# LeonhardFeiner/sparse_rcnn

Measured on AMD Instinct MI355X. Metric: active-voxels/sec fwd+bwd, ScanNet U-Net backbone, higher is better.
Workload: dtype f32

## Files before the change

### include/scn_mi355x.h

```cpp
#ifndef SCN_MI355X_H
#define SCN_MI355X_H

#include <stdint.h>

#ifdef __cplusplus
extern "C" {
#endif

#define SCN_OK 0
#define SCN_EINVAL 1
#define SCN_ESIZE 2
#define SCN_EHASH 3
#define SCN_EHIP 4

#define SCN_ABI_VERSION 5

#define SCN_F_RELU_IN 1
#define SCN_F_W_TRANSPOSED 2
#define SCN_F_OFF_REVERSE 4
#define SCN_F_RESIDUAL_LAST 8
#define SCN_F_SPLIT_SUM 16
#define SCN_F_TILE_ORDER_X 64
#define SCN_F_GEMM_V1 32

// ... 68 lines not shown
int scn_gemm_table(const float* X, int64_t n_in, int cin, const int32_t* table, int n_off, int64_t n_out,
                   const float* W, const float* bias, const float* residual, const float* relu_mask, float* Y,
                   int cout, int flags, scn_stream_t stream);

int64_t scn_tiles_scratch_bytes(int n_off, int64_t n);
int scn_tiles_build(const int32_t* table, int n_off, int64_t n, int32_t* perm, int32_t* tstab, uint32_t* tile_mask,
                    int32_t* tile_order, void* scratch, scn_stream_t stream);
int64_t scn_tiles_order_ints(int64_t n, int with_x);
int scn_tiles_build_x(const int32_t* table, int n_off, int64_t n, int32_t* perm, int32_t* tstab, uint32_t* tile_mask,
                      int32_t* tile_order, int with_x, void* scratch, scn_stream_t stream);

int64_t scn_sort_pairs_scratch_bytes(int64_t n);
int scn_sort_pairs(const uint32_t* keys, const int32_t* vals, int64_t n, int bits, uint32_t* keys_out,
                   int32_t* vals_out, void* scratch, scn_stream_t stream);

int64_t scn_conv_tiles_scratch_bytes(int cin, int64_t n_out, int cout);
int64_t scn_conv_tiles_arrival_counters(int cin, int64_t n_out, int cout);
int scn_conv_tiles(const float* X, int64_t n_in, int cin, const int32_t* tstab, const uint32_t* tile_mask, const int32_t* perm,
                   const int32_t* tile_order, int n_off, int64_t n_out, const float* W, const float* bias, const float* residual,
                   const float* relu_mask, float* Y, int cout, int flags, void* scratch, int32_t* arrival,
                   scn_stream_t stream);
typedef struct scn_conv_role {
    const void* X; const void* W; const void* bias; const void* residual; const void* relu_mask; void* Y;
    int32_t flags; int32_t reserved;
} scn_conv_role;
int scn_conv_tiles_chain(int n_roles, const scn_conv_role* roles, int64_t n_in, int cin, const int32_t* tstab,
                         const uint32_t* tile_mask, const int32_t* perm, const int32_t* tile_order, int n_off, int64_t n_out,
                         int cout, void* scratch, int32_t* arrival, scn_stream_t stream);
void scn_conv_tiles_chain_counts(int64_t out[2], int reset);
void scn_conv_tiles_path_counts(int64_t out[4], int reset);
int64_t scn_conv_tiles_split_count(int reset);
int scn_conv_tiles_finish(int cin, int64_t n_out, const float* bias, const float* residual, const float* relu_mask,
                          float* Y, int cout, int flags, void* scratch, scn_stream_t stream);

int64_t scn_conv_tiles_bf16_image_bytes(int cin, int cout, int n_off);
int scn_conv_tiles_bf16_pack(const float* W, int cin, int cout, int n_off, int flags, uint16_t* image, scn_stream_t stream);
int scn_conv_tiles_bf16_pack_many(int n, const float* const* W_host, const int32_t* cin_host, const int32_t* cout_host,
                                  const int32_t* n_off_host, const int32_t* flags_host, uint16_t* const* image_host,
                                  scn_stream_t stream);
int64_t scn_conv_tiles_bf16_scratch_bytes(int cin, int64_t n_out, int cout);
int64_t scn_conv_tiles_bf16_arrival_counters(int cin, int64_t n_out, int cout);
int scn_conv_tiles_bf16(const uint16_t* X, int64_t n_in, int cin, const int32_t* tstab, const uint32_t* tile_mask,
                        const int32_t* perm, const int32_t* tile_order, int n_off, int64_t n_out, const uint16_t* image,
                        const float* bias, const uint16_t* residual, const uint16_t* relu_mask, uint16_t* Y, int cout,
                        int flags, void* scratch, int32_t* arrival, scn_stream_t stream);

int scn_gemm_rules(const float* X, int cin, const int32_t* in_rows, const int32_t* out_rows,
                   const int64_t* prefix_host, int n_off, const float* W, const float* bias, const float* relu_mask,
                   float* Y, int cout, int flags, scn_stream_t stream);

int64_t scn_wgrad_scratch_bytes(int cin, int cout, const int64_t* prefix_host, int n_off);
int scn_wgrad_rules(const float* X, int cin, const float* dY, int cout, const int32_t* in_rows,
                    const int32_t* out_rows, const int64_t* prefix_host, int n_off, float* dW, void* scratch,
                    int flags, scn_stream_t stream);

int scn_gemm_rows2(const void* X0, int cx0, const void* X1, int cx1, int64_t n, const float* W, const float* bias,
                   const void* residual, const void* relu_mask, void* Y0, int cy0, void* Y1, int cy1, int flags,
                   int bf16_storage, scn_stream_t stream);

int scn_gemm_table_bf16(const uint16_t* X, int64_t n_in, int cin, const int32_t* table, int n_off, int64_t n_out,
                        const float* W, const float* bias, const uint16_t* residual, const uint16_t* relu_mask,
                        uint16_t* Y, int cout, int flags, scn_stream_t stream);
int scn_gemm_rules_bf16(const uint16_t* X, int cin, const int32_t* in_rows, const int32_t* out_rows,
                        const int64_t* prefix_host, int n_off, const float* W, const float* bias,
                        const uint16_t* relu_mask, uint16_t* Y, int cout, int flags, scn_stream_t stream);

int scn_wgrad_rules_bf16(const uint16_t* X, int cin, const uint16_t* dY, int cout, const int32_t* in_rows,
                         const int32_t* out_rows, const int64_t* prefix_host, int n_off, float* dW, void* scratch,
                         int flags, scn_stream_t stream);
int scn_wgrad_bias_rules_bf16(const uint16_t* X, int cin, const uint16_t* dY, int cout, const int32_t* in_rows,
                              const int32_t* out_rows, const int64_t* prefix_host, int n_off, float* dW, float* db,
                              uint32_t db_offsets, void* scratch, int flags, scn_stream_t stream);
int scn_wgrad_bias_rules(const float* X, int cin, const float* dY, int cout, const int32_t* in_rows,
                         const int32_t* out_rows, const int64_t* prefix_host, int n_off, float* dW, float* db,
                         uint32_t db_offsets, void* scratch, int flags, scn_stream_t stream);

int scn_wgrad_defer_begin(void);
int scn_wgrad_defer_flush(scn_stream_t stream);
int scn_wgrad_step_begin(void);
int scn_wgrad_step_hold(int on);
int scn_wgrad_step_flush(scn_stream_t stream);
int scn_wgrad_step_discard(void);
void scn_wgrad_group_counts(int64_t out[4], int reset);
int64_t scn_wgrad_scratch_bytes2(int cin, int cout, const int64_t* prefix_host, int n_off);
int scn_wgrad_bias_rules2(const float* X0, const float* dY0, const float* X1, const float* dY1, int cin, int cout,
                          const int32_t* in_rows, const int32_t* out_rows, const int64_t* prefix_host, int n_off,
                          float* dW, float* db, uint32_t db_offsets, void* scratch, int flags, scn_stream_t stream);

int64_t scn_wgrad_scratch_bytes_n(int cin, int cout, const int64_t* prefix_host, int n_off, int n_prob);
int scn_wgrad_bias_rules_n(const float* const* Xs, const float* const* dYs, int n_prob, int cin, int cout,
                          const int32_t* in_rows, const int32_t* out_rows, const int64_t* prefix_host, int n_off,
                          float* dW, float* db, uint32_t db_offsets, void* scratch, int flags, scn_stream_t stream);
int scn_wgrad_bias_rules_n_bf16(const uint16_t* const* Xs, const uint16_t* const* dYs, int n_prob, int cin, int cout,
                               const int32_t* in_rows, const int32_t* out_rows, const int64_t* prefix_host, int n_off,
                               float* dW, float* db, uint32_t db_offsets, void* scratch, int flags, scn_stream_t stream);
int scn_wgrad_bias_rules2_bf16(const uint16_t* X0, const uint16_t* dY0, const uint16_t* X1, const uint16_t* dY1, int cin,
                               int cout, const int32_t* in_rows, const int32_t* out_rows, const int64_t* prefix_host,
                               int n_off, float* dW, float* db, uint32_t db_offsets, void* scratch, int flags,
                               scn_stream_t stream);

#define SCN_COLSUM_BLOCKS 512
int scn_colsum(const float* dY, int64_t n, int c, float* db, void* scratch, scn_stream_t stream);
int scn_colsum_bf16(const uint16_t* dY, int64_t n, int c, float* db, void* scratch, scn_stream_t stream);


int scn_relu_fwd(const float* X, int64_t count, float* Y, scn_stream_t stream);
int scn_relu_bwd(const float* X, const float* dY, int64_t count, float* dX, scn_stream_t stream);
int scn_add(const float* A, const float* B, int64_t count, float* Y, scn_stream_t stream);

int64_t scn_bn_scratch_bytes(int c);
int scn_bn_stats(const float* X, int64_t n, int c, float* mean, float* var_biased,
                 void* scratch , scn_stream_t stream);
int scn_bn_fwd(const float* X, int64_t n, int c, const float* mean, const float* var, float eps, const float* gamma,
               const float* beta, float leak, float* Y, scn_stream_t stream);
int scn_bn_bwd(const float* X, const float* dY, int64_t n, int c, const float* mean, const float* var, float eps,
               const float* gamma, const float* beta, float leak, int training, float* dX, float* dgamma, float* dbeta,
               void* scratch , scn_stream_t stream);

int scn_bn_sums(const float* X, int64_t n, int c, double* sums, void* scratch, scn_stream_t stream);
int scn_bn_bwd_reduce(const float* X, const float* dY, int64_t n, int c, const float* mean, const float* var, float eps,
                      const float* gamma, const float* beta, float leak, float* dgamma, float* dbeta, double* sums,
                      void* scratch, scn_stream_t stream);
int scn_bn_bwd_apply(const float* X, const float* dY, int64_t n, int c, const float* mean, const float* var, float eps,
                     const float* gamma, const float* beta, float leak, const double* sums, int64_t n_stat, float* dX,
                     scn_stream_t stream);

int scn_input_fwd(const float* feats, const int32_t* item_row, const int32_t* row_count, const int32_t* row_first,
                  int64_t n_items, int64_t n_rows, int c, int mode, float* Y, double* acc64, int32_t* row_last,
                  scn_stream_t stream);
int scn_input_bwd(const float* dY, const int32_t* item_row, const int32_t* row_count, const int32_t* row_first,
                  const int32_t* row_last, int64_t n_items, int c, int mode, float* dfeats, scn_stream_t stream);
int scn_gather_rows(const float* X, const int32_t* rows, int64_t m, int c, float* Y, scn_stream_t stream);
int scn_segment_sum(const float* dY, const int32_t* item_row, int64_t n_items, int64_t n_rows, int c, float* dX,
                    double* acc64, scn_stream_t stream);

int64_t scn_segment_pool_scratch_bytes(int n_samples, int c);
int scn_sample_counts(const int32_t* coords, int64_t n, int n_samples, int32_t* cnt, int32_t* unsorted, scn_stream_t stream);
int scn_segment_pool_fwd(const float* X, const int32_t* coords, int64_t n, int c, int n_samples, int op, float* Y,
                         int32_t* cnt, int32_t* unsorted, void* scratch, scn_stream_t stream);
int scn_segment_pool_bwd(const float* X, const float* Y, const float* dY, const int32_t* coords, int64_t n, int c,
                         int n_samples, int op, const int32_t* cnt, float* dX, void* scratch, scn_stream_t stream);

int scn_sparse_to_dense_fwd(const float* X, const int32_t* coords, int64_t n, int c, const int64_t* size3_host,
                            float* out, scn_stream_t stream);
int scn_sparse_to_dense_bwd(const float* dOut, const int32_t* coords, int64_t n, int c, const int64_t* size3_host,
                            float* dX, scn_stream_t stream);

int scn_pool_fwd(const float* X, const int32_t* child, int64_t n_coarse, int c, int average, float* Y,
                 scn_stream_t stream);
int scn_pool_bwd(const float* X, const float* Y, const float* dY, const int32_t* parent, int64_t n_fine, int c,
                 int average, float* dX, scn_stream_t stream);


int scn_mask_scatter(const float* scores, int64_t m, int k, const int32_t* src_point, const int32_t* box_of,
                     const int64_t* class_of_box, int num_valid, const int64_t* row_base, float* out,
                     scn_stream_t stream);

int scn_mask_gather(const float* scores, int64_t m, int k, const int32_t* src_point, const int32_t* box_of,
                    const int64_t* label_of_box, const int64_t* gt_base, const float* gt_flat, float* pred, float* gt,
                    uint8_t* keep_row, scn_stream_t stream);
int scn_mask_gather_bwd(const float* dpred, int64_t m, int k, const int32_t* box_of, const int64_t* label_of_box,
                        const int64_t* gt_base, float* dscores, scn_stream_t stream);

int scn_nms(const float* boxes, int batch, int n, float overlap_threshold, uint8_t* keep, scn_stream_t stream);
int64_t scn_nms_scratch_bytes(int batch, int n);
int scn_nms_bits(const float* boxes, int batch, int n, float overlap_threshold, uint8_t* keep, void* scratch,
                 scn_stream_t stream);

int64_t scn_topk_scratch_bytes(int batch);
int scn_topk_boxes(const float* scores, const float* boxes, int batch, int64_t n, int k, float* out_scores,
                   int64_t* out_index, float* out_boxes, void* scratch, scn_stream_t stream);


int64_t scn_vox_scratch_bytes(int64_t n);
int scn_vox_project(const float* points, int64_t n, const float* rot_and_scale_host, const float* offset_host,
                    float* aug, float* shift_max, void* scratch, scn_stream_t stream);

int scn_vox_discretize(const float* aug, int64_t n, const float* shift, const int32_t* test_start_host,
                       const int32_t* size_host, int32_t* discrete, int32_t* table, scn_stream_t stream);

int scn_vox_gather(const int32_t* discrete, const int32_t* rows, int64_t m, const int32_t* start_host,
                   int64_t batch_index, int64_t* out, scn_stream_t stream);


int scn_pad_params_many(int n, const float* const* in_host, float* const* out_host, const int32_t* desc_host, int backward,
                        scn_stream_t stream);
// ... 188 lines not shown
```

### sparse_rcnn_amd/_lib.py

```python
from __future__ import annotations

import ctypes as C
import os

import torch

_HERE = os.path.dirname(os.path.abspath(__file__))
LIB_PATH = os.environ.get("SCN_MI355X_LIB") or os.path.join(_HERE, "libscn_mi355x.so")

_lib = None

p = C.c_void_p
i32, i64, f32 = C.c_int, C.c_int64, C.c_float

_SIGS = {
    "scn_abi_version": (C.c_int, []),
    "scn_last_error_string": (C.c_char_p, []),
    "scn_debug_set": (C.c_int, [C.c_char_p, C.c_char_p]),
    "scn_debug_get": (C.c_int, [C.c_char_p, C.POINTER(C.c_int), C.POINTER(i64)]),
    "scn_hash_capacity": (i64, [i64]),
    "scn_coords_to_i32": (C.c_int, [p, i64, p, p, C.POINTER(i64), p]),
    "scn_dedup_scratch_bytes": (i64, [i64]),
    "scn_dedup_build": (C.c_int, [p, i64, i32, p, p, i64, p, p, p, p, p, C.POINTER(i64), p]),
    "scn_dedup_launch": (C.c_int, [p, i64, i32, p, p, i64, p, p, p, p, p, p, p]),
    "scn_dedup_launch_div": (C.c_int, [p, i64, i32, i32, i32, p, p, i64, p, p, p, p, p, p, p]),
    "scn_child_table_div": (C.c_int, [p, p, i64, i64, i32, i32, i32, p, p, p]),
    "scn_parent_lookup_div": (C.c_int, [p, i64, i32, i32, i32, p, p, i64, p, p, p]),
    "scn_subm_table": (C.c_int, [p, i64, p, p, i64, i32, p, p]),
    "scn_child_table": (C.c_int, [p, p, i64, i64, p, p, p]),
    "scn_rules_blocks": (i64, [i32, i64]),
    "scn_rules_scan": (C.c_int, [p, i32, i64, p, p, C.POINTER(i64), p]),
    "scn_rules_fill": (C.c_int, [p, i32, i64, p, p, p, p, p]),
    "scn_pyramid_workspace_bytes": (i64, [i64, i32, i32]),
    "scn_pyramid_build": (C.c_int, [p, i64, i32, i32, p, i64, C.POINTER(i64), p]),
    "scn_pyramid_build_ex": (C.c_int, [p, i64, i32, i32, p, i64, C.POINTER(i64), i32, p]),
    "scn_roi_units": (i64, [i64]),
    "scn_roi_count": (C.c_int, [p, i64, p, i32, p, p, p, p]),
    "scn_roi_fill": (C.c_int, [p, i64, p, i32, p, p, p, p, p, p]),
    "scn_roi_inside": (C.c_int, [p, p, i64, i64, i32, p, p]),
    "scn_roi_coords": (C.c_int, [p, p, p, i64, p, p]),
    "scn_roi_boxes": (C.c_int, [p, p, i32, p, p, p, p]),
    "scn_gemm_table": (C.c_int, [p, i64, i32, p, i32, i64, p, p, p, p, p, i32, i32, p]),
    "scn_tiles_scratch_bytes": (i64, [i32, i64]),
    "scn_tiles_build": (C.c_int, [p, i32, i64, p, p, p, p, p, p]),
    "scn_tiles_build_x": (C.c_int, [p, i32, i64, p, p, p, p, i32, p, p]),
    "scn_tiles_order_ints": (i64, [i64, i32]),
    "scn_sort_pairs_scratch_bytes": (i64, [i64]),
    "scn_sort_pairs": (C.c_int, [p, p, i64, i32, p, p, p, p]),
    "scn_conv_tiles_scratch_bytes": (i64, [i32, i64, i32]),
    "scn_conv_tiles_arrival_counters": (i64, [i32, i64, i32]),
    "scn_conv_tiles": (C.c_int, [p, i64, i32, p, p, p, p, i32, i64, p, p, p, p, p, i32, i32, p, p, p]),
    "scn_conv_tiles_chain": (C.c_int, [i32, p, i64, i32, p, p, p, p, i32, i64, i32, p, p, p]),
    "scn_conv_tiles_chain_counts": (None, [C.POINTER(i64), i32]),
    "scn_wgrad_tiles32_scratch_bytes": (i64, []),
    "scn_wgrad_tiles32": (C.c_int, [p, i64, p, i64, p, p, p, p, p, p, i32, p]),
    "scn_conv_tiles_path_counts": (None, [C.POINTER(i64), i32]),
    "scn_conv_tiles_split_count": (i64, [i32]),
    "scn_conv_tiles_finish": (C.c_int, [i32, i64, p, p, p, p, i32, i32, p, p]),
    "scn_conv_tiles_bf16_image_bytes": (i64, [i32, i32, i32]),
    "scn_conv_tiles_bf16_pack": (C.c_int, [p, i32, i32, i32, i32, p, p]),
    "scn_conv_tiles_bf16_pack_many": (C.c_int, [i32, p, p, p, p, p, p, p]),
    "scn_conv_tiles_bf16_scratch_bytes": (i64, [i32, i64, i32]),
    "scn_conv_tiles_bf16_arrival_counters": (i64, [i32, i64, i32]),
    "scn_conv_tiles_bf16": (C.c_int, [p, i64, i32, p, p, p, p, i32, i64, p, p, p, p, p, i32, i32, p, p, p]),
    "scn_gemm_rules": (C.c_int, [p, i32, p, p, C.POINTER(i64), i32, p, p, p, p, i32, i32, p]),
    "scn_wgrad_scratch_bytes": (i64, [i32, i32, C.POINTER(i64), i32]),
    "scn_wgrad_rules": (C.c_int, [p, i32, p, i32, p, p, C.POINTER(i64), i32, p, p, i32, p]),
    "scn_gemm_table_bf16": (C.c_int, [p, i64, i32, p, i32, i64, p, p, p, p, p, i32, i32, p]),
    "scn_gemm_rules_bf16": (C.c_int, [p, i32, p, p, C.POINTER(i64), i32, p, p, p, p, i32, i32, p]),
    "scn_gemm_rows2": (C.c_int, [p, i32, p, i32, i64, p, p, p, p, p, i32, p, i32, i32, i32, p]),
    "scn_wgrad_rules_bf16": (C.c_int, [p, i32, p, i32, p, p, C.POINTER(i64), i32, p, p, i32, p]),
    "scn_wgrad_bias_rules": (C.c_int, [p, i32, p, i32, p, p, C.POINTER(i64), i32, p, p, C.c_uint32, p, i32, p]),
    "scn_wgrad_bias_rules_bf16": (C.c_int, [p, i32, p, i32, p, p, C.POINTER(i64), i32, p, p, C.c_uint32, p, i32, p]),
    "scn_wgrad_scratch_bytes2": (i64, [i32, i32, C.POINTER(i64), i32]),
    "scn_wgrad_defer_begin": (C.c_int, []),
    "scn_wgrad_defer_flush": (C.c_int, [p]),
    "scn_wgrad_step_begin": (C.c_int, []),
    "scn_wgrad_step_hold": (C.c_int, [i32]),
    "scn_wgrad_step_flush": (C.c_int, [p]),
    "scn_wgrad_step_discard": (C.c_int, []),
    "scn_wgrad_group_counts": (None, [C.POINTER(i64), i32]),
    "scn_wgrad_bias_rules2": (C.c_int, [p, p, p, p, i32, i32, p, p, C.POINTER(i64), i32, p, p, C.c_uint32, p, i32, p]),
    "scn_wgrad_bias_rules2_bf16": (C.c_int, [p, p, p, p, i32, i32, p, p, C.POINTER(i64), i32, p, p, C.c_uint32, p, i32, p]),
    "scn_wgrad_scratch_bytes_n": (i64, [i32, i32, C.POINTER(i64), i32, i32]),
    "scn_wgrad_bias_rules_n": (C.c_int, [C.POINTER(p), C.POINTER(p), i32, i32, i32, p, p, C.POINTER(i64), i32, p, p, C.c_uint32, p, i32, p]),
    "scn_wgrad_bias_rules_n_bf16": (C.c_int, [C.POINTER(p), C.POINTER(p), i32, i32, i32, p, p, C.POINTER(i64), i32, p, p, C.c_uint32, p, i32, p]),
    "scn_colsum": (C.c_int, [p, i64, i32, p, p, p]),
    "scn_colsum_bf16": (C.c_int, [p, i64, i32, p, p, p]),
    "scn_relu_fwd": (C.c_int, [p, i64, p, p]),
    "scn_relu_bwd": (C.c_int, [p, p, i64, p, p]),
    "scn_add": (C.c_int, [p, p, i64, p, p]),
    "scn_bn_scratch_bytes": (i64, [i32]),
    "scn_bn_stats": (C.c_int, [p, i64, i32, p, p, p, p]),
    "scn_bn_sums": (C.c_int, [p, i64, i32, p, p, p]),
    "scn_bn_bwd_reduce": (C.c_int, [p, p, i64, i32, p, p, f32, p, p, f32, p, p, p, p, p]),
    "scn_bn_bwd_apply": (C.c_int, [p, p, i64, i32, p, p, f32, p, p, f32, p, i64, p, p]),
    "scn_bn_fwd": (C.c_int, [p, i64, i32, p, p, f32, p, p, f32, p, p]),
    "scn_bn_bwd": (C.c_int, [p, p, i64, i32, p, p, f32, p, p, f32, i32, p, p, p, p, p]),
    "scn_input_fwd": (C.c_int, [p, p, p, p, i64, i64, i32, i32, p, p, p, p]),
    "scn_input_bwd": (C.c_int, [p, p, p, p, p, i64, i32, i32, p, p]),
    "scn_gather_rows": (C.c_int, [p, p, i64, i32, p, p]),
    "scn_segment_sum": (C.c_int, [p, p, i64, i64, i32, p, p, p]),
    "scn_mask_scatter": (C.c_int, [p, i64, i32, p, p, p, i32, p, p, p]),
    "scn_mask_gather": (C.c_int, [p, i64, i32, p, p, p, p, p, p, p, p, p]),
    "scn_mask_gather_bwd": (C.c_int, [p, i64, i32, p, p, p, p, p]),
    "scn_vox_scratch_bytes": (i64, [i64]),
    "scn_vox_project": (C.c_int, [p, i64, p, p, p, p, p, p]),
    "scn_vox_discretize": (C.c_int, [p, i64, p, p, p, p, p, p]),
    "scn_vox_gather": (C.c_int, [p, p, i64, p, i64, p, p]),
    "scn_nms": (C.c_int, [p, i32, i32, f32, p, p]),
    "scn_dilate_gather_fwd": (C.c_int, [p, p, i32, C.POINTER(i64), i32, i32, p, p, p]),
    "scn_dilate_gather_bwd": (C.c_int, [p, p, i64, C.POINTER(i64), i32, i32, p, p]),
    "scn_cell_map": (C.c_int, [p, i64, i32, C.POINTER(i64), p, p, p, p]),
    "scn_nms_scratch_bytes": (i64, [i32, i32]),
    "scn_nms_bits": (C.c_int, [p, i32, i32, f32, p, p, p]),
    "scn_topk_scratch_bytes": (C.c_int64, [i32]),
    "scn_topk_boxes": (C.c_int, [p, p, i32, i64, i32, p, p, p, p, p]),
    "scn_pool_fwd": (C.c_int, [p, p, i64, i32, i32, p, p]),
    "scn_pool_bwd": (C.c_int, [p, p, p, p, i64, i32, i32, p, p]),
    "scn_segment_pool_scratch_bytes": (i64, [i32, i32]),
    "scn_sample_counts": (C.c_int, [p, i64, i32, p, p, p]),
    "scn_segment_pool_fwd": (C.c_int, [p, p, i64, i32, i32, i32, p, p, p, p, p]),
    "scn_segment_pool_bwd": (C.c_int, [p, p, p, p, i64, i32, i32, i32, p, p, p, p]),
    "scn_pad_params_many": (C.c_int, [i32, p, p, p, i32, p]),
    "scn_cast_f32_to_bf16": (C.c_int, [p, i64, p, p]),
    "scn_cast_bf16_to_f32": (C.c_int, [p, i64, p, p]),
    "scn_add_bf16": (C.c_int, [p, p, i64, p, p]),
    "scn_gather_rows_bf16": (C.c_int, [p, p, i64, i32, p, p]),
    "scn_segment_sum_bf16": (C.c_int, [p, p, i64, i64, i32, p, p, p]),
    "scn_pool_fwd_bf16": (C.c_int, [p, p, i64, i32, i32, p, p]),
    "scn_pool_bwd_bf16": (C.c_int, [p, p, p, p, i64, i32, i32, p, p]),
    "scn_sparse_to_dense_fwd_bf16": (C.c_int, [p, p, i64, i32, C.POINTER(i64), p, p]),
    "scn_sparse_to_dense_bwd_bf16": (C.c_int, [p, p, i64, i32, C.POINTER(i64), p, p]),
    "scn_exec_struct_bytes": (i64, [i32]),
    "scn_exec_requirements": (C.c_int, [p, i32, p, i32, C.POINTER(i64), C.POINTER(i64)]),
    "scn_exec_run": (C.c_int, [p, i32, p, i32, p, p, p, p, i64, p, p]),
    "scn_exec_run_streams": (C.c_int, [p, i32, p, i32, p, p, p, p, i64, p, p, p, p, i64]),
    "scn_exec_timing_enable": (C.c_int, [i32]),
    "scn_exec_timing_collect": (i64, [p, p, i64]),
    "scn_sparse_to_dense_fwd": (C.c_int, [p, p, i64, i32, C.POINTER(i64), p, p]),
    "scn_sparse_to_dense_bwd": (C.c_int, [p, p, i64, i32, C.POINTER(i64), p, p]),
    "scn_adam_segment_bytes": (i64, []),
    "scn_adam_launches": (C.c_int, [p, i32, C.POINTER(i32)]),
    "scn_adam_many": (C.c_int, [p, i32, C.c_double, C.c_double, C.c_double, C.c_double, p]),
    "scn_rpn_targets": (C.c_int, [p, i64, p, C.POINTER(i64), i32, p, p, p, p]),
    "scn_rpn_sample_workspace_bytes": (i64, []),
    "scn_rpn_sample_batchwise": (C.c_int, [p, i64, f32, f32, f32, C.c_uint64, C.c_uint64, p, p, p, p, p, p]),
    "scn_rpn_loss_scratch_bytes": (i64, [i64]),
    "scn_rpn_loss": (C.c_int, [p, p, p, p, p, p, i64, f32, p, p, p, p, p, p]),
    "scn_rpn_loss_scale": (C.c_int, [p, p, i64, p, p, p, p, p]),
    "scn_mask_overlap_draw": (C.c_int, [p, C.POINTER(i64), p, C.POINTER(i64), i32, p, p, i32, f32, i32, C.c_uint64,
                                        C.c_uint64, C.POINTER(i64), p, p, p, p, p]),
    "scn_mask_loss_scratch_bytes": (i64, [i64, i64]),
    "scn_mask_loss": (C.c_int, [p, i64, i32, p, p, p, C.POINTER(i64), p, C.POINTER(i64), p, C.POINTER(i64), C.POINTER(i64), i32,
                                p, p, p, p]),
    "scn_mask_loss_bwd": (C.c_int, [p, p, i64, i64, i32, p, p, p]),
    "scn_mask_pack": (C.c_int, [C.POINTER(p), C.POINTER(i64), C.POINTER(i64), i32, p, p]),
    "scn_xent_scratch_bytes": (i64, [i64, i32]),
    "scn_xent_fwd": (C.c_int, [p, i64, i32, p, p, i64, p, p, p, p]),
    "scn_xent_bwd": (C.c_int, [p, p, i64, i32, p, p, i64, p, p, p]),
    "scn_softmax_argmax": (C.c_int, [p, i64, i32, p, p, p]),
    "scn_eval_mask_bits": (C.c_int, [p, i64, i32, p, p, p, i32, f32, p, i64, i64, p, p]),
    "scn_eval_pack_threshold": (C.c_int, [p, i64, i64, f32, p, p]),
    "scn_eval_mask_iou": (C.c_int, [p, C.POINTER(i64), p, C.POINTER(i64), C.POINTER(i64), C.POINTER(i64), C.POINTER(i64),
                                    C.POINTER(i64), i32, p, p, p, p, p, p]),
    "scn_eval_bbox_iou": (C.c_int, [p, C.POINTER(i64), p, C.POINTER(i64), C.POINTER(i64), i32, p, p]),
    "scn_eval_match": (C.c_int, [p, p, p, p, i32, i64, p, p, p, p, p, p, p, i32, i32, p, p, p]),
    "scn_eval_confusion": (C.c_int, [p, p, i64, i32, p, p, p]),
    "scn_sample_stats": (C.c_int, [p, p, p, i64, i32, p, p, p, p]),
    "scn_sample_pack": (C.c_int, [p, i64, p, p, p, i32, p, p, i32, p, i32, i32, i32, i32, p, p, p, p, i64, p, p]),
    "scn_roialign_fwd": (C.c_int, [p, i32, C.POINTER(i64), i32, p, p, i64, C.POINTER(i64), p, p, p]),
# ... 124 lines not shown
```

### sparse_rcnn_amd/csrc/scn_common.h

```cpp
#pragma once
#include <hip/hip_runtime.h>
#include <atomic>
#include <stdint.h>
#include <stdio.h>
#include <string.h>

#include "../../include/scn_mi355x.h"

namespace scn {

extern thread_local char g_err[512];

inline int fail(int code, const char* fmt, const char* a = "", long long b = 0, long long c = 0) {
    snprintf(g_err, sizeof(g_err), fmt, a, b, c);
    return code;
}

#define SCN_HIP(expr)                                                                               \
    do {                                                                                            \
        hipError_t e_ = (expr);                                                                     \
        if (e_ != hipSuccess) {                                                                     \
            snprintf(scn::g_err, sizeof(scn::g_err), "%s failed: %s (%s:%d)", #expr,                \
                     hipGetErrorString(e_), __FILE__, __LINE__);                                    \
            return SCN_EHIP;                                                                        \
        }                                                                                           \
    } while (0)

#define SCN_LAUNCH_CHECK()                                                                          \
    do {                                                                                            \
        hipError_t e_ = hipGetLastError();                                                          \
        if (e_ != hipSuccess) {                                                                     \
            snprintf(scn::g_err, sizeof(scn::g_err), "kernel launch failed: %s (%s:%d)",            \
                     hipGetErrorString(e_), __FILE__, __LINE__);                                    \
            return SCN_EHIP;                                                                        \
        }                                                                                           \
    } while (0)

#define SCN_REQUIRE(cond)                                                                           \
    do {                                                                                            \
        if (!(cond)) {                                                                              \
            snprintf(scn::g_err, sizeof(scn::g_err), "%s: requirement failed: %s", __func__, #cond); \
            return SCN_EINVAL;                                                                      \
        }                                                                                           \
    } while (0)

enum Switch {
    SW_TS_SPLIT, SW_TS_SPLIT_MAX, SW_TS_NO_TAIL, SW_TS_W_HALF, SW_TS_W_BOTH, SW_TB_NB, SW_TB_KH, SW_TB_STREAM,
    SW_TB_NO_XORDER, SW_TS_STREAM, SW_TSS_NW, SW_EXEC_DEFER_SUMS, SW_PYRAMID_V1, SW_PYRAMID_ONE_STREAM, SW_WD_NO_T3,
    SW_WGRAD_BF16_MFMA, SW_WGRAD_SPLITS, SW_WD_NO_EVEC, SW_PYRAMID_NO_BRICKS, SW_CU_BUDGET, SW_EXP_A, SW_EXP_B, SW_TS_NO_CHAIN, SW_TS_PROG, SW_TB_NO_BINS,
    SW_EXEC_GROUP_WGRAD, SW_EXEC_GROUP_STEP, SW_COUNT
};
struct SwitchVal { bool set = false; long long i = 0; double f = 0.0; };
SwitchVal sw(Switch s);
inline int cu_budget() { const SwitchVal v = sw(SW_CU_BUDGET); return (v.set && v.i >= 32 && v.i <= 256) ? (int)v.i : 256; }

struct DeviceOnce {
    std::atomic<uint64_t> mask{0};
    static int cur() { int d = 0; return (hipGetDevice(&d) == hipSuccess && d >= 0 && d < 64) ? d : -1; }
    bool needed() const { const int d = cur(); return d < 0 || !(mask.load(std::memory_order_acquire) & (1ull << d)); }
    void done() { const int d = cur(); if (d >= 0) mask.fetch_or(1ull << d, std::memory_order_release); }
};

int wgrad_defer_group(bool on);

inline hipStream_t S(scn_stream_t s) { return reinterpret_cast<hipStream_t>(s); }

inline int64_t cdiv(int64_t a, int64_t b) { return (a + b - 1) / b; }

inline int ew_grid(int64_t work_items, int block) {
    int64_t g = cdiv(work_items, block);
    if (g > 256 * 8) g = 256 * 8;
    if (g < 1) g = 1;
    return (int)g;
}

}

#define SCN_EMPTY_KEY 0xFFFFFFFFFFFFFFFFull

__device__ __forceinline__ unsigned long long scn_pack_key(int x, int y, int z, int b) {
    return ((unsigned long long)(unsigned)b << 48) | ((unsigned long long)(unsigned)x << 32) |
           ((unsigned long long)(unsigned)y << 16) | (unsigned long long)(unsigned)z;
}

__device__ __forceinline__ unsigned long long scn_hash_slot(unsigned long long key, unsigned long long mask) {
    unsigned long long h = key;
    h ^= h >> 33;
    h *= 0xff51afd7ed558ccdull;
    h ^= h >> 33;
    h *= 0xc4ceb9fe1a85ec53ull;
    h ^= h >> 33;
    return h & mask;
}

__device__ __forceinline__ float scn_mask_sigmoid(float x) { return 1.f / (1.f + __expf(-x)); }

__device__ __forceinline__ float scn_box_iou(const float* as, const float* ae, float area_a, const float* bx) {
#pragma clang fp contract(off)
    float inter = 1.f;
#pragma unroll
    for (int d = 0; d < 3; ++d) {
        const float lo = fmaxf(as[d], bx[d]), hi = fminf(ae[d], bx[3 + d]);
        const float e = fmaxf((hi - lo), 0.f);
        inter = d == 0 ? e : (inter * e);
    }
    const float uni = (area_a + bx[6]) - inter;
    return (inter / uni);
}
```

### sparse_rcnn_amd/csrc/scn_conv.hip

```cpp
#include "scn_common.h"

using scn::S;
using scn::cdiv;

namespace scn {
bool gemm_lt_usable(const void* X0, const void* X1, int cx0, int cx1, const void* W);
int gemm_lt_rows(const void* X0, int cx0, const void* X1, int cx1, int64_t n, const float* W, const float* bias,
                 const void* residual, const void* relu_mask, void* Y0, int cy0, void* Y1, int cy1, int flags, bool hb,
                 scn_stream_t stream);
int gemm_lt_rules(const void* X, int cin, const int32_t* in_rows, const int32_t* out_rows, const int64_t* prefix_host,
                  int n_off, const float* W, const float* bias, const void* relu_mask, void* Y, int cout, int flags,
                  bool hb, scn_stream_t stream);
}

typedef float f32x16 __attribute__((ext_vector_type(16)));

#define MFMA(a, b, c) __builtin_amdgcn_mfma_f32_32x32x2f32((a), (b), (c), 0, 0, 0)

__device__ __forceinline__ int acc_row(int v, int h) { return (v & 3) + 8 * (v >> 2) + 4 * h; }

__device__ __forceinline__ float bf16_bits_to_f32(unsigned short h) { return __uint_as_float((unsigned)h << 16); }
__device__ __forceinline__ unsigned short f32_to_bf16_bits(float f) { return __builtin_bit_cast(unsigned short, (__bf16)f); }

template <bool FAST, bool WT, bool HB = false>
// ... 178 lines not shown
                           : X + (long long)(idx >= 0 ? idx : 0) * cin;
    tile_mac<FAST, WT, HB>(acc, xrow, idx >= 0, cin, Wo, cout, n, n_ok, h, flags & SCN_F_RELU_IN);

    const float bv = (bias && n_ok) ? bias[n] : 0.f;
#pragma unroll
    for (int v = 0; v < 16; ++v) {
        const int r = __shfl(orow, acc_row(v, h));
        if (r >= 0 && n_ok) {
            const long long off = (long long)r * cout + n;
            float y = acc[v] + bv;
            if (HB) {
                if (relu_mask && !(bf16_bits_to_f32(((const unsigned short*)relu_mask)[off]) > 0.f)) y = 0.f;
                ((unsigned short*)Y)[off] = f32_to_bf16_bits(y);
            } else {
                if (relu_mask && !(relu_mask[off] > 0.f)) y = 0.f;
                Y[off] = y;
            }
        }
    }
}

static int make_seg_tiles(const int64_t* prefix_host, int n_off, int tile, SegTiles& seg) {
    seg.n_off = n_off;
    seg.rule_start[0] = prefix_host[0];
    seg.tile_start[0] = 0;
    for (int o = 0; o < n_off; ++o) {
        int64_t cnt = prefix_host[o + 1] - prefix_host[o];
        if (cnt < 0) return SCN_EINVAL;
        seg.rule_start[o + 1] = prefix_host[o + 1];
        seg.tile_start[o + 1] = seg.tile_start[o] + cdiv(cnt, tile);
    }
    return SCN_OK;
}

static int gemm_rules_impl(const float* X, int cin, const int32_t* in_rows, const int32_t* out_rows,
                           const int64_t* prefix_host, int n_off, const float* W, const float* bias,
                           const float* relu_mask, float* Y, int cout, int flags, scn_stream_t stream, bool hb) {
    SCN_REQUIRE(prefix_host && n_off >= 1 && n_off <= 32 && cin >= 1 && cout >= 1);
    SegTiles seg;
    SCN_REQUIRE(make_seg_tiles(prefix_host, n_off, 32, seg) == SCN_OK);
    const long long tiles = seg.tile_start[n_off];
    if (tiles == 0) return SCN_OK;
    SCN_REQUIRE(X && in_rows && out_rows && W && Y);
    const bool fast = (cin % 8 == 0) && (((uintptr_t)X & 15) == 0) && (((uintptr_t)W & 15) == 0);
    const bool wt = flags & SCN_F_W_TRANSPOSED;
    if (fast && cout > 32 && !(flags & SCN_F_GEMM_V1))
        return scn::gemm_lt_rules(X, cin, in_rows, out_rows, prefix_host, n_off, W, bias, relu_mask, Y, cout, flags, hb,
                                  stream);
    dim3 grid((unsigned)cdiv(tiles, 4), (unsigned)cdiv(cout, 32));
#define LAUNCH_R(F, T, H)                                                                                     \
    hipLaunchKernelGGL((k_gemm_rules<F, T, H>), grid, dim3(256), 0, S(stream), X, cin, in_rows, out_rows, seg, \
                       W, bias, relu_mask, Y, cout, flags)
#define PICK_R(H)                                                                                             \
    do {                                                                                                      \
        if (fast && wt) LAUNCH_R(true, true, H);                                                              \
        else if (fast) LAUNCH_R(true, false, H);                                                              \
        else if (wt) LAUNCH_R(false, true, H);                                                                \
        else LAUNCH_R(false, false, H);                                                                       \
    } while (0)
    if (hb) PICK_R(true); else PICK_R(false);
#undef PICK_R
#undef LAUNCH_R
    SCN_LAUNCH_CHECK();
    return SCN_OK;
}

extern "C" int scn_gemm_rules(const float* X, int cin, const int32_t* in_rows, const int32_t* out_rows,
                              const int64_t* prefix_host, int n_off, const float* W, const float* bias,
                              const float* relu_mask, float* Y, int cout, int flags, scn_stream_t stream) {
    return gemm_rules_impl(X, cin, in_rows, out_rows, prefix_host, n_off, W, bias, relu_mask, Y, cout, flags, stream,
                           false);
}

extern "C" int scn_gemm_rules_bf16(const uint16_t* X, int cin, const int32_t* in_rows, const int32_t* out_rows,
                                   const int64_t* prefix_host, int n_off, const float* W, const float* bias,
                                   const uint16_t* relu_mask, uint16_t* Y, int cout, int flags, scn_stream_t stream) {
    return gemm_rules_impl((const float*)X, cin, in_rows, out_rows, prefix_host, n_off, W, bias,
                           (const float*)relu_mask, (float*)Y, cout, flags, stream, true);
}

template <bool HB>
__global__ __launch_bounds__(256) void k_colsum_partial(const float* __restrict__ dY, long long n, int c,
                                                        float* __restrict__ partial) {
    const unsigned short* dYh = (const unsigned short*)dY;
    const long long rows_per_block = (n + gridDim.x - 1) / gridDim.x;
    const long long r_lo = blockIdx.x * rows_per_block;
    long long r_hi = r_lo + rows_per_block;
    if (r_hi > n) r_hi = n;
    __shared__ float red[256];
    for (int c0 = 0; c0 < c; c0 += 256) {
        const int width = min(256, c - c0);
        const int lanes_per_row = width;
        const int rows_par = 256 / lanes_per_row > 0 ? 256 / lanes_per_row : 1;
        const int col = threadIdx.x % lanes_per_row;
        const int rsub = threadIdx.x / lanes_per_row;
        float s = 0.f;
        if (rsub < rows_par)
            for (long long r = r_lo + rsub; r < r_hi; r += rows_par)
                s += HB ? bf16_bits_to_f32(dYh[r * c + c0 + col]) : dY[r * c + c0 + col];
        red[threadIdx.x] = (rsub < rows_par) ? s : 0.f;
        __syncthreads();
        if (threadIdx.x < width) {
            float t = 0.f;
            for (int k = 0; k < rows_par; ++k) t += red[k * lanes_per_row + threadIdx.x];
            partial[(long long)blockIdx.x * c + c0 + threadIdx.x] = t;
        }
        __syncthreads();
    }
}

__global__ __launch_bounds__(256) void k_colsum_final(const float* __restrict__ partial, int nblk, int c,
                                                      float* __restrict__ db) {
    const int col = blockIdx.x;
    float s = 0.f;
    for (int b = threadIdx.x; b < nblk; b += 256) s += partial[(long long)b * c + col];
#pragma unroll
    for (int d = 32; d >= 1; d >>= 1) s += __shfl_down(s, d);
    __shared__ float w[4];
    if ((threadIdx.x & 63) == 0) w[threadIdx.x >> 6] = s;
    __syncthreads();
    if (threadIdx.x == 0) db[col] = (w[0] + w[1]) + (w[2] + w[3]);
}

static int colsum_impl(const float* dY, int64_t n, int c, float* db, void* scratch, scn_stream_t stream, bool hb) {
    SCN_REQUIRE(n >= 0 && c >= 1 && db && scratch);
    int nblk = (int)(n < SCN_COLSUM_BLOCKS * 8 ? cdiv(n, 8) : SCN_COLSUM_BLOCKS);
    if (nblk < 1) nblk = 1;
    if (n > 0) SCN_REQUIRE(dY);
    if (hb)
        hipLaunchKernelGGL(k_colsum_partial<true>, dim3(nblk), dim3(256), 0, S(stream), dY, (long long)n, c, (float*)scratch);
    else
        hipLaunchKernelGGL(k_colsum_partial<false>, dim3(nblk), dim3(256), 0, S(stream), dY, (long long)n, c, (float*)scratch);
    SCN_LAUNCH_CHECK();
    hipLaunchKernelGGL(k_colsum_final, dim3(c), dim3(256), 0, S(stream), (const float*)scratch, nblk, c, db);
    SCN_LAUNCH_CHECK();
    return SCN_OK;
}

extern "C" int scn_colsum(const float* dY, int64_t n, int c, float* db, void* scratch, scn_stream_t stream) {
    return colsum_impl(dY, n, c, db, scratch, stream, false);
}

extern "C" int scn_colsum_bf16(const uint16_t* dY, int64_t n, int c, float* db, void* scratch, scn_stream_t stream) {
    return colsum_impl((const float*)dY, n, c, db, scratch, stream, true);
}
```

### sparse_rcnn_amd/csrc/scn_debug.hip

```cpp
#include <stdlib.h>

#include <mutex>

#include "scn_common.h"

namespace scn {
namespace {
struct Entry { const char* name; SwitchVal v; };
Entry g_sw[SW_COUNT] = {
    {"SCN_TS_SPLIT", {}},        {"SCN_TS_SPLIT_MAX", {}},  {"SCN_TS_NO_TAIL", {}},       {"SCN_TS_W_HALF", {}},
    {"SCN_TS_W_BOTH", {}},       {"SCN_TB_NB", {}},         {"SCN_TB_KH", {}},            {"SCN_TB_STREAM", {}},
    {"SCN_TB_NO_XORDER", {}},    {"SCN_TS_STREAM", {}},     {"SCN_TSS_NW", {}},           {"SCN_EXEC_DEFER_SUMS", {}},
    {"SCN_PYRAMID_V1", {}},      {"SCN_PYRAMID_ONE_STREAM", {}}, {"SCN_WD_NO_T3", {}},    {"SCN_WGRAD_BF16_MFMA", {}},
    {"SCN_WGRAD_SPLITS", {}},    {"SCN_WD_NO_EVEC", {}},    {"SCN_PYRAMID_NO_BRICKS", {}},            {"SCN_CU_BUDGET", {}},
    {"SCN_EXP_A", {}},           {"SCN_EXP_B", {}},         {"SCN_TS_NO_CHAIN", {}},
    {"SCN_TS_PROG", {}},         {"SCN_TB_NO_BINS", {}},    {"SCN_EXEC_GROUP_WGRAD", {}},
    {"SCN_EXEC_GROUP_STEP", {}},
};
std::once_flag g_once;
std::mutex g_mu;

void assign(SwitchVal& v, const char* s) {
    v.set = s != nullptr;
    v.i = s ? atoll(s) : 0;
    v.f = s ? atof(s) : 0.0;
}
void load_env() {
    for (int k = 0; k < SW_COUNT; ++k) assign(g_sw[k].v, getenv(g_sw[k].name));
}
}

SwitchVal sw(Switch s) {
    std::call_once(g_once, load_env);
    std::lock_guard<std::mutex> lock(g_mu);
    return g_sw[s].v;
}
}

extern "C" int scn_debug_set(const char* name, const char* value) {
    SCN_REQUIRE(name != nullptr);
    std::call_once(scn::g_once, scn::load_env);
    std::lock_guard<std::mutex> lock(scn::g_mu);
    for (int k = 0; k < scn::SW_COUNT; ++k)
        if (strcmp(scn::g_sw[k].name, name) == 0) {
            scn::assign(scn::g_sw[k].v, value);
            return SCN_OK;
        }
    return scn::fail(SCN_EINVAL, "scn_debug_set: no switch named %s", name);
}

extern "C" int scn_debug_get(const char* name, int* is_set, int64_t* value) {
    SCN_REQUIRE(name != nullptr);
    for (int k = 0; k < scn::SW_COUNT; ++k)
        if (strcmp(scn::g_sw[k].name, name) == 0) {
            const scn::SwitchVal v = scn::sw((scn::Switch)k);
            if (is_set) *is_set = v.set ? 1 : 0;
            if (value) *value = v.i;
            return SCN_OK;
        }
    return scn::fail(SCN_EINVAL, "scn_debug_get: no switch named %s", name);
}
```

### sparse_rcnn_amd/csrc/scn_exec.hip

```cpp
#include <stdlib.h>
#include <vector>

#include <atomic>
#include <mutex>
#include <vector>

#include "scn_common.h"

using scn::cdiv;

namespace {

struct Ctx {
    const scn_exec_level* levels;
    int n_levels;
    void* const* bufs;
    const void* const* params;
    void* const* grads;
    void* scratch;
    int32_t* arrival;
    scn_stream_t stream;
};

inline int64_t align256(int64_t b) { return (b + 255) & ~(int64_t)255; }

int64_t wgrad_scratch_of(const scn_exec_op& o, const scn_exec_level& L) {
    switch (o.op) {
    case SCN_OP_WGRAD_SUBM: return scn_wgrad_scratch_bytes(o.cin, o.cout, L.prefix_host, 27);
    case SCN_OP_WGRAD2_SUBM: return scn_wgrad_scratch_bytes2(o.cin, o.cout, L.prefix_host, 27);
    case SCN_OP_WGRAD_DOWN:
    case SCN_OP_WGRAD_UP: return scn_wgrad_scratch_bytes(o.cin, o.cout, L.c_prefix_host, 8);
    case SCN_OP_WGRAD_IDENT: {
        const int64_t ident[2] = {0, (o.flags & SCN_XF_COARSE_ROWS) ? L.n_coarse : L.n};
        return scn_wgrad_scratch_bytes(o.cin, o.cout, ident, 1);
    }
    default: return 0;
    }
}

inline bool bf(const scn_exec_op& o) { return (o.flags & SCN_XF_BF16) != 0; }
inline int call_flags(const scn_exec_op& o) { return o.flags & 0xffff; }
inline int64_t rows_of(const scn_exec_op& o, const scn_exec_level& L) {
    return (o.flags & SCN_XF_COARSE_ROWS) ? L.n_coarse : L.n;
}

template <typename T>
inline T* B(const Ctx& c, int id) { return id < 0 ? nullptr : (T*)c.bufs[id]; }
template <typename T>
inline const T* P(const Ctx& c, int id) { return id < 0 ? nullptr : (const T*)c.params[id]; }
template <typename T>
inline T* G(const Ctx& c, int id) { return id < 0 ? nullptr : (T*)c.grads[id]; }

int run_op(const Ctx& c0, const scn_exec_op& o, void* own_scratch = nullptr) {
    SCN_REQUIRE(o.level >= 0 && o.level < c0.n_levels);
    const scn_exec_level& L = c0.levels[o.level];
    Ctx c = c0;
    if (own_scratch) c.scratch = own_scratch;
    const int fl = call_flags(o);
    const bool h = bf(o);
    scn_stream_t st = c.stream;
    typedef uint16_t u16;
    switch (o.op) {
    case SCN_OP_GEMM_IDENT: {
        const int64_t n = rows_of(o, L);
        if (h) return scn_gemm_table_bf16(B<u16>(c, o.x), n, o.cin, nullptr, 1, n, P<float>(c, o.w), P<float>(c, o.b),
                                          B<u16>(c, o.r), B<u16>(c, o.m), B<u16>(c, o.y), o.cout, fl, st);
        return scn_gemm_table(B<float>(c, o.x), n, o.cin, nullptr, 1, n, P<float>(c, o.w), P<float>(c, o.b), B<float>(c, o.r),
                              B<float>(c, o.m), B<float>(c, o.y), o.cout, fl, st);
    }
    case SCN_OP_CONV_SUBM:
    case SCN_OP_CONV_CHILD: {
        const bool child = o.op == SCN_OP_CONV_CHILD;
        const int64_t n_in = L.n, n_out = child ? L.n_coarse : L.n;
        const int n_off = child ? 8 : 27;
        const int32_t* tstab = child ? L.c_tstab : L.tstab;
        const uint32_t* tmask = child ? L.c_tile_mask : L.tile_mask;
        const int32_t* perm = child ? L.c_perm : L.perm;
        const int32_t* order = child ? L.c_tile_order : L.tile_order;
        if (h) {
            int32_t* arr = scn_conv_tiles_bf16_arrival_counters(o.cin, n_out, o.cout) ? c.arrival : nullptr;
            const int flx = fl | ((!child && (L.flags & SCN_XL_TILE_ORDER_X)) ? SCN_F_TILE_ORDER_X : 0);
            return scn_conv_tiles_bf16(B<u16>(c, o.x), n_in, o.cin, tstab, tmask, perm, order, n_off, n_out, P<u16>(c, o.w),
                                       P<float>(c, o.b), B<u16>(c, o.r), B<u16>(c, o.m), B<u16>(c, o.y), o.cout, flx, c.scratch,
                                       arr, st);
        }
        int32_t* arr = o.cin > 32 ? c.arrival : nullptr;
        return scn_conv_tiles(B<float>(c, o.x), n_in, o.cin, tstab, tmask, perm, order, n_off, n_out, P<float>(c, o.w),
                              P<float>(c, o.b), B<float>(c, o.r), B<float>(c, o.m), B<float>(c, o.y), o.cout, fl, c.scratch, arr,
                              st);
    }
    case SCN_OP_RULES_CHILD: {
        if (h) return scn_gemm_rules_bf16(B<u16>(c, o.x), o.cin, L.c_out_rows, L.c_in_rows, L.c_prefix_host, 8, P<float>(c, o.w),
                                          P<float>(c, o.b), B<u16>(c, o.m), B<u16>(c, o.y), o.cout, fl, st);
        return scn_gemm_rules(B<float>(c, o.x), o.cin, L.c_out_rows, L.c_in_rows, L.c_prefix_host, 8, P<float>(c, o.w),
                              P<float>(c, o.b), B<float>(c, o.m), B<float>(c, o.y), o.cout, fl, st);
    }
    case SCN_OP_ROWS2: {
        const int64_t n = rows_of(o, L);
        if (o.y1 >= 0)
            return scn_gemm_rows2(B<void>(c, o.x), o.cin, nullptr, 0, n, P<float>(c, o.w), nullptr, nullptr, nullptr,
                                  B<void>(c, o.y), o.cout, B<void>(c, o.y1), o.c1, fl, h ? 1 : 0, st);
        return scn_gemm_rows2(B<void>(c, o.x), o.cin, B<void>(c, o.x1), o.c1, n, P<float>(c, o.w), P<float>(c, o.b), nullptr,
                              nullptr, B<void>(c, o.y), o.cout, nullptr, 0, fl, h ? 1 : 0, st);
    }
    case SCN_OP_WGRAD_SUBM: {
        const uint32_t dbm = o.b >= 0 ? (1u << 13) : 0u;
        if (h) return scn_wgrad_bias_rules_bf16(B<u16>(c, o.x), o.cin, B<u16>(c, o.y), o.cout, L.in_rows, L.out_rows, L.prefix_host,
                                                27, G<float>(c, o.w), G<float>(c, o.b), dbm, c.scratch, fl, st);
        return scn_wgrad_bias_rules(B<float>(c, o.x), o.cin, B<float>(c, o.y), o.cout, L.in_rows, L.out_rows, L.prefix_host, 27,
                                    G<float>(c, o.w), G<float>(c, o.b), dbm, c.scratch, fl, st);
    }
    case SCN_OP_WGRAD2_SUBM: {
        const uint32_t dbm = o.b >= 0 ? (1u << 13) : 0u;
        if (h) return scn_wgrad_bias_rules2_bf16(B<u16>(c, o.x), B<u16>(c, o.y), B<u16>(c, o.x1), B<u16>(c, o.y1), o.cin, o.cout,
                                                 L.in_rows, L.out_rows, L.prefix_host, 27, G<float>(c, o.w), G<float>(c, o.b), dbm,
                                                 c.scratch, fl, st);
        return scn_wgrad_bias_rules2(B<float>(c, o.x), B<float>(c, o.y), B<float>(c, o.x1), B<float>(c, o.y1), o.cin, o.cout,
                                     L.in_rows, L.out_rows, L.prefix_host, 27, G<float>(c, o.w), G<float>(c, o.b), dbm, c.scratch,
                                     fl, st);
    }
    case SCN_OP_WGRAD_DOWN: {
        if (h) return scn_wgrad_rules_bf16(B<u16>(c, o.x), o.cin, B<u16>(c, o.y), o.cout, L.c_in_rows, L.c_out_rows,
                                           L.c_prefix_host, 8, G<float>(c, o.w), c.scratch, fl, st);
        return scn_wgrad_rules(B<float>(c, o.x), o.cin, B<float>(c, o.y), o.cout, L.c_in_rows, L.c_out_rows, L.c_prefix_host, 8,
                               G<float>(c, o.w), c.scratch, fl, st);
    }
    case SCN_OP_WGRAD_UP: {
        if (o.b < 0) {
            if (h) return scn_wgrad_rules_bf16(B<u16>(c, o.x), o.cin, B<u16>(c, o.y), o.cout, L.c_out_rows, L.c_in_rows,
                                               L.c_prefix_host, 8, G<float>(c, o.w), c.scratch, fl, st);
            return scn_wgrad_rules(B<float>(c, o.x), o.cin, B<float>(c, o.y), o.cout, L.c_out_rows, L.c_in_rows, L.c_prefix_host,
                                   8, G<float>(c, o.w), c.scratch, fl, st);
        }
        if (h) return scn_wgrad_bias_rules_bf16(B<u16>(c, o.x), o.cin, B<u16>(c, o.y), o.cout, L.c_out_rows, L.c_in_rows,
                                                L.c_prefix_host, 8, G<float>(c, o.w), G<float>(c, o.b), 0xFFu, c.scratch, fl, st);
        return scn_wgrad_bias_rules(B<float>(c, o.x), o.cin, B<float>(c, o.y), o.cout, L.c_out_rows, L.c_in_rows, L.c_prefix_host,
                                    8, G<float>(c, o.w), G<float>(c, o.b), 0xFFu, c.scratch, fl, st);
    }
    case SCN_OP_WGRAD_IDENT: {
        const int64_t ident[2] = {0, rows_of(o, L)};
        float* dW = G<float>(c, o.w);
        SCN_REQUIRE(dW != nullptr);
        dW += o.aux;
        if (o.b < 0) {
            if (h) return scn_wgrad_rules_bf16(B<u16>(c, o.x), o.cin, B<u16>(c, o.y), o.cout, nullptr, nullptr, ident, 1, dW,
                                               c.scratch, fl, st);
            return scn_wgrad_rules(B<float>(c, o.x), o.cin, B<float>(c, o.y), o.cout, nullptr, nullptr, ident, 1, dW, c.scratch, fl,
                                   st);
        }
        if (h) return scn_wgrad_bias_rules_bf16(B<u16>(c, o.x), o.cin, B<u16>(c, o.y), o.cout, nullptr, nullptr, ident, 1, dW,
                                                G<float>(c, o.b), 1u, c.scratch, fl, st);
        return scn_wgrad_bias_rules(B<float>(c, o.x), o.cin, B<float>(c, o.y), o.cout, nullptr, nullptr, ident, 1, dW,
                                    G<float>(c, o.b), 1u, c.scratch, fl, st);
    }
    case SCN_OP_COLSUM: {
        const int64_t n = rows_of(o, L);
        if (h) return scn_colsum_bf16(B<u16>(c, o.x), n, o.cin, G<float>(c, o.b), c.scratch, st);
        return scn_colsum(B<float>(c, o.x), n, o.cin, G<float>(c, o.b), c.scratch, st);
    }
    case SCN_OP_ADD: {
        const int64_t count = rows_of(o, L) * o.cin;
        if (h) return scn_add_bf16(B<u16>(c, o.x), B<u16>(c, o.x1), count, B<u16>(c, o.y), st);
        return scn_add(B<float>(c, o.x), B<float>(c, o.x1), count, B<float>(c, o.y), st);
    }
    case SCN_OP_CAST: {
        const int64_t count = rows_of(o, L) * o.cin;
        if (h) return scn_cast_f32_to_bf16(B<float>(c, o.x), count, B<u16>(c, o.y), st);
        return scn_cast_bf16_to_f32(B<u16>(c, o.x), count, B<float>(c, o.y), st);
    }
    default:
        return scn::fail(SCN_EINVAL, "scn_exec_run: unknown op %s%lld", "", o.op);
    }
}

}

extern "C" int64_t scn_exec_struct_bytes(int which) {
    return which == 0 ? (int64_t)sizeof(scn_exec_op) : (which == 1 ? (int64_t)sizeof(scn_exec_level) : -1);
}

namespace {
int pass_needs(const scn_exec_op* ops, int n_ops, const scn_exec_level* levels, int n_levels, int64_t* shared, int64_t* wg_sum,
               int64_t* wg_max, int* n_wg, int64_t* arrival) {
    int64_t sb = 256, ac = 0, ws = 0, wm = 0;
    int nw = 0;
    for (int i = 0; i < n_ops; ++i) {
        const scn_exec_op& o = ops[i];
        SCN_REQUIRE(o.level >= 0 && o.level < n_levels);
        const scn_exec_level& L = levels[o.level];
        int64_t s = 0, a = 0;
        switch (o.op) {
        case SCN_OP_CONV_SUBM:
        case SCN_OP_CONV_CHILD: {
            const int64_t n_out = o.op == SCN_OP_CONV_CHILD ? L.n_coarse : L.n;
            if (bf(o)) {
                s = scn_conv_tiles_bf16_scratch_bytes(o.cin, n_out, o.cout);
                a = scn_conv_tiles_bf16_arrival_counters(o.cin, n_out, o.cout);
            } else {
                s = scn_conv_tiles_scratch_bytes(o.cin, n_out, o.cout);
                a = scn_conv_tiles_arrival_counters(o.cin, n_out, o.cout);
            }
            break;
        }
        case SCN_OP_COLSUM: s = (int64_t)SCN_COLSUM_BLOCKS * o.cin * (int64_t)sizeof(float); break;
        default: {
            const int64_t w = wgrad_scratch_of(o, L);
            if (w < 0) return scn::fail(SCN_EINVAL, "scn_exec: op %s%lld has bad arguments", "", i);
            if (w > 0) { ws += align256(w); ++nw; if (w > wm) wm = w; }
            break;
        }
        }
        if (s < 0) return scn::fail(SCN_EINVAL, "scn_exec: op %s%lld has bad arguments", "", i);
        if (s > sb) sb = s;
        if (a > ac) ac = a;
    }
    *shared = sb; *wg_sum = ws; *wg_max = wm; *n_wg = nw; *arrival = ac;
    return SCN_OK;
}
}

extern "C" int scn_exec_requirements(const scn_exec_op* ops, int n_ops, const scn_exec_level* levels, int n_levels,
                                     int64_t* scratch_bytes, int64_t* arrival_counters) {
    SCN_REQUIRE(n_ops >= 0 && (n_ops == 0 || ops) && levels && n_levels >= 1 && scratch_bytes && arrival_counters);
    int64_t shared, wg_sum, wg_max, ac;
    int n_wg;
    const int rc = pass_needs(ops, n_ops, levels, n_levels, &shared, &wg_sum, &wg_max, &n_wg, &ac);
    if (rc != SCN_OK) return rc;
    int64_t sb = align256(shared) + wg_sum;
    if (wg_max > sb) sb = wg_max;
    *scratch_bytes = sb;
    *arrival_counters = ac;
    return SCN_OK;
}

namespace {
struct EventPool {
    static constexpr int N = 32;
    hipEvent_t ev[N] = {};
    int next = 0;
    bool ok = false;
    bool init() {
        if (ok) return true;
        for (auto& e : ev)
            if (hipEventCreateWithFlags(&e, hipEventDisableTiming) != hipSuccess) return false;
        return ok = true;
    }
    hipEvent_t take() { hipEvent_t e = ev[next]; next = (next + 1) % N; return e; }
};
thread_local EventPool g_events;

struct TimingRec { hipEvent_t a, b; int64_t info[7]; };
struct Timing {
    std::mutex mu;
    std::atomic<bool> on{false}, all{false};
    std::vector<hipEvent_t> pool;
    size_t used = 0;
    std::vector<TimingRec> recs;
    hipEvent_t take() {
        if (used == pool.size()) {
            hipEvent_t e = nullptr;
            if (hipEventCreate(&e) != hipSuccess) return nullptr;
            pool.push_back(e);
        }
        return pool[used++];
    }
};
Timing g_timing;

inline bool is_wgrad(int op) {
    return op == SCN_OP_WGRAD_SUBM || op == SCN_OP_WGRAD2_SUBM || op == SCN_OP_WGRAD_DOWN || op == SCN_OP_WGRAD_UP ||
           op == SCN_OP_WGRAD_IDENT;
}
inline bool is_leaf(int op) {
    return op == SCN_OP_WGRAD_SUBM || op == SCN_OP_WGRAD2_SUBM || op == SCN_OP_WGRAD_DOWN || op == SCN_OP_WGRAD_UP ||
           op == SCN_OP_WGRAD_IDENT || op == SCN_OP_COLSUM;
}

bool overwritten_later(const scn_exec_op* ops, int n_ops, int i, void* const* bufs) {
    const scn_exec_op& o = ops[i];
    const int reads[4] = {o.x, o.y, o.x1, o.y1};
    for (int j = i + 1; j < n_ops; ++j) {
        if (is_leaf(ops[j].op)) continue;
        const int writes[2] = {ops[j].y, ops[j].y1};
        for (int w : writes) {
            if (w < 0) continue;
            for (int r : reads)
                if (r >= 0 && (r == w || (bufs[r] != nullptr && bufs[r] == bufs[w]))) return true;
        }
    }
    return false;
}
}

extern "C" int scn_exec_run_streams(const scn_exec_op* ops, int n_ops, const scn_exec_level* levels, int n_levels,
                                    void* const* bufs, const void* const* params, void* const* grads, void* scratch,
                                    int64_t scratch_bytes, int32_t* arrival, scn_stream_t stream, scn_stream_t side_stream,
                                    void* side_scratch, int64_t side_scratch_bytes) {
    SCN_REQUIRE(n_ops >= 0 && (n_ops == 0 || ops) && levels && n_levels >= 1 && bufs && scratch && scratch_bytes >= 256);
    const bool fork = side_stream != nullptr && side_stream != stream && side_scratch != nullptr && side_scratch_bytes >= scratch_bytes;
    if (fork && !g_events.init()) return scn::fail(SCN_EHIP, "%sevents for the side stream could not be created", "");
    const bool defer_env = !(scn::sw(scn::SW_EXEC_DEFER_SUMS).set && scn::sw(scn::SW_EXEC_DEFER_SUMS).i == 0);
    int n_wg = 0;
    for (int i = 0; i < n_ops; ++i) n_wg += is_wgrad(ops[i].op) ? 1 : 0;
    std::vector<int64_t> own(defer_env && !fork && n_wg >= 2 ? n_ops : 0, 0);
    bool defer = false;
    if (!own.empty()) {
        int64_t shared, wg_sum, wg_max, ac;
        int nw;
        const int rc_needs = pass_needs(ops, n_ops, levels, n_levels, &shared, &wg_sum, &wg_max, &nw, &ac);
        if (rc_needs != SCN_OK) return rc_needs;
        if (align256(shared) + wg_sum <= scratch_bytes) {
            int64_t cursor = align256(shared);
            for (int i = 0; i < n_ops; ++i) {
                const int64_t w = is_wgrad(ops[i].op) ? wgrad_scratch_of(ops[i], levels[ops[i].level]) : 0;
                if (w > 0) { own[i] = cursor; cursor += align256(w); }
            }
            defer = true;
        }
    }
    const scn::SwitchVal group_sw = scn::sw(scn::SW_EXEC_GROUP_WGRAD);
    const bool group = defer && !(group_sw.set && group_sw.i == 0) && !g_timing.on;
    Ctx c{levels, n_levels, bufs, params, grads, scratch, arrival, stream};
    Ctx cs{levels, n_levels, bufs, params, grads, side_scratch, arrival, side_stream};
    if (defer) SCN_REQUIRE(scn_wgrad_defer_begin() == SCN_OK);
    if (group) SCN_REQUIRE(scn::wgrad_defer_group(true) == SCN_OK);
    bool side_used = false;
    for (int i = 0; i < n_ops; ++i) {
        int rc;
        if (fork && is_leaf(ops[i].op)) {
            hipEvent_t e = g_events.take();
            SCN_HIP(hipEventRecord(e, scn::S(stream)));
            SCN_HIP(hipStreamWaitEvent(scn::S(side_stream), e, 0));
            rc = run_op(cs, ops[i]);
            side_used = true;
        } else if (g_timing.on && (g_timing.all || ops[i].op == SCN_OP_CONV_SUBM || ops[i].op == SCN_OP_CONV_CHILD)) {
            std::lock_guard<std::mutex> lock(g_timing.mu);
            const scn_exec_op& o = ops[i];
            const scn_exec_level& L = levels[o.level];
            const bool child = o.op == SCN_OP_CONV_CHILD;
            TimingRec r{};
            r.a = g_timing.take();
            r.b = g_timing.take();
            if (r.a && r.b) SCN_HIP(hipEventRecord(r.a, scn::S(stream)));
            rc = run_op(c, ops[i], defer && own[i] ? (char*)scratch + own[i] : nullptr);
            if (r.a && r.b) {
                SCN_HIP(hipEventRecord(r.b, scn::S(stream)));
                r.info[0] = o.op; r.info[1] = bf(o) ? 1 : 0; r.info[2] = o.cin; r.info[3] = o.cout;
                r.info[4] = L.n; r.info[5] = child ? L.n_coarse : L.n;
                r.info[6] = child ? L.n : (L.prefix_host ? L.prefix_host[27] - L.prefix_host[0] : 0);
                g_timing.recs.push_back(r);
            }
        } else if (group && is_wgrad(ops[i].op) && overwritten_later(ops, n_ops, i, bufs)) {
            (void)scn::wgrad_defer_group(false);
            rc = run_op(c, ops[i], own[i] ? (char*)scratch + own[i] : nullptr);
            (void)scn::wgrad_defer_group(true);
        } else {
            rc = run_op(c, ops[i], defer && own[i] ? (char*)scratch + own[i] : nullptr);
        }
        if (rc != SCN_OK) {
            char inner[400];
            snprintf(inner, sizeof(inner), "%s", scn::g_err);
            snprintf(scn::g_err, sizeof(scn::g_err), "scn_exec_run: op %d (kind %d, level %d): %s", i, ops[i].op, ops[i].level,
                     inner);
            if (defer) (void)scn_wgrad_defer_flush(stream);
            return rc;
        }
    }
    if (defer) {
        const int rc = scn_wgrad_defer_flush(stream);
        if (rc != SCN_OK) return rc;
    }
    if (side_used) {
        hipEvent_t e = g_events.take();
        SCN_HIP(hipEventRecord(e, scn::S(side_stream)));
        SCN_HIP(hipStreamWaitEvent(scn::S(stream), e, 0));
    }
    return SCN_OK;
}

extern "C" int scn_exec_timing_enable(int on) {
    std::lock_guard<std::mutex> lock(g_timing.mu);
    g_timing.on = on != 0;
    g_timing.all = on == 2;
    return SCN_OK;
}

extern "C" int64_t scn_exec_timing_collect(float* ms, int64_t* info, int64_t cap) {
    std::lock_guard<std::mutex> lock(g_timing.mu);
    int64_t n = 0;
    size_t taken = 0;
    for (; taken < g_timing.recs.size() && n < cap; ++taken) {
        const TimingRec& r = g_timing.recs[taken];
        float t = 0.f;
        if (hipEventSynchronize(r.b) != hipSuccess || hipEventElapsedTime(&t, r.a, r.b) != hipSuccess) continue;
        ms[n] = t;
        for (int j = 0; j < 7; ++j) info[7 * n + j] = r.info[j];
        ++n;
    }
    g_timing.recs.erase(g_timing.recs.begin(), g_timing.recs.begin() + (ptrdiff_t)taken);
    if (g_timing.recs.empty()) g_timing.used = 0;
    return n;
}

extern "C" int scn_exec_run(const scn_exec_op* ops, int n_ops, const scn_exec_level* levels, int n_levels, void* const* bufs,
                            const void* const* params, void* const* grads, void* scratch, int64_t scratch_bytes,
                            int32_t* arrival, scn_stream_t stream) {
    return scn_exec_run_streams(ops, n_ops, levels, n_levels, bufs, params, grads, scratch, scratch_bytes, arrival, stream,
                                nullptr, nullptr, 0);
}
```

### sparse_rcnn_amd/csrc/scn_wgrad.hip

```cpp
#include <stdlib.h>

#include <string.h>
#include <mutex>
#include <vector>

#include "scn_common.h"

#ifndef WD_DEEP_ALL
#define WD_DEEP_ALL 1
#endif

using scn::S;
using scn::cdiv;

typedef float f32x4 __attribute__((ext_vector_type(4)));
#define MFMA16(a, b, c) __builtin_amdgcn_mfma_f32_16x16x4f32((a), (b), (c), 0, 0, 0)

#ifndef WD_EXP
#define WD_EXP 0
#endif
#ifndef WD_TIMELINE
#define WD_TIMELINE 0
#endif
#if WD_TIMELINE
// ... 299 lines not shown
        for (int b = 0; b < TB; ++b) acc[a][b] = (f32x4){0.f, 0.f, 0.f, 0.f};
    f32x4 dbacc[TB];
#pragma unroll
    for (int b = 0; b < TB; ++b) dbacc[b] = (f32x4){0.f, 0.f, 0.f, 0.f};
    s16x8 ones;
#pragma unroll
    for (int e = 0; e < 8; ++e) ones[e] = (lane & 15) == 0 ? (short)0x3F80 : (short)0;

    const int g = lane >> 4, q = (lane & 15) >> 2, pp = lane & 3;
    int tr_a[2][TA], tr_b[2][TB];
#pragma unroll
    for (int t = 0; t < 2; ++t) {
        const int row = 8 * g + 4 * t + q;
#pragma unroll
        for (int a = 0; a < TA; ++a) tr_a[t][a] = wtb_off(row, 2 * (wi * TA + a) + (pp >> 1)) + 8 * (pp & 1);
#pragma unroll
        for (int b = 0; b < TB; ++b) tr_b[t][b] = IMG + wtb_off(row, 2 * (wj * TB + b) + (pp >> 1)) + 8 * (pp & 1);
    }

    int idx0[NLD], idx1[NLD];
    uint4 st[NLD];
    if (nsteps > 0) {
        load_idx(0, idx0);
        load_idx(1, idx1);
        load_rows(idx0, st);
    }
    for (int s = 0; s < nsteps; ++s) {
        const int buf = s & 1;
        store_rows(buf, st);
        if (s + 1 < nsteps) {
            if (s & 1) { load_rows(idx0, st); load_idx(s + 2, idx1); }
            else { load_rows(idx1, st); load_idx(s + 2, idx0); }
        }
        __syncthreads();
        const char* base = wlds + buf * 2 * IMG;
        bf16x8 fa[TA], fb[TB];
#pragma unroll
        for (int a = 0; a < TA; ++a) {
            const s16x4 lo = __builtin_amdgcn_ds_read_tr16_b64_v4i16((__attribute__((address_space(3))) s16x4*)(base + tr_a[0][a]));
            const s16x4 hi = __builtin_amdgcn_ds_read_tr16_b64_v4i16((__attribute__((address_space(3))) s16x4*)(base + tr_a[1][a]));
            fa[a] = __builtin_bit_cast(bf16x8, __builtin_shufflevector(lo, hi, 0, 1, 2, 3, 4, 5, 6, 7));
        }
#pragma unroll
        for (int b = 0; b < TB; ++b) {
            const s16x4 lo = __builtin_amdgcn_ds_read_tr16_b64_v4i16((__attribute__((address_space(3))) s16x4*)(base + tr_b[0][b]));
            const s16x4 hi = __builtin_amdgcn_ds_read_tr16_b64_v4i16((__attribute__((address_space(3))) s16x4*)(base + tr_b[1][b]));
            fb[b] = __builtin_bit_cast(bf16x8, __builtin_shufflevector(lo, hi, 0, 1, 2, 3, 4, 5, 6, 7));
        }
#pragma unroll
        for (int a = 0; a < TA; ++a)
#pragma unroll
            for (int b = 0; b < TB; ++b) acc[a][b] = MFMAB32(fa[a], fb[b], acc[a][b]);
        if (do_db) {
#pragma unroll
            for (int b = 0; b < TB; ++b) dbacc[b] = MFMAB32(__builtin_bit_cast(bf16x8, ones), fb[b], dbacc[b]);
        }
    }

    float* slab = slabs + ((long long)unit * (plan.nbi * plan.nbj) + blockIdx.z) * (CBI * CBJ);
    const int i = lane & 15, kq = lane >> 4;
#pragma unroll
    for (int a = 0; a < TA; ++a)
#pragma unroll
        for (int b = 0; b < TB; ++b)
#pragma unroll
            for (int j = 0; j < 4; ++j)
                slab[(16 * (wi * TA + a) + 4 * kq + j) * CBJ + 16 * (wj * TB + b) + i] = acc[a][b][j];
    if (do_db && kq == 0) {
#pragma unroll
        for (int b = 0; b < TB; ++b) {
            const int c = co0 + 16 * (wj * TB + b) + i;
            if (c < cout_pad) db_slabs[(long long)unit * cout_pad + c] = dbacc[b][0];
        }
    }
}

struct SumArgs {
    const float* slabs; float* dW; const float* db_slabs; float* db;
    int unit_start[129];
    int n_off, n_real, cbi, cbj, nbi, nbj, cin, cout, cout_pad, main_blocks, G;
    unsigned db_mask;
};

template <int V, typename A>
__device__ __forceinline__ void wgradd_sum_body(const A& a, int block) {
    typedef typename Frag<V>::type vec_t;
    const float* __restrict__ slabs = a.slabs;
    const int cin = a.cin, cout = a.cout, G = a.G;
    if (block >= a.main_blocks) {
        const int cidx = block - a.main_blocks;
        const int prob = cidx / cout, co = cidx - prob * cout;
        float s = 0.f;
        for (int o = 0; o < a.n_real; ++o) {
            if (!((a.db_mask >> o) & 1u)) continue;
            const int ov = prob * a.n_real + o;
            for (int u = a.unit_start[ov] + threadIdx.x; u < a.unit_start[ov + 1]; u += 256)
                s += a.db_slabs[(long long)u * a.cout_pad + co];
        }
#pragma unroll
        for (int d = 32; d >= 1; d >>= 1) s += __shfl_down(s, d);
        __shared__ float w[4];
        if ((threadIdx.x & 63) == 0) w[threadIdx.x >> 6] = s;
        __syncthreads();
        if (threadIdx.x == 0) a.db[cidx] = (w[0] + w[1]) + (w[2] + w[3]);
        return;
    }
    __shared__ __attribute__((aligned(16))) float part[256 * V];
    const int per_block = 256 / G;
    const int el = threadIdx.x % per_block, g = threadIdx.x / per_block;
    const long long total = (long long)a.n_off * cin * (cout / V);
    const int cbi = a.cbi, cbj = a.cbj, nblk = a.nbi * a.nbj;
    const long long eg = (long long)block * per_block + el;
    vec_t sum;
#pragma unroll
    for (int v = 0; v < V; ++v) sum[v] = 0.f;
    long long e = 0;
    if (eg < total) {
        e = eg * V;
        const int co = (int)(e % cout);
        const int ci = (int)((e / cout) % cin);
        const int o = (int)(e / ((long long)cin * cout));
        const int blk = (ci / cbi) * a.nbj + co / cbj;
        const int u0 = a.unit_start[o], nu = a.unit_start[o + 1] - u0;
        const long long stride = (long long)nblk * cbi * cbj;
        const float* p = slabs + ((long long)u0 * nblk + blk) * (cbi * cbj) + (ci % cbi) * cbj + co % cbj;
        for (int s = g; s < nu; s += G) {
            const vec_t x = *(const vec_t*)(p + s * stride);
#pragma unroll
            for (int v = 0; v < V; ++v) sum[v] += x[v];
        }
    }
    if (G > 1) {
        *(vec_t*)(part + (g * per_block + el) * V) = sum;
        __syncthreads();
        if (g == 0) {
            for (int k = 1; k < G; ++k) {
                const vec_t x = *(const vec_t*)(part + (k * per_block + el) * V);
#pragma unroll
                for (int v = 0; v < V; ++v) sum[v] += x[v];
            }
        }
    }
    if (g == 0 && eg < total) *(vec_t*)(a.dW + e) = sum;
}

template <int V>
__global__ __launch_bounds__(256) void k_wgradd_sum(SumArgs a) { wgradd_sum_body<V>(a, (int)blockIdx.x); }

#define WD_SUM_MANY 6
struct SumJobs { int n; int block_start[WD_SUM_MANY + 1]; SumArgs job[WD_SUM_MANY]; };

__global__ __launch_bounds__(256) void k_wgradd_sum_many(SumJobs jobs) {
    int j = 0;
    while (j + 1 < jobs.n && (int)blockIdx.x >= jobs.block_start[j + 1]) ++j;
    wgradd_sum_body<4>(jobs.job[j], (int)blockIdx.x - jobs.block_start[j]);
}

__global__ __launch_bounds__(256) void k_wgradd_sum_many_tab(const SumArgs* __restrict__ job,
                                                             const int* __restrict__ block_start, int n) {
    int lo = 0, hi = n;
    while (hi - lo > 1) {
        const int mid = (lo + hi) >> 1;
        if ((int)blockIdx.x >= block_start[mid]) lo = mid; else hi = mid;
    }
    wgradd_sum_body<4>(job[lo], (int)blockIdx.x - block_start[lo]);
}

namespace {
struct Shape { int ta, tb; bool quad; };

Shape pick_shape(int cin, int cout, bool hb = false) {
    Shape s;
    s.ta = cin > 32 ? 4 : 2;
    s.tb = cout > 32 ? 4 : 2;
    s.quad = cin > 64 && cout > 64;
    const bool no_t3 = scn::sw(scn::SW_WD_NO_T3).set;
    if (!hb && !no_t3 && cin % 48 == 0 && cout % 48 == 0 && cin <= 96 && cout <= 96) { s.ta = s.tb = 3; s.quad = false; }
    return s;
}

int tb_tiles(int c) { return c <= 32 ? 1 : (c <= 64 ? 2 : 4); }
bool tb_usable(int cin, int cout) {
    const bool off = scn::sw(scn::SW_WGRAD_BF16_MFMA).set && scn::sw(scn::SW_WGRAD_BF16_MFMA).i == 0;
    return !off && cin % 8 == 0 && cout % 8 == 0;
}

int make_dplan(int cin, int cout, const int64_t* prefix_host, int n_off, DPlan& pl, bool hb_mfma = false, bool hb = false) {
    const Shape sh = pick_shape(cin, cout, hb || hb_mfma);
    pl.n_off = n_off;
    pl.n_real = n_off;
    pl.p_rules = 0;
    pl.cbi = 16 * sh.ta * (sh.quad ? 2 : 1);
    pl.cbj = 16 * sh.tb * (sh.quad ? 2 : 1);
    if (hb_mfma) { pl.cbi = 32 * tb_tiles(cin); pl.cbj = 32 * tb_tiles(cout); }
    pl.nbi = (int)cdiv(cin, pl.cbi);
    pl.nbj = (int)cdiv(cout, pl.cbj);
    pl.rule_start[0] = prefix_host[0];
    for (int o = 0; o < n_off; ++o) {
        if (prefix_host[o + 1] < prefix_host[o]) return SCN_EINVAL;
        pl.rule_start[o + 1] = prefix_host[o + 1];
    }
    const int64_t total = prefix_host[n_off] - prefix_host[0];
    const int64_t nblk = (int64_t)pl.nbi * pl.nbj;
    int occ = sh.quad ? 2 : (sh.ta == 4 && sh.tb == 4 ? 2 : (sh.ta == 2 && sh.tb == 2 ? 4 : 3));
    int rounds = (sh.quad ? nblk > 1 : (sh.ta == 4 && sh.tb == 4) || (sh.ta == 3 && nblk > 1)) ? 2 : 1;
    const bool tb_big = hb_mfma && tb_tiles(cin) == 4 && tb_tiles(cout) == 4;
    if (hb_mfma) { occ = 4; rounds = 1; }
    int64_t target = ((int64_t)scn::cu_budget() * occ * rounds) / nblk - n_off;
    if (scn::sw(scn::SW_WGRAD_SPLITS).set) target = (int)scn::sw(scn::SW_WGRAD_SPLITS).i;
    if (target < 1) target = 1;
    const int64_t gran = hb_mfma ? 32 : (sh.quad ? 16 : 64);
    int64_t per = cdiv(cdiv(total, target), gran) * gran;
    if (tb_big && !scn::sw(scn::SW_WGRAD_SPLITS).set && n_off > 0 && total > 0 && per < 1024) {
        const int64_t avg = cdiv(total, n_off), slots = ((int64_t)scn::cu_budget() * 2) / nblk;
        int64_t k = (slots + n_off / 2) / n_off;
        if (k < 1) k = 1;
        for (;; --k) {
            per = cdiv(cdiv(avg, k), gran) * gran;
            int64_t units = 0;
            for (int o = 0; o < n_off; ++o) units += cdiv(prefix_host[o + 1] - prefix_host[o], per);
            if (units <= slots || k == 1) break;
        }
    }
    const int64_t min_per = hb_mfma ? 256 : (sh.quad ? 128 : 512);
    if (per < min_per) per = min_per;
    pl.per = per;
    pl.unit_start[0] = 0;
    for (int o = 0; o < n_off; ++o)
        pl.unit_start[o + 1] = pl.unit_start[o] + (int)cdiv(prefix_host[o + 1] - prefix_host[o], per);
    return SCN_OK;
}
}

extern "C" int64_t scn_wgrad_scratch_bytes(int cin, int cout, const int64_t* prefix_host, int n_off) {
    if (!prefix_host || n_off < 1 || n_off > 32 || cin < 1 || cout < 1) return -1;
    int64_t best = -1;
    for (int v = 0; v < 3; ++v) {
        if (v == 2 && !tb_usable(cin, cout)) continue;
        DPlan pl;
        if (make_dplan(cin, cout, prefix_host, n_off, pl, v == 2, v == 1) != SCN_OK) return -1;
        const int64_t b = (int64_t)pl.unit_start[n_off] *
                              ((int64_t)pl.nbi * pl.nbj * pl.cbi * pl.cbj + (int64_t)pl.nbj * pl.cbj) * (int64_t)sizeof(float) + 512;
        if (b > best) best = b;
    }
    return best;
}

static int multi_problem_plan(int cin, int cout, const int64_t* prefix_host, int n_off, int n_prob, DPlan& pl,
                              bool hb_mfma = false, bool hb = false) {
    if (n_off > 32 || n_prob < 2 || n_prob > WD_MAX_PROB || prefix_host[0] != 0) return SCN_EINVAL;
    int64_t vprefix[129];
    const int64_t P = prefix_host[n_off];
    for (int v = 0; v <= n_prob * n_off; ++v) vprefix[v] = (v / n_off) * P + prefix_host[v % n_off];
    vprefix[n_prob * n_off] = n_prob * P;
    const int rc = make_dplan(cin, cout, vprefix, n_prob * n_off, pl, hb_mfma, hb);
    pl.n_real = n_off;
    pl.p_rules = P;
    return rc;
}

namespace {
struct WdLaunch {
    DPlan pl;
    int ta, tb;
    bool quad, edge, ident, hb;
    const float* X; const float* dY;
    int cin, cout, relu_in, cout_pad, n_prob;
    const int32_t* in_rows; const int32_t* out_rows;
    float* slabs; float* db_slabs;
    unsigned db_mask;
    WdOps more;
    int kind() const { return WD_KIND(ta, tb, quad, edge, ident, hb); }
    int units() const { return pl.unit_start[pl.n_off]; }
    int64_t workgroups() const { return (int64_t)units() * pl.nbi * pl.nbj; }
    double wg_work() const { return (double)pl.per * pl.cbi * pl.cbj; }
    size_t lds() const { return (quad ? 4 * 64 : 4 * ta * tb * 4 * 64 + 4 * 64) * sizeof(float); }
};

std::atomic<int64_t> g_counts[4];

int launch_direct(const WdLaunch& r, scn_stream_t stream) {
    g_counts[2].fetch_add(1, std::memory_order_relaxed);
    const dim3 grid((unsigned)r.units(), 1, (unsigned)(r.pl.nbi * r.pl.nbj));
    const bool ident = r.ident, edge = r.edge, hb = r.hb;
#define LAUNCH_WD(TA_, TB_, Q_, E_, I_, H_)                                                                      \
    do {                                                                                                         \
        const size_t lds_ = ((Q_) ? 4 * 64 : 4 * (TA_) * (TB_) * 4 * 64 + 4 * 64) * sizeof(float);               \
        static scn::DeviceOnce attr_set;                                                                            \
        if (attr_set.needed()) {                                                                                         \
            SCN_HIP(hipFuncSetAttribute((const void*)k_wgrad_direct<TA_, TB_, Q_, E_, I_, H_>,                   \
                                        hipFuncAttributeMaxDynamicSharedMemorySize, 160 * 1024));                \
            attr_set.done();                                                                                     \
        }                                                                                                        \
        hipLaunchKernelGGL((k_wgrad_direct<TA_, TB_, Q_, E_, I_, H_>), grid, dim3(256), lds_, S(stream), r.X, r.cin, \
                           r.dY, r.cout, r.in_rows, r.out_rows, r.pl, r.slabs, r.relu_in, r.db_slabs, r.db_mask,  \
                           r.cout_pad, r.more);                                                                  \
    } while (0)
#define PICK_I(TA_, TB_, Q_, E_, H_)                                                                             \
    do { if (ident) LAUNCH_WD(TA_, TB_, Q_, E_, true, H_); else LAUNCH_WD(TA_, TB_, Q_, E_, false, H_); } while (0)
#define PICK_EI(TA_, TB_, Q_)                                                                                    \
    do {                                                                                                         \
        if (hb) { if (edge) PICK_I(TA_, TB_, Q_, true, true); else PICK_I(TA_, TB_, Q_, false, true); }          \
        else { if (edge) PICK_I(TA_, TB_, Q_, true, false); else PICK_I(TA_, TB_, Q_, false, false); }           \
    } while (0)
    if (r.quad) PICK_EI(4, 4, true);
    else if (r.ta == 3) { if (ident) LAUNCH_WD(3, 3, false, false, true, false); else LAUNCH_WD(3, 3, false, false, false, false); }
    else if (r.ta == 4 && r.tb == 4) PICK_EI(4, 4, false);
    else if (r.ta == 4) PICK_EI(4, 2, false);
    else if (r.tb == 4) PICK_EI(2, 4, false);
    else PICK_EI(2, 2, false);
#undef PICK_EI
#undef PICK_I
#undef LAUNCH_WD
    SCN_LAUNCH_CHECK();
    return SCN_OK;
}

int group_variant(const WdLaunch& r) {
    if (r.hb || r.edge || r.n_prob > 2 || r.pl.n_off > WG_MAXV || r.pl.n_real > WG_MAXR) return 0;
    return (r.ta == 2 && r.tb == 2 && !r.quad) ? 4 : 2;
}

struct DeferState {
    bool on = false, group = false;
    std::vector<SumArgs> jobs; std::vector<int> blocks;
    std::vector<WdLaunch> units;
};
thread_local DeferState g_defer;

struct StepState {
    bool open = false, hold = false;
    std::vector<SumArgs> jobs; std::vector<int> blocks;
    std::vector<WdLaunch> units;
    void clear() { jobs.clear(); blocks.clear(); units.clear(); }
};
thread_local StepState g_step;

struct TableRing {
    static constexpr int N = 4;
    struct Slot { char* host = nullptr; char* dev = nullptr; size_t cap = 0; hipEvent_t ev = nullptr; bool busy = false; };
    std::mutex mu;
    Slot slot[N];
    int next = 0;
    int release(Slot& s) {
        if (s.busy) SCN_HIP(hipEventSynchronize(s.ev));
        s.busy = false;
        if (s.host) SCN_HIP(hipHostFree(s.host));
        s.host = nullptr;
        if (s.dev) SCN_HIP(hipFree(s.dev));
        s.dev = nullptr;
        s.cap = 0;
        return SCN_OK;
    }
    int take(size_t bytes, Slot** out) {
        Slot& s = slot[next];
        next = (next + 1) % N;
        if (!s.ev) SCN_HIP(hipEventCreateWithFlags(&s.ev, hipEventDisableTiming));
        if (s.busy) SCN_HIP(hipEventSynchronize(s.ev));
        s.busy = false;
        if (s.cap < bytes) {
            const int rc = release(s);
            if (rc != SCN_OK) return rc;
            const size_t cap = (bytes + 65535) & ~(size_t)65535;
            SCN_HIP(hipHostMalloc((void**)&s.host, cap, hipHostMallocDefault));
            SCN_HIP(hipMalloc((void**)&s.dev, cap));
            s.cap = cap;
        }
        *out = &s;
        return SCN_OK;
    }
};
constexpr int RING_DEVICES = 64;
TableRing g_rings[RING_DEVICES];

void fill_gjob(const WdLaunch& r, GJob& J) {
    for (int p = 0; p < 2; ++p) {
        J.X[p] = p == 0 ? (const void*)r.X : (r.n_prob > 1 ? r.more.X[p] : nullptr);
        J.dY[p] = p == 0 ? (const void*)r.dY : (r.n_prob > 1 ? r.more.dY[p] : nullptr);
    }
    J.in_rows = r.in_rows; J.out_rows = r.out_rows; J.slabs = r.slabs; J.db_slabs = r.db_slabs;
    J.per = r.pl.per;
    J.cin = r.cin; J.cout = r.cout; J.relu_in = r.relu_in; J.cout_pad = r.cout_pad;
    J.n_off = r.pl.n_off; J.n_real = r.pl.n_real; J.nbi = r.pl.nbi; J.nbj = r.pl.nbj;
    J.units = r.units(); J.kind = r.kind(); J.db_mask = r.db_mask;
    for (int v = 0; v <= r.pl.n_off; ++v) J.unit_start[v] = r.pl.unit_start[v];
    for (int o = 0; o <= r.pl.n_real; ++o) J.prefix[o] = r.pl.rule_start[o];
}

void sort_members(const std::vector<WdLaunch>& R, std::vector<int>& members) {
    std::stable_sort(members.begin(), members.end(), [&](int a, int b) {
        if (R[a].wg_work() != R[b].wg_work()) return R[a].wg_work() > R[b].wg_work();
        return R[a].workgroups() > R[b].workgroups();
    });
}

template <typename SRC>
int launch_group(int var, const SRC& g, unsigned blocks, size_t lds, scn_stream_t stream) {
    if (var == 4) {
        g_counts[0].fetch_add(1, std::memory_order_relaxed);
        hipLaunchKernelGGL((k_wgrad_group<4, SRC>), dim3(blocks), dim3(256), lds, S(stream), g);
    } else {
        static scn::DeviceOnce attr_set;
        if (attr_set.needed()) {
            SCN_HIP(hipFuncSetAttribute((const void*)k_wgrad_group<2, SRC>, hipFuncAttributeMaxDynamicSharedMemorySize,
                                        160 * 1024));
            attr_set.done();
        }
        g_counts[1].fetch_add(1, std::memory_order_relaxed);
        hipLaunchKernelGGL((k_wgrad_group<2, SRC>), dim3(blocks), dim3(256), lds, S(stream), g);
    }
    SCN_LAUNCH_CHECK();
    return SCN_OK;
}

int flush_units(scn_stream_t stream) {
    std::vector<WdLaunch>& R = g_defer.units;
    if (R.empty()) return SCN_OK;
    size_t dom = 0;
    for (size_t k = 1; k < R.size(); ++k)
        if ((double)R[k].workgroups() * R[k].wg_work() > (double)R[dom].workgroups() * R[dom].wg_work()) dom = k;
    const int var = group_variant(R[dom]);
    std::vector<int> members;
    for (size_t k = 0; k < R.size(); ++k) {
        const int v = group_variant(R[k]);
        if (var != 0 && v != 0 && v >= var) members.push_back((int)k);
    }
    if (members.size() < 2) members.clear();
    std::vector<char> grouped(R.size(), 0);
    for (int k : members) grouped[k] = 1;
    for (size_t k = 0; k < R.size(); ++k)
        if (!grouped[k]) {
            const int rc = launch_direct(R[k], stream);
            if (rc != SCN_OK) return rc;
        }
    sort_members(R, members);
    for (size_t base = 0; base < members.size(); base += WG_MAX_JOBS) {
        GroupJobs g;
        memset(&g, 0, sizeof(g));
        g.n = (int)(members.size() - base < WG_MAX_JOBS ? members.size() - base : WG_MAX_JOBS);
        size_t lds = 0;
        for (int q = 0; q < g.n; ++q) {
            const WdLaunch& r = R[members[base + q]];
            fill_gjob(r, g.job[q]);
            g.block_start[q + 1] = g.block_start[q] + (int)r.workgroups();
            if (r.lds() > lds) lds = r.lds();
        }
        const int rc = launch_group(var, g, (unsigned)g.block_start[g.n], lds, stream);
        if (rc != SCN_OK) return rc;
    }
    return SCN_OK;
}

int flush_step(scn_stream_t stream) {
    const std::vector<WdLaunch>& R = g_step.units;
    std::vector<int> m2, m4;
    for (size_t k = 0; k < R.size(); ++k) {
        const int v = group_variant(R[k]);
        if (v == 4) m4.push_back((int)k);
        else if (v == 2) m2.push_back((int)k);
    }
    if (m2.size() < 2) m2.clear();
    if (m4.size() < 2) m4.clear();
    std::vector<char> grouped(R.size(), 0);
    for (int k : m2) grouped[k] = 1;
    for (int k : m4) grouped[k] = 1;
    for (size_t k = 0; k < R.size(); ++k)
        if (!grouped[k]) {
            const int rc = launch_direct(R[k], stream);
            if (rc != SCN_OK) return rc;
        }
    sort_members(R, m2);
    sort_members(R, m4);
    const size_t n2 = m2.size(), n4 = m4.size(), ns = g_step.jobs.size();
    if (n2 + n4 + ns == 0) return SCN_OK;
    auto up = [](size_t b) { return (b + 63) & ~(size_t)63; };
    const size_t o2 = 0, o4 = up(o2 + n2 * sizeof(GJob)), os = up(o4 + n4 * sizeof(GJob));
    const size_t b2 = up(os + ns * sizeof(SumArgs)), b4 = up(b2 + (n2 + 1) * sizeof(int));
    const size_t bs = up(b4 + (n4 + 1) * sizeof(int)), bytes = up(bs + (ns + 1) * sizeof(int));
    int dev_id = 0;
    SCN_HIP(hipGetDevice(&dev_id));
    SCN_REQUIRE(dev_id >= 0 && dev_id < RING_DEVICES);
    TableRing& ring = g_rings[dev_id];
    std::lock_guard<std::mutex> ring_lock(ring.mu);
    TableRing::Slot* slot = nullptr;
    int rc = ring.take(bytes, &slot);
    if (rc != SCN_OK) return rc;
    char* h = slot->host;
    memset(h, 0, bytes);
    size_t lds2 = 0, lds4 = 0;
    int* s2 = (int*)(h + b2);
    for (size_t q = 0; q < n2; ++q) {
        const WdLaunch& r = R[m2[q]];
        fill_gjob(r, ((GJob*)(h + o2))[q]);
        s2[q + 1] = s2[q] + (int)r.workgroups();
        if (r.lds() > lds2) lds2 = r.lds();
    }
    int* s4 = (int*)(h + b4);
    for (size_t q = 0; q < n4; ++q) {
        const WdLaunch& r = R[m4[q]];
        fill_gjob(r, ((GJob*)(h + o4))[q]);
        s4[q + 1] = s4[q] + (int)r.workgroups();
        if (r.lds() > lds4) lds4 = r.lds();
    }
    int* ss = (int*)(h + bs);
    for (size_t q = 0; q < ns; ++q) {
        memcpy(h + os + q * sizeof(SumArgs), &g_step.jobs[q], sizeof(SumArgs));
        ss[q + 1] = ss[q] + g_step.blocks[q];
    }
    SCN_HIP(hipMemcpyAsync(slot->dev, h, bytes, hipMemcpyHostToDevice, S(stream)));
    const char* d = slot->dev;
    if (n2) {
        GroupTable t{(const GJob*)(d + o2), (const int*)(d + b2), (int)n2};
        rc = launch_group(2, t, (unsigned)s2[n2], lds2, stream);
    }
    if (rc == SCN_OK && n4) {
        GroupTable t{(const GJob*)(d + o4), (const int*)(d + b4), (int)n4};
        rc = launch_group(4, t, (unsigned)s4[n4], lds4, stream);
    }
    if (rc == SCN_OK && ns) {
        g_counts[3].fetch_add(1, std::memory_order_relaxed);
        hipLaunchKernelGGL(k_wgradd_sum_many_tab, dim3((unsigned)ss[ns]), dim3(256), 0, S(stream),
                           (const SumArgs*)(d + os), (const int*)(d + bs), (int)ns);
        const hipError_t e = hipGetLastError();
        if (e != hipSuccess) rc = scn::fail(SCN_EHIP, "kernel launch failed: %s", hipGetErrorString(e));
    }
    if (hipEventRecord(slot->ev, S(stream)) == hipSuccess) slot->busy = true;
    else if (rc == SCN_OK) rc = scn::fail(SCN_EHIP, "%shipEventRecord failed for a job-table slot", "");
    return rc;
}
}

namespace scn {
int wgrad_defer_group(bool on) {
    if (on && !g_defer.on) return SCN_EINVAL;
    g_defer.group = on;
    return SCN_OK;
}
}

static int wgrad_impl(const float* X, int cin, const float* dY, int cout, const int32_t* in_rows,
                      const int32_t* out_rows, const int64_t* prefix_host, int n_off_real, float* dW, float* db,
                      unsigned db_mask, void* scratch, int flags, scn_stream_t stream, bool hb = false,
                      int n_prob = 1, const void* const* Xs = nullptr, const void* const* dYs = nullptr) {
    SCN_REQUIRE(prefix_host && n_off_real >= 1 && n_off_real <= 32 && cin >= 1 && cout >= 1 && dW && scratch);
    SCN_REQUIRE((in_rows == nullptr) == (out_rows == nullptr));
    SCN_REQUIRE(in_rows || n_off_real == 1);
    const bool multi = n_prob > 1;
    SCN_REQUIRE(n_prob >= 1 && n_prob <= WD_MAX_PROB && (!multi || (Xs && dYs && in_rows)));
    WdOps more{};
    uintptr_t all_ptrs = (uintptr_t)X | (uintptr_t)dY;
    for (int q = 0; multi && q < n_prob; ++q) {
        SCN_REQUIRE(Xs[q] && dYs[q]);
        more.X[q] = Xs[q];
        more.dY[q] = dYs[q];
        all_ptrs |= (uintptr_t)Xs[q] | (uintptr_t)dYs[q];
    }
    SCN_REQUIRE(!multi || (Xs[0] == (const void*)X && dYs[0] == (const void*)dY));
    const int n_off = n_prob * n_off_real;
    const bool mfma16 = hb && tb_usable(cin, cout) && ((all_ptrs & 15) == 0);
    DPlan pl;
    if (multi) SCN_REQUIRE(multi_problem_plan(cin, cout, prefix_host, n_off_real, n_prob, pl, mfma16, hb) == SCN_OK);
    else SCN_REQUIRE(make_dplan(cin, cout, prefix_host, n_off, pl, mfma16, hb) == SCN_OK);
    SCN_REQUIRE(prefix_host[n_off_real] == prefix_host[0] || (X && dY));
    SCN_REQUIRE((all_ptrs & (hb ? 1 : 3)) == 0);
    if (pl.unit_start[n_off] == 0) {
        SCN_HIP(hipMemsetAsync(dW, 0, sizeof(float) * (size_t)n_off * cin * cout, S(stream)));
        if (db) SCN_HIP(hipMemsetAsync(db, 0, sizeof(float) * (size_t)n_prob * cout, S(stream)));
        return SCN_OK;
    }
    const Shape sh = pick_shape(cin, cout, hb);
    const bool edge = (cin % (16 * sh.ta) != 0) || (cout % (16 * sh.tb) != 0) ||
                      ((all_ptrs & (sh.ta == 3 ? 3 : 15)) != 0);
    const bool ident = in_rows == nullptr;
    const int cout_pad = pl.nbj * pl.cbj;
    float* db_slabs = db ? (float*)scratch + (int64_t)pl.unit_start[n_off] * pl.nbi * pl.nbj * pl.cbi * pl.cbj : nullptr;
    dim3 grid((unsigned)pl.unit_start[n_off], 1, (unsigned)(pl.nbi * pl.nbj));
    const bool evec = edge && !hb && cin % sh.ta == 0 && cout % sh.tb == 0 && (all_ptrs & 15) == 0 &&
                      (cin * 4) % 16 == 0 && (cout * 4) % 16 == 0 && !scn::sw(scn::SW_WD_NO_EVEC).set;
    const int relu_in = ((flags & SCN_F_RELU_IN) ? 1 : 0) | (evec ? 2 : 0);
    const int V = (cout % 4 == 0 && (((uintptr_t)dW | (uintptr_t)scratch) & 15) == 0) ? 4 : 1;
    const bool deferred = g_defer.on && V == 4;
    if (mfma16) {
        const int ta = tb_tiles(cin), tb = tb_tiles(cout);
#define LAUNCH_WT(TA_, TB_, I_)                                                                                  \
    hipLaunchKernelGGL((k_wgrad_tb<TA_, TB_, I_>), grid, dim3(256), 4 * 32 * 256, S(stream), (const unsigned short*)X, cin, \
                       (const unsigned short*)dY, cout, in_rows, out_rows, pl, (float*)scratch, relu_in, db_slabs, db_mask, \
                       cout_pad, more)
#define PICK_WT(TA_, TB_) do { if (ident) LAUNCH_WT(TA_, TB_, true); else LAUNCH_WT(TA_, TB_, false); } while (0)
        if (ta == 1 && tb == 1) PICK_WT(1, 1);
        else if (ta == 1 && tb == 2) PICK_WT(1, 2);
        else if (ta == 1 && tb == 4) PICK_WT(1, 4);
        else if (ta == 2 && tb == 1) PICK_WT(2, 1);
        else if (ta == 2 && tb == 2) PICK_WT(2, 2);
        else if (ta == 2 && tb == 4) PICK_WT(2, 4);
        else if (ta == 4 && tb == 1) PICK_WT(4, 1);
        else if (ta == 4 && tb == 2) PICK_WT(4, 2);
        else PICK_WT(4, 4);
#undef PICK_WT
#undef LAUNCH_WT
        SCN_LAUNCH_CHECK();
        g_counts[2].fetch_add(1, std::memory_order_relaxed);
    } else {
        WdLaunch r;
        r.pl = pl;
        r.ta = sh.ta; r.tb = sh.tb; r.quad = sh.quad; r.edge = edge; r.ident = ident; r.hb = hb;
        if (sh.ta == 3) r.edge = false;
        r.X = X; r.dY = dY; r.cin = cin; r.cout = cout; r.relu_in = relu_in; r.cout_pad = cout_pad; r.n_prob = n_prob;
        r.in_rows = in_rows; r.out_rows = out_rows; r.slabs = (float*)scratch; r.db_slabs = db_slabs; r.db_mask = db_mask;
        r.more = more;
        if (deferred && g_defer.group) g_defer.units.push_back(r);
        else {
            const int rc = launch_direct(r, stream);
            if (rc != SCN_OK) return rc;
        }
    }
    const int64_t groups = (int64_t)n_off * cin * (cout / V);
    int G = 1;
    while (G < 16 && groups * G < 128 * 1024) G *= 2;
    SumArgs sa;
    sa.slabs = (const float*)scratch; sa.dW = dW; sa.db_slabs = db_slabs; sa.db = db;
    memcpy(sa.unit_start, pl.unit_start, sizeof(sa.unit_start));
    sa.n_off = pl.n_off; sa.n_real = pl.n_real; sa.cbi = pl.cbi; sa.cbj = pl.cbj; sa.nbi = pl.nbi; sa.nbj = pl.nbj;
    sa.cin = cin; sa.cout = cout; sa.cout_pad = cout_pad; sa.main_blocks = (int)cdiv(groups, 256 / G); sa.G = G;
    sa.db_mask = db_mask;
    const int blocks = sa.main_blocks + (db ? n_prob * cout : 0);
    if (deferred) {
        g_defer.jobs.push_back(sa);
        g_defer.blocks.push_back(blocks);
        return SCN_OK;
    }
    if (V == 4) hipLaunchKernelGGL(k_wgradd_sum<4>, dim3(blocks), dim3(256), 0, S(stream), sa);
    else hipLaunchKernelGGL(k_wgradd_sum<1>, dim3(blocks), dim3(256), 0, S(stream), sa);
    SCN_LAUNCH_CHECK();
    g_counts[3].fetch_add(1, std::memory_order_relaxed);
    return SCN_OK;
}

extern "C" int scn_wgrad_defer_begin(void) {
    g_defer.on = true;
    g_defer.group = false;
    g_defer.jobs.clear();
    g_defer.blocks.clear();
    g_defer.units.clear();
    return SCN_OK;
}

extern "C" int scn_wgrad_defer_flush(scn_stream_t stream) {
    SCN_REQUIRE(g_defer.on);
    g_defer.on = false;
    g_defer.group = false;
    if (g_step.open && g_step.hold) {
        g_step.units.insert(g_step.units.end(), g_defer.units.begin(), g_defer.units.end());
        g_step.jobs.insert(g_step.jobs.end(), g_defer.jobs.begin(), g_defer.jobs.end());
        g_step.blocks.insert(g_step.blocks.end(), g_defer.blocks.begin(), g_defer.blocks.end());
        g_defer.units.clear();
        g_defer.jobs.clear();
        g_defer.blocks.clear();
        return SCN_OK;
    }
    int rc = flush_units(stream);
    g_defer.units.clear();
    const size_t n = g_defer.jobs.size();
    for (size_t base = 0; rc == SCN_OK && base < n; base += WD_SUM_MANY) {
        SumJobs jobs;
        jobs.n = (int)(n - base < WD_SUM_MANY ? n - base : WD_SUM_MANY);
        jobs.block_start[0] = 0;
        for (int j = 0; j < jobs.n; ++j) {
            jobs.job[j] = g_defer.jobs[base + j];
            jobs.block_start[j + 1] = jobs.block_start[j] + g_defer.blocks[base + j];
        }
        if (jobs.n == 1) hipLaunchKernelGGL(k_wgradd_sum<4>, dim3(jobs.block_start[1]), dim3(256), 0, S(stream), jobs.job[0]);
        else hipLaunchKernelGGL(k_wgradd_sum_many, dim3(jobs.block_start[jobs.n]), dim3(256), 0, S(stream), jobs);
        g_counts[3].fetch_add(1, std::memory_order_relaxed);
        const hipError_t e = hipGetLastError();
        if (e != hipSuccess) rc = scn::fail(SCN_EHIP, "kernel launch failed: %s", hipGetErrorString(e));
    }
    g_defer.jobs.clear();
    g_defer.blocks.clear();
    return rc;
}

extern "C" int scn_wgrad_step_begin(void) {
    g_step.open = true;
    g_step.hold = false;
    g_step.clear();
    return SCN_OK;
}

extern "C" int scn_wgrad_step_hold(int on) {
    const scn::SwitchVal v = scn::sw(scn::SW_EXEC_GROUP_STEP);
    g_step.hold = on != 0 && g_step.open && !(v.set && v.i == 0);
    return g_step.hold ? 1 : 0;
}

extern "C" int scn_wgrad_step_flush(scn_stream_t stream) {
    SCN_REQUIRE(g_step.open);
    g_step.open = g_step.hold = false;
    const int rc = flush_step(stream);
    g_step.clear();
    return rc;
}

extern "C" int scn_wgrad_step_discard(void) {
    g_step.open = g_step.hold = false;
    g_step.clear();
    return SCN_OK;
}

extern "C" void scn_wgrad_group_counts(int64_t out[4], int reset) {
    for (int k = 0; k < 4; ++k) {
        if (out) out[k] = g_counts[k].load(std::memory_order_relaxed);
        if (reset) g_counts[k].store(0, std::memory_order_relaxed);
    }
}

extern "C" int scn_wgrad_rules(const float* X, int cin, const float* dY, int cout, const int32_t* in_rows,
                               const int32_t* out_rows, const int64_t* prefix_host, int n_off, float* dW, void* scratch,
                               int flags, scn_stream_t stream) {
    return wgrad_impl(X, cin, dY, cout, in_rows, out_rows, prefix_host, n_off, dW, nullptr, 0u, scratch, flags, stream);
}

extern "C" int scn_wgrad_rules_bf16(const uint16_t* X, int cin, const uint16_t* dY, int cout, const int32_t* in_rows,
                                    const int32_t* out_rows, const int64_t* prefix_host, int n_off, float* dW,
                                    void* scratch, int flags, scn_stream_t stream) {
    return wgrad_impl((const float*)X, cin, (const float*)dY, cout, in_rows, out_rows, prefix_host, n_off, dW, nullptr,
                      0u, scratch, flags, stream, true);
}

extern "C" int scn_wgrad_bias_rules(const float* X, int cin, const float* dY, int cout, const int32_t* in_rows,
                                    const int32_t* out_rows, const int64_t* prefix_host, int n_off, float* dW, float* db,
                                    uint32_t db_offsets, void* scratch, int flags, scn_stream_t stream) {
    SCN_REQUIRE(db && db_offsets);
    return wgrad_impl(X, cin, dY, cout, in_rows, out_rows, prefix_host, n_off, dW, db, db_offsets, scratch, flags,
                      stream);
}

extern "C" int64_t scn_wgrad_scratch_bytes_n(int cin, int cout, const int64_t* prefix_host, int n_off, int n_prob) {
    if (!prefix_host || n_off < 1 || n_off > 32 || cin < 1 || cout < 1 || n_prob < 2 || n_prob > WD_MAX_PROB) return -1;
    int64_t best = -1;
    for (int v = 0; v < 3; ++v) {
        if (v == 2 && !tb_usable(cin, cout)) continue;
        DPlan pl;
        if (multi_problem_plan(cin, cout, prefix_host, n_off, n_prob, pl, v == 2, v == 1) != SCN_OK) return -1;
        const int64_t b = (int64_t)pl.unit_start[n_prob * n_off] *
                              ((int64_t)pl.nbi * pl.nbj * pl.cbi * pl.cbj + (int64_t)pl.nbj * pl.cbj) * (int64_t)sizeof(float) + 512;
        if (b > best) best = b;
    }
    return best;
}

extern "C" int64_t scn_wgrad_scratch_bytes2(int cin, int cout, const int64_t* prefix_host, int n_off) {
    return scn_wgrad_scratch_bytes_n(cin, cout, prefix_host, n_off, 2);
}

extern "C" int scn_wgrad_bias_rules_n(const float* const* Xs, const float* const* dYs, int n_prob, int cin, int cout,
                                     const int32_t* in_rows, const int32_t* out_rows, const int64_t* prefix_host, int n_off,
                                     float* dW, float* db, uint32_t db_offsets, void* scratch, int flags,
                                     scn_stream_t stream) {
    SCN_REQUIRE(Xs && dYs && n_prob >= 2 && n_prob <= WD_MAX_PROB && in_rows && out_rows);
    SCN_REQUIRE((db != nullptr) == (db_offsets != 0));
    return wgrad_impl(Xs[0], cin, dYs[0], cout, in_rows, out_rows, prefix_host, n_off, dW, db, db_offsets, scratch, flags,
                      stream, false, n_prob, (const void* const*)Xs, (const void* const*)dYs);
}

extern "C" int scn_wgrad_bias_rules_n_bf16(const uint16_t* const* Xs, const uint16_t* const* dYs, int n_prob, int cin,
                                          int cout, const int32_t* in_rows, const int32_t* out_rows,
                                          const int64_t* prefix_host, int n_off, float* dW, float* db, uint32_t db_offsets,
                                          void* scratch, int flags, scn_stream_t stream) {
    SCN_REQUIRE(Xs && dYs && n_prob >= 2 && n_prob <= WD_MAX_PROB && in_rows && out_rows);
    SCN_REQUIRE((db != nullptr) == (db_offsets != 0));
    return wgrad_impl((const float*)Xs[0], cin, (const float*)dYs[0], cout, in_rows, out_rows, prefix_host, n_off, dW, db,
                      db_offsets, scratch, flags, stream, true, n_prob, (const void* const*)Xs, (const void* const*)dYs);
}

extern "C" int scn_wgrad_bias_rules2(const float* X0, const float* dY0, const float* X1, const float* dY1, int cin, int cout,
                                     const int32_t* in_rows, const int32_t* out_rows, const int64_t* prefix_host, int n_off,
                                     float* dW, float* db, uint32_t db_offsets, void* scratch, int flags,
                                     scn_stream_t stream) {
    const float* Xs[2] = {X0, X1};
    const float* dYs[2] = {dY0, dY1};
    return scn_wgrad_bias_rules_n(Xs, dYs, 2, cin, cout, in_rows, out_rows, prefix_host, n_off, dW, db, db_offsets, scratch,
                                 flags, stream);
}
// ... 19 lines not shown
```

### sparse_rcnn_amd/dp.py

```python
from __future__ import annotations

import contextlib
import os

import torch
import torch.distributed as dist


def _dist_on(min_world=2):
    return dist.is_available() and dist.is_initialized() and dist.get_world_size() >= min_world


class FlatParams:

    TAIL_FRACTION = 0.05
    EVENT_RING = 32

    def __init__(self, module: torch.nn.Module, n_buckets: int = 0):
        self.params = [p for p in module.parameters() if p.requires_grad]
        total = sum(p.numel() for p in self.params)
        ref = self.params[0]
        self.flat = torch.empty(total, dtype=ref.dtype, device=ref.device)
        self.flat_grad = torch.zeros(total, dtype=ref.dtype, device=ref.device)
        self.grad_views = []
# ... 90 lines not shown
    def _launch_bucket(self, b):
        ids, flat_slice = self.buckets[b]
        have = [(self.grad_views[i], self.params[i].grad) for i in ids if self.params[i].grad is not None]
        if len(have) != len(ids):
            flat_slice.zero_()
        if have:
            torch._foreach_copy_([v for v, _ in have], [g for _, g in have])
        if self.rank_weight != 1.0:
            flat_slice.mul_(self.rank_weight)
        self._works.append(dist.all_reduce(flat_slice, op=dist.ReduceOp.SUM, async_op=True))

    def zero_grad(self):
        for p in self.params:
            p.grad = None
        if self.buckets:
            self._reset_buckets()

    def gather_grads(self):
        have = [(v, p.grad) for v, p in zip(self.grad_views, self.params) if p.grad is not None]
        if len(have) != len(self.params):
            self.flat_grad.zero_()
        if have:
            torch._foreach_copy_([v for v, _ in have], [g for _, g in have])
        self.flat_grad_valid = True

    def _event_pair(self):
        if not self.flat.is_cuda:
            return None
        if len(self._events) < self.EVENT_RING:
            self._events.append((torch.cuda.Event(enable_timing=True), torch.cuda.Event(enable_timing=True)))
        pair = self._events[self._ev_used % self.EVENT_RING]
        self._ev_used += 1
        return pair

    def exposed_allreduce_ms(self):
        n = min(self._ev_used, len(self._events))
        if n == 0:
            return None
        return sum(a.elapsed_time(b) for a, b in self._events[:n]) / n

    def all_reduce_mean(self, weight: float | None = None, total_weight: float | None = None):
        if not self.sync:
            raise RuntimeError("all_reduce_mean inside `accumulate()`: the block is for the micro-batches BEFORE the last one")
        w = self.rank_weight if weight is None else float(weight)
        world = float(dist.get_world_size()) if _dist_on(1) else 1.0
        if self.buckets:
            if w != self.rank_weight:
                raise ValueError("bucketed all-reduce: set FlatParams.rank_weight BEFORE backward (slices are packed and "
                                 "scaled from the gradient hooks); got weight=%r, rank_weight=%r" % (w, self.rank_weight))
            ev = self._event_pair()
            self._drain(force=True)
            if ev is not None:
                ev[0].record()
            for wk in self._works:
                wk.wait()
            if ev is not None:
                ev[1].record()
            self.grad_scale = 1.0 / (total_weight if total_weight is not None else world)
            self.flat_grad_valid = True
            return
        self.gather_grads()
        if w != 1.0:
            self.flat_grad.mul_(w)
        if _dist_on(2):
            dist.all_reduce(self.flat_grad, op=dist.ReduceOp.SUM)
        self.grad_scale = 1.0 / (total_weight if total_weight is not None else world)

    def mean_grad(self) -> torch.Tensor:
        if not self.flat_grad_valid:
            raise RuntimeError("flat_grad was not packed by the last step (step_single_rank fast path): call "
                               "gather_grads() / all_reduce_mean(), or set SCN_STEP_PACKED=1")
        return self.flat_grad if self.grad_scale == 1.0 else self.flat_grad * self.grad_scale

    def mean_grad_views(self):
        flat, out, off = self.mean_grad(), [], 0
        for p in self.params:
            out.append(flat[off:off + p.numel()].view_as(p))
            off += p.numel()
        return out

    def sgd_step(self, lr: float):
        self.flat.add_(self.flat_grad, alpha=-lr * self.grad_scale)

    def step_single_rank(self, lr: float):
        if self.buckets or os.environ.get("SCN_STEP_PACKED") or _dist_on(2) or self.rank_weight != 1.0:
            self.all_reduce_mean()
            self.sgd_step(lr)
            return
        self.flat_grad_valid = False
        if self._datas[0].data_ptr() != self.params[0].data_ptr() or self._datas[-1].data_ptr() != self.params[-1].data_ptr():
            self._datas = [p.data for p in self.params]
        grads = [p.grad for p in self.params]
        if any(g is None for g in grads):
            have = [(d, g) for d, g in zip(self._datas, grads) if g is not None]
            if have:
                torch._foreach_add_([d for d, _ in have], [g for _, g in have], alpha=-lr)
        else:
            torch._foreach_add_(self._datas, grads, alpha=-lr)

    def adam_step(self, adam):
        adam.step_flat(self)

    def adam_step_single_rank(self, adam):
        if self.buckets or os.environ.get("SCN_STEP_PACKED") or _dist_on(2) or self.rank_weight != 1.0:
            self.all_reduce_mean()
            self.adam_step(adam)
            return
        self.flat_grad_valid = False
        if self._datas[0].data_ptr() != self.params[0].data_ptr() or self._datas[-1].data_ptr() != self.params[-1].data_ptr():
            self._datas = [p.data for p in self.params]
        adam.step_params(self._datas, [p.grad for p in self.params])


def broadcast_params(fp: FlatParams, src: int = 0):
    if _dist_on(2):
        dist.broadcast(fp.flat, src)
```

### sparse_rcnn_amd/executor.py

```python
from __future__ import annotations

import contextlib
import ctypes as C
import os
import threading

import torch

from . import _lib as L
from . import functional as F
from . import modules as M

ENABLED = os.environ.get("SCN_EXEC", "1") != "0"
SIDE_LEAVES = os.environ.get("SCN_EXEC_SIDE", "0") != "0"
_side_streams, _side_scratch = {}, {}

i32, i64, vp = C.c_int32, C.c_int64, C.c_void_p

OP_GEMM_IDENT, OP_CONV_SUBM, OP_CONV_CHILD, OP_RULES_CHILD, OP_ROWS2 = 1, 2, 3, 4, 5
OP_WGRAD_SUBM, OP_WGRAD2_SUBM, OP_WGRAD_DOWN, OP_WGRAD_UP, OP_WGRAD_IDENT, OP_COLSUM, OP_ADD, OP_CAST = 6, 7, 8, 9, 10, 11, 12, 13
XF_BF16, XF_COARSE_ROWS = 1 << 16, 1 << 17
BACK = L.F_W_TRANSPOSED | L.F_OFF_REVERSE


# ... 319 lines not shown
def compile_decoder_stage(level, up, nin, blocks, c_coarse, bf16):
    st = Stage(bf16, 2)
    c = _phys(up)
    IN0 = st.buf(level + 1, c_coarse, None, "x")
    IN1 = st.buf(level, c, None, "x")
    st.in_ids = [IN0, IN1]
    OUT = st.buf(level, c, None, "x")
    st.out_id = OUT
    mu, mn = st.mod(up, c_coarse), st.mod(nin, 2 * c)
    upb = st.buf(level, c)
    st.op(st.fwd, OP_RULES_CHILD, level, c_coarse, c, x=IN0, y=upb, w=st.param("w", mu), b=st.param("b", mu),
          flags=L.F_RELU_IN | st.hb)
    h = st.buf(level, c)
    st.op(st.fwd, OP_ROWS2, level, c, c, x=upb, x1=IN1, c1=c, y=h, w=st.param("w", mn), b=st.param("b", mn), flags=st.hb)
    last, saved = st.units_fwd(level, c, h, blocks, out_id=OUT)
    DOUT = st.buf(level, c, None, "x")
    st.dout_id = DOUT
    g = st.units_bwd(level, c, DOUT, saved)
    DIN0 = st.buf(level + 1, c_coarse, None, "x")
    DIN1 = st.buf(level, c, None, "x")
    st.din_ids = [DIN0, DIN1]
    dup = st.buf(level, c, kind="b")
    st.op(st.bwd, OP_ROWS2, level, c, c, x=g, y=dup, y1=DIN1, c1=c, w=st.param("w", mn), flags=L.F_W_TRANSPOSED | st.hb)
    gwn, gbn = st.gregion((mn, "w")), st.gregion((mn, "b"))
    st.op(st.bwd, OP_WGRAD_IDENT, level, c, c, x=upb, y=g, w=gwn, b=gbn, aux=0, flags=st.hb)
    st.op(st.bwd, OP_WGRAD_IDENT, level, c, c, x=IN1, y=g, w=gwn, b=-1, aux=c * c, flags=st.hb)
    st.op(st.bwd, OP_CONV_CHILD, level, c, c_coarse, x=dup, y=DIN0, m=IN0,
          w=st.weight(mu, c, c_coarse, 8, L.F_W_TRANSPOSED, True), flags=L.F_W_TRANSPOSED | st.hb)
    gwu, gbu = st.gregion((mu, "w")), st.gregion((mu, "b"))
    st.op(st.bwd, OP_WGRAD_UP, level, c_coarse, c, x=IN0, y=dup, w=gwu, b=gbu, flags=L.F_RELU_IN | st.hb)
    return st.freeze()


def _layout(specs, ns):
    offs, tot = [], 0
    for lv, row_bytes in specs:
        offs.append(tot)
        tot += (ns[lv] * row_bytes + 255) & ~255
    return offs, tot


def _run(stage, ops, levels, table, ptab, gtab, dev, side=False, own_scratch=None):
    if own_scratch is not None:
        return _run_plain(stage, ops, levels, table, ptab, gtab, dev, False, own_scratch)
    from . import profiling
    t = profiling.TIMER
    if t is not None and t.exec_timing():
        lib = L.lib()
        lib.scn_exec_timing_enable(1)
        try:
            return _run_plain(stage, ops, levels, table, ptab, gtab, dev, side)
        finally:
            lib.scn_exec_timing_enable(0)
    return _run_plain(stage, ops, levels, table, ptab, gtab, dev, side)


def _run_plain(stage, ops, levels, table, ptab, gtab, dev, side=False, own_scratch=None):
    lib = L.lib()
    arr, _, ns = levels
    sb, ac = i64(0), i64(0)
    L.check(lib.scn_exec_requirements(ops, len(ops), arr, len(ns), C.byref(sb), C.byref(ac)))
    if own_scratch is not None:
        scratch = torch.empty(max(sb.value, 256), dtype=torch.uint8, device=dev)
        own_scratch.append(scratch)
    else:
        scratch = L.scratch(sb.value, dev)
    arrival = L.arrival(max(ac.value, 1), dev)
    if side and SIDE_LEAVES:
        key = (dev.index, L.stream())
        st = _side_streams.get(key)
        if st is None:
            st = _side_streams[key] = torch.cuda.Stream(device=dev)
        ss = _side_scratch.get(key)
        if ss is None or ss.numel() < scratch.numel():
            ss = _side_scratch[key] = torch.empty(scratch.numel(), dtype=torch.uint8, device=dev)
        L.check(lib.scn_exec_run_streams(ops, len(ops), arr, len(ns), table, ptab, gtab, scratch.data_ptr(), scratch.numel(),
                                         arrival.data_ptr(), L.stream(), st.cuda_stream, ss.data_ptr(), ss.numel()))
        return
    L.check(lib.scn_exec_run(ops, len(ops), arr, len(ns), table, ptab, gtab, scratch.data_ptr(), scratch.numel(),
                             arrival.data_ptr(), L.stream()))


_step_scope = threading.local()
LAST_STEP_SCOPE = {"passes": 0, "delivered": 0}


class _StepScope:
    def __init__(self):
        self.deliver = []
        self.pending = set()
        self.keep = []
        self.passes = 0


def step_scope_passes():
    sc = getattr(_step_scope, "scope", None)
    return None if sc is None else sc.passes


@contextlib.contextmanager
def step_weight_gradients():
    if getattr(_step_scope, "scope", None) is not None:
        raise RuntimeError("executor.step_weight_gradients is not nestable")
    lib = L.lib()
    L.check(lib.scn_wgrad_step_begin())
    sc = _step_scope.scope = _StepScope()
    try:
        yield sc
    except BaseException:
        _step_scope.scope = None
        lib.scn_wgrad_step_discard()
        raise
    _step_scope.scope = None
    try:
        L.check(lib.scn_wgrad_step_flush(L.stream()))
    except BaseException:
        lib.scn_wgrad_step_discard()
        raise
    LAST_STEP_SCOPE["passes"], LAST_STEP_SCOPE["delivered"] = sc.passes, len(sc.deliver)
    with torch.no_grad():
        for p, view in sc.deliver:
            if p.grad is None:
                p.grad = view
            else:
                p.grad.add_(view)
    sc.keep.clear()
    sc.deliver.clear()


def _step_eligible(stage, kept, needs, pending=()):
    if stage.bf16 or SIDE_LEAVES or torch.is_grad_enabled():
        return None
    from . import profiling
    t = profiling.TIMER
    if t is not None and t.exec_timing():
        return None
    out, k = [], 0
    for mi, (m, _) in enumerate(stage.mods):
        for which, p in ((0, m.weight), (1, m.bias)):
            j = 2 * mi + which
            if p is None:
                return None
            if kept[k] is not p or not p.is_leaf:
                return None
            k += 1
            if not needs[j]:
                continue
            if p.grad is not None or id(p) in pending or p._backward_hooks or getattr(p, "_post_accumulate_grad_hooks", None):
                return None
            out.append((j, p))
    return out


LAST_FORWARD = {"lean": False, "ws_bytes": 0}


def _lean(inputs, phys):
    return not torch.is_grad_enabled() or not any(t is not None and t.requires_grad for t in (*inputs, *phys))


class StageFunction(torch.autograd.Function):

    @staticmethod
    def forward(ctx, stage, levels, lean, *ts):
        n_in = stage.n_inputs
        inputs = [F._feat(t) for t in ts[:n_in]]
        phys = ts[n_in:]
        dev = inputs[0].device
        ns = levels[2]
        lean = bool(lean) and F.RELU_RECORD is None
        offs, total = _lean_layout(stage, ns) if lean else _layout(stage.fwd_specs, ns)
        LAST_FORWARD["lean"], LAST_FORWARD["ws_bytes"] = lean, total
        ws = torch.empty(max(total, 256), dtype=torch.uint8, device=dev)
        lv, ch, es, _ = stage.bufs[stage.out_id]
        out = torch.empty((ns[lv], ch), dtype=torch.float32 if es == 4 else torch.bfloat16, device=dev)
        table = (vp * len(stage.bufs))()
        base = ws.data_ptr()
        for i, o in zip(stage.fwd_ws, offs):
            table[i] = base + o
        for i, t in zip(stage.in_ids, inputs):
            blv, bch, bes, _ = stage.bufs[i]
            if t.shape != (ns[blv], bch) or t.element_size() != bes:
                raise L.ScnError(f"executor: input slab {tuple(t.shape)} {t.dtype} where the plan expects {(ns[blv], bch)} x {bes} B")
            table[i] = t.data_ptr()
        table[stage.out_id] = out.data_ptr()
        ptab = (vp * max(len(stage.params), 1))()
        images = []
        f32 = torch.float32
        for k, j in stage.w_entries:
            t = phys[j]
            ptab[k] = (t if (t.dtype is f32 and t.is_contiguous()) else F._f32(t)).data_ptr()
        for k, j in stage.b_entries:
            t = phys[j]
            ptab[k] = 0 if t is None else (t if (t.dtype is f32 and t.is_contiguous()) else F._f32(t)).data_ptr()
        for k, j, cin, cout, n_off, fl in stage.img_entries:
            if lean and fl:
                continue
            W = phys[j]
            ent = F.packed_entry(W, cin, cout, n_off, fl)
            if ent is None:
                img = F.pack_weights_bf16(W.detach(), cin, cout, n_off, fl)
                ent = (img, img.data_ptr())
# ... 132 lines not shown
```

### sparse_rcnn_amd/trainstep.py

```python
from __future__ import annotations

import torch

from . import _lib as L
from .dp import FlatParams, broadcast_params
from .maskhead import MaskBranch
from .synthetic import make_batch, make_boxes, make_instances, make_segmentation
from .unet import Backbone

REF_PLAN = (32, 48, 64, 80, 96, 112)

WORKLOADS = {
    "cfg2": ((32, 64, 128, 256), (512, 512, 256), 150_000, 0, "configs[1]", 1),
    "cfg2-bn": ((32, 64, 128, 256), (512, 512, 256), 150_000, 0, "configs[1] with BatchNormReLU units (batchnorm=True)", 1),
    "cfg3": ((32, 64, 128, 256), (512, 512, 256), 150_000, 64, "configs[2]", 1),
    "cfg3-rpn": ((32, 64, 128, 256), (512, 512, 256), 150_000, 64, "configs[2] with the RPN boundary inside the step", 1),
    "cfg5": ((32, 64, 128, 256, 512), (1024, 1024, 512), 600_000, 0, "configs[4] shape (one scene per GPU)", 1),
    "ref": (REF_PLAN, (512, 512, 256), 150_000, 0, "configs[1] scene, the REFERENCE's own channel plan 32-48-64-80-96-112", 1),
    "ref-crop": (REF_PLAN, (128, 128, 64), 12_500, 0, "the reference's training batch: 12 crops of 128x128x64 voxels, "
                 "plan 32-48-64-80-96-112", 12),
    "ref-crop-rpn": (REF_PLAN, (128, 128, 64), 12_500, 256, "the reference's training batch (12 crops of 128x128x64, plan "
                     "32-48-64-80-96-112) with its RPN shape: two anchor levels, 5x128 / 5x256 dilation stacks, 256 kept", 12),
}


import os as _os

EARLY_ROI_CUT = _os.environ.get("SCN_ROI_EARLY", "0") != "0"
RPN_BEFORE_DECODER = _os.environ.get("SCN_RPN_EARLY", "1") != "0"
LATE_PREFETCH = _os.environ.get("SCN_LATE_PREFETCH", "1") != "0"
BACKWARD_INLINE = _os.environ.get("SCN_BACKWARD_INLINE", "1") != "0"


def _backward(roots, grads, step_scope=False):
    if step_scope:
        from . import executor
        with executor.step_weight_gradients():
            return _backward(roots, grads)
    if BACKWARD_INLINE:
        with torch.autograd.set_multithreading_enabled(False):
            torch.autograd.backward(roots, grads)
    else:
        torch.autograd.backward(roots, grads)


class SparseStepModel(torch.nn.Module):

    def __init__(self, channels, with_mask, storage, with_rpn=False, n_boxes=64, batchnorm=False, with_class=False,
                 with_segmentation=False):
        super().__init__()
        self.backbone = Backbone(7, channels, batchnorm=batchnorm, bf16_blocks=storage)
        self.mask = MaskBranch(channels[0], 7, bf16_blocks=storage) if with_mask else None
        self.rpn = self.roi_selector = None
        self.rpn_levels = None
        if with_rpn == "reference":
            from .rpn import MultiLevelRpn, RoiSelector, REF_ANCHOR_LEVELS_VOXELS
            self.rpn_levels = (2, 3)
            self.rpn = MultiLevelRpn([(channels[2], 4, 128, REF_ANCHOR_LEVELS_VOXELS[0]),
                                      (channels[3], 8, 256, REF_ANCHOR_LEVELS_VOXELS[1])], num_dilations=5,
                                     autocast_bf16=bool(storage), **(dict(keep_volume=True) if with_class == "dense" else {}))
            self.roi_selector = RoiSelector(1024, n_boxes, 0.5)
        elif with_rpn:
            from .rpn import DenseRpn, RoiSelector
            self.rpn_levels = (len(channels) - 1,)
            self.rpn = DenseRpn(channels[-1], stride=2 ** (len(channels) - 1), autocast_bf16=bool(storage),
                                **(dict(keep_volume=True) if with_class == "dense" else {}))
            self.roi_selector = RoiSelector(1024, n_boxes, 0.5)
        self.class_branch = self.segmentation = None
        self.class_level = None
        if with_class:
            if self.rpn is None:
                raise ValueError("with_class needs an RPN (the class branch reads its coarsest level)")
            from .classhead import ClassBranch, DenseClassBranch
            if with_class == "dense":
                src = self.rpn.levels[self.rpn.class_output_index] if hasattr(self.rpn, "levels") else self.rpn
                self.class_level = self.rpn_levels[self.rpn.class_output_index if hasattr(self.rpn, "levels") else 0]
                self.class_branch = DenseClassBranch(src.width, src.stride)
            else:
                self.class_level = self.rpn_levels[-1]
                self.class_branch = ClassBranch(channels[self.class_level], 2 ** self.class_level)
        if with_segmentation:
            from .classhead import SegmentationHead
            self.segmentation = SegmentationHead(channels[0], 20)

    def run_rpn(self, interims):
        lv = [interims[i] for i in self.rpn_levels]
        return self.rpn(lv if len(lv) > 1 else lv[0])

    def run_class(self, interims, boxes):
        from .classhead import DenseClassBranch
        if isinstance(self.class_branch, DenseClassBranch):
            if self.rpn.volume is None:
                raise L.ScnError("the dense class branch reads the RPN's kept volume: run_rpn first")
            slab, size, batch, md = self.rpn.volume
            return self.class_branch(slab, size, batch, boxes, metadata=md)
        return self.class_branch(interims[self.class_level], boxes)


class SceneStep:
    def __init__(self, workload="cfg2", device=None, dtype="f32", prefetch=True, seed=1, grad_seed=100, n_buckets=4,
                 target=None, channels=None, grid=None, n_boxes=None, lr=None, weighting="equal", batches_per_step=1,
                 optimizer="sgd", betas=(0.9, 0.999), eps=1e-8, weight_decay=0.0, rpn_loss=False, mask_loss=False, n_gt=None,
                 class_loss=False, segmentation_loss=False, batches=None, step_group=True, dense_class=False):
        ch, gr, tg, nb, self.baseline_entry, n_samples = WORKLOADS[workload]
        if rpn_loss and not workload.endswith("-rpn"):
            raise ValueError("rpn_loss=True needs an RPN in the step (the -rpn workloads)")
        if mask_loss and not workload.endswith("-rpn"):
            raise ValueError("mask_loss=True needs an RPN in the step (the -rpn workloads)")
        if class_loss and not workload.endswith("-rpn"):
            raise ValueError("class_loss=True needs an RPN in the step (the -rpn workloads)")
        if dense_class and not class_loss:
            raise ValueError("dense_class=True chooses the class branch's arm: it needs class_loss=True")
        if segmentation_loss and not nb:
            raise ValueError("segmentation_loss=True needs a workload with boxes (cfg3, cfg3-rpn, ref-crop-rpn): the labels "
                             "come from the scene's instances")
        if n_gt is not None and not workload.endswith("-rpn"):
            raise ValueError("n_gt applies to the ground truth of the -rpn workloads")
        if n_gt is not None and int(n_gt) < 1:
            raise ValueError("n_gt >= 1 required")
        self.n_gt = None if n_gt is None else int(n_gt)
        if batches is not None:
# ... 111 lines not shown
        self.adam = None
        if optimizer == "adam":
            from .optim import FlatAdam
            self.adam = FlatAdam(self.flat, lr=self.lr, betas=betas, eps=eps, weight_decay=weight_decay)
        self._gen = torch.Generator(device="cpu").manual_seed(grad_seed)
        self._gys, self._gms, self._grs = {}, {}, {}
        self._gm_pool = None
        self.rpn_out = None
        self._md_next = None
        self.n_active = 0
        self.n_roi_rows = 0
        self.out = self.logits = self.fin = None

    def _scene_from_batch(self, batch, k):
        from .loss import PackedMasks, pack_gt_masks
        coords, feats, size, batch_size, splits = batch["data"]
        size = torch.as_tensor(size).to("cpu", torch.long)
        factor = self._size_factor
        if any(int(v) % factor or int(v) < factor for v in size):
            raise ValueError(f"batches[{k}]: spatial size {tuple(int(v) for v in size)} is not a multiple of {factor} on every axis, "
                             f"which the {len(self.channels)}-level network of '{self.workload}'"
                             + (" with the class branch's two further 2^3/2 convolutions" if factor > 2 ** (len(self.channels) - 1)
                                else "") + f" needs: convert the samples with required_size_factor={factor}")
        if feats.shape[1] != 7:
            raise ValueError(f"batches[{k}]: 7 feature columns (colour, ones, normal) required, got {feats.shape[1]}")
        gt = [b.to(self.device, torch.float32) for b in batch["gt_bbox"]]
        gt_mask = batch["gt_mask"]
        if not isinstance(gt_mask, PackedMasks):
            gt_mask = pack_gt_masks([mk.to(self.device) for mk in gt_mask])
        return dict(coords_cpu=None, feats_cpu=None, size=size, batch_size=int(batch_size), splits=list(splits),
                    coords=coords.to(self.device), feats=feats.to(self.device, torch.float32).contiguous(), boxes=gt, gt_boxes=gt,
                    gt_dev=gt, gt_label=[l.to(self.device) for l in batch["gt_label"]], gt_mask=gt_mask, gt_mask_cpu=None,
                    seg_target=batch["gt_segmentation"].to(self.device))

    def _use_scene(self, k):
        sc = self._scenes[k]
        self.coords_cpu, self.feats_cpu, self.size, self.batch_size, self.splits = (
            sc["coords_cpu"], sc["feats_cpu"], sc["size"], sc["batch_size"], sc["splits"])
        self.coords, self.feats, self.boxes = sc["coords"], sc["feats"], sc["boxes"]
        self.gt_boxes = sc["gt_boxes"]
        self._k = k

    def _scene_shape(self):
        return tuple(float(v) for v in self.size)

    def _rpn_target_setup(self, k):
        got = self._rpn_targets.get(k)
        if got is None:
            rpn = self.model.rpn
            if hasattr(rpn, "levels"):
                calc = rpn.target_calculator(tuple(int(v) for v in self.size), self.device)
            else:
                calc = rpn.target_calculator(tuple(int(v) // rpn.stride for v in self.size), self.device)
            offs = [0]
            for b in self.gt_boxes:
                offs.append(offs[-1] + b.shape[0])
            gt = torch.cat([b.reshape(-1, 6) for b in self.gt_boxes], 0).float().to(self.device) if offs[-1] else None
            got = self._rpn_targets[k] = (calc, gt, offs)
        return got

    def _init_rpn(self):
        g = torch.Generator().manual_seed(1234)
        rpn = self.model.rpn
        with torch.no_grad():
            for h in ([r.head for r in rpn.levels] if hasattr(rpn, "levels") else [rpn.head]):
                w = torch.randn(h.weight.shape, generator=g) * 0.02
                w[6::7] = torch.randn(w[6::7].shape, generator=g) * 0.5
                h.weight.copy_(w.to(h.weight.device))
                h.bias.zero_()

    def _take_index(self, k):
        md = self._md_next.result() if self._md_next is not None else None
        self._md_next = None
        return md

    def _start_prefetch(self, k):
        if self.prefetch and self._md_next is None:
            nx = self._scenes[(k + 1) % self.batches_per_step]
            self._md_next = self.model.backbone.prefetch_in_thread(nx["coords"], nx["size"], nx["batch_size"])

    def upstream_grads(self, k=0):
        return self._gys.get(k), self._gms.get(k)

    def forward_backward(self, k=0, zero=True):
        m = self.model
        if k != self._k:
            self._use_scene(k)
        scale = 1.0 / self.batches_per_step
        fin = self.feats.detach().requires_grad_()
        md = self._take_index(k)
        if not LATE_PREFETCH:
            self._start_prefetch(k)
        rpn_state = {}

        def rpn_after_encoder(interims):
            rpn_bbox, rpn_score, anchors = m.run_rpn(interims)
            rpn_state["out"] = (rpn_bbox, rpn_score, anchors,
                                m.roi_selector.start(rpn_bbox, rpn_score, anchors, self._scene_shape()))
        hook = rpn_after_encoder if (self.with_rpn and RPN_BEFORE_DECODER) else None
        cut = None
        if m.mask is not None and EARLY_ROI_CUT and not self.mask_loss:
            cut = m.mask.prepare_cut(self.coords, self.size, self.boxes)
        rpn_prep = None
        if self.rpn_loss:
            calc, gt, offs = self._rpn_target_setup(k)
            ov, am, tg = calc.from_concatenated(gt, offs)
            rpn_prep = (ov, am, tg) + tuple(self.rpn_criterion.bbox_target_selector(ov))
        out = m.backbone(self.coords, fin, self.size, self.batch_size, metadata=md, after_encoder=hook)
        self._start_prefetch(k)
        if self.segmentation_loss:
            seg_logits = m.segmentation(out)
            if seg_logits.dtype != torch.float32:
                seg_logits = seg_logits.float()
            if self.keep_class_grads:
                seg_logits.retain_grad()
            seg_target = self._scenes[k]["seg_target"]
            self.segmentation_losses = self.segmentation_criterion(seg_logits, seg_target)
            self.segmentation_out = (seg_logits, seg_target)
            root0, gys = self.segmentation_losses, self._seg_grad
            self.n_active = int(out.features.shape[0]) * self.batches_per_step
        else:
            gy = self._gys.get(k)
            if gy is None or gy.shape != out.features.shape:
                gy = self._gys[k] = torch.randn(out.features.shape, generator=self._gen).to(self.device)
                self.n_active = sum(g.shape[0] for g in self._gys.values())
            gys = gy if scale == 1.0 else gy * scale
            root0 = out.features
        if self.weighting == "count":
            import torch.distributed as dist
            self.flat.rank_weight = float(out.features.shape[0])
            tot = torch.tensor([self.flat.rank_weight], dtype=torch.float64)
            if dist.is_available() and dist.is_initialized() and dist.get_world_size() > 1:
                tot = tot.to(self.device if dist.get_backend() == "nccl" else "cpu")
                dist.all_reduce(tot)
            self._total_weight = float(tot.item())
        if m.mask is None:
            if zero:
                self.flat.zero_grad()
            _backward([root0], [gys], step_scope=self.step_group and not self.flat.buckets and self.flat.sync)
            logits = None
        else:
            scene = (self.coords, fin, self.size, self.batch_size, self.splits)
            boxes, roots, root_grads = self.boxes, [root0], [gys]
            if self.with_rpn:
                if "out" not in rpn_state:
                    rpn_after_encoder(m.backbone.unet.interims)
                rpn_bbox, rpn_score, anchors, sel_state = rpn_state["out"]
                roi_score, boxes, roi_index = m.roi_selector.finish(sel_state)
                self.rpn_out = (rpn_bbox, rpn_score, anchors, roi_score, boxes, roi_index)
                descs = overlaps = None
                proposals = boxes
                if self.mask_loss:
                    sc = self._scenes[k]
                    overlaps, boxes, descs = self.mask_selector.select(boxes, sc["gt_dev"])
                    boxes = list(boxes)
                elif self.mask_boxes is not None:
                    boxes = [b[:self.mask_boxes] for b in boxes]
                if self.keep_rpn_grads:
                    rpn_bbox.retain_grad()
                    rpn_score.retain_grad()
                if self.rpn_loss:
                    calc = self._rpn_targets[k][0]
                    if calc.anchors.data_ptr() != anchors.data_ptr() or calc.anchors.shape != anchors.shape:
                        raise L.ScnError("SceneStep: the RPN loss's anchors are not the ones the RPN returned")
                    self.rpn_losses = self.rpn_criterion.loss(rpn_prep, rpn_score, rpn_bbox)
                    roots += list(self.rpn_losses)
                    root_grads += [self._rpn_grad, self._rpn_grad]
                else:
                    gr = self._grs.get(k)
                    if gr is None or gr[0].shape != rpn_bbox.shape:
                        gr = self._grs[k] = tuple((torch.randn(t.shape, generator=self._gen) * 1e-3).to(self.device)
                                                  for t in (rpn_bbox, rpn_score))
                    roots += [rpn_bbox, rpn_score]
                    root_grads += [g if scale == 1.0 else g * scale for g in gr]
            if self.class_loss:
                sc = self._scenes[k]
                if overlaps is None:
                    overlaps, cboxes, cdescs = self.class_selector.select(proposals, sc["gt_dev"])
                else:
                    cboxes, cdescs = self.class_selector(overlaps)
                class_scores, csel = m.run_class(m.backbone.unet.interims, list(cboxes))
                if self.keep_class_grads:
                    class_scores.retain_grad()
                sel_scores, sel_labels = self.class_loss_selector(class_scores, csel, cdescs, overlaps, sc["gt_label"])
                self.class_losses = self.class_criterion(sel_scores, sel_labels)
                self.class_out = (class_scores, csel, cdescs, sel_labels)
                roots.append(self.class_losses)
                root_grads.append(self._class_grad)
            logits, selection = m.mask(scene, out, boxes, prepared_cut=cut)
            gm = self._gms.get(k)
            if self.mask_loss:
                sc = self._scenes[k]
                if self.keep_mask_grads and logits.requires_grad:
                    logits.retain_grad()
                self.mask_out = (selection, descs)
                self.mask_losses = self.mask_criterion(logits, selection, descs, sc["gt_label"], sc["gt_mask"])
                if self.mask_losses.requires_grad:
                    roots.append(self.mask_losses)
                    root_grads.append(self._mask_grad)
                self.n_roi_rows = int(logits.shape[0])
            elif gm is None or gm.shape != logits.shape:
                if self.with_rpn:
                    pool = self._gm_pool
                    if pool is None or pool.shape[0] < logits.shape[0] or pool.shape[1:] != logits.shape[1:]:
                        rows = max(2 * logits.shape[0], 1 << 18)
                        pool = self._gm_pool = torch.randn((rows,) + tuple(logits.shape[1:]), generator=self._gen).to(self.device)
                    gm = self._gms[k] = pool[:logits.shape[0]]
                else:
                    gm = self._gms[k] = torch.randn(logits.shape, generator=self._gen).to(self.device)
                self.n_roi_rows = sum(g.shape[0] for g in self._gms.values())
            if logits.requires_grad and logits.shape[0] and not self.mask_loss:
                roots.append(logits)
                root_grads.append(gm if scale == 1.0 else gm * scale)
            if zero:
                self.flat.zero_grad()
            _backward(roots, root_grads, step_scope=self.step_group and not self.flat.buckets and self.flat.sync)
        self.out, self.logits, self.fin = out, logits, fin

    def forward_only(self, k=0):
        m = self.model
        if k != self._k:
            self._use_scene(k)
        md = self._take_index(k)
        self._start_prefetch(k)
        with torch.no_grad():
            out = m.backbone(self.coords, self.feats, self.size, self.batch_size, metadata=md)
            logits = None
            if m.mask is not None:
                scene = (self.coords, self.feats, self.size, self.batch_size, self.splits)
                boxes = self.boxes
                if self.with_rpn:
                    rpn_bbox, rpn_score, anchors = m.run_rpn(m.backbone.unet.interims)
                    _, boxes, _ = m.roi_selector(rpn_bbox, rpn_score, anchors, self._scene_shape())
                    if self.mask_boxes is not None:
                        boxes = [b[:self.mask_boxes] for b in boxes]
                logits, _ = m.mask(scene, out, boxes)
        return out, logits

    def predict(self, k=0):
        m = self.model
        if m.class_branch is None:
            raise ValueError("predict() needs the class branch: build the step with class_loss=True")
        from . import roi
        from .loss import ClassPredictor, SegmentationPredictor
        if k != self._k:
            self._use_scene(k)
        md = self._take_index(k)
        self._start_prefetch(k)
        with torch.no_grad():
            out = m.backbone(self.coords, self.feats, self.size, self.batch_size, metadata=md)
            interims = m.backbone.unet.interims
            rpn_bbox, rpn_score, anchors = m.run_rpn(interims)
            _, boxes, _ = m.roi_selector(rpn_bbox, rpn_score, anchors, self._scene_shape())
            boxes = list(boxes)
            class_scores, csel = m.run_class(interims, boxes)
            class_indices, class_prob, class_raw = ClassPredictor()(class_scores, csel)
            scene = (self.coords, self.feats, self.size, self.batch_size, self.splits)
            logits, (sel, counts, splits) = m.mask(scene, out, boxes)
            masks = roi.mask_predict(logits, sel, counts, splits, class_raw)
            result = {"roi_bbox": boxes, "class": list(class_indices), "class_propabilities": list(class_prob), "mask": masks}
            if m.segmentation is not None:
                seg = m.segmentation(out)
                result["segmentation_class"], result["segmentation_probabilites"] = SegmentationPredictor(True)(seg.float())
            self.predict_out = (class_scores, logits, (sel, counts, splits))
        return result

    def evaluate(self, scenes=None, *, score_threshold=0.9, mask_threshold=0.5, overlap_thresholds=(0.25, 0.5), eval_on_gt=True):
        m = self.model
        if m.class_branch is None:
            raise ValueError("evaluate() needs the class branch: build the step with class_loss=True")
        from . import evaluation as E
        from .loss import ClassPredictor, SegmentationPredictor, pack_gt_masks
        k_cls = m.mask.classes
        bbox_calc = E.BboxOverlapCalculator(score_threshold=score_threshold)
        mask_calc = E.MaskOverlapCalculator(mask_threshold, score_threshold=score_threshold)
        names = ["bbox", "mask"] + (["gtbbox", "gtmask", "gtlabelmask"] if eval_on_gt else [])
        acc = {n: E.OverlapAccumulator(bbox_calc if "bbox" in n else mask_calc) for n in names}
        label_acc = E.ConfusionAccumulator(E.ConfusionCalculator(k_cls))
        bin_acc = E.BinaryConfusionAccumulator(E.BinaryMaskConfusionCalculator(mask_threshold))
        seg_acc = None
        for k in (range(self.batches_per_step) if scenes is None else scenes):
            if k != self._k:
                self._use_scene(k)
            sc = self._scenes[k]
            self.finish()
            with torch.no_grad():
                out = m.backbone(self.coords, self.feats, self.size, self.batch_size, metadata=None)
                interims = m.backbone.unet.interims
                rpn_bbox, rpn_score, anchors = m.run_rpn(interims)
                roi_score, boxes, _ = m.roi_selector(rpn_bbox, rpn_score, anchors, self._scene_shape())
                roi_score, boxes = list(roi_score), list(boxes)
                class_scores, csel = m.run_class(interims, boxes)
                class_indices, _, class_raw = ClassPredictor()(class_scores, csel)
                gt_boxes, gt_label = sc["gt_dev"], sc["gt_label"]
                if eval_on_gt:
                    gt_class_scores, gcsel = m.run_class(interims, gt_boxes)
                    gt_class, _, gt_class_raw = ClassPredictor()(gt_class_scores, gcsel)
                scene = (self.coords, self.feats, self.size, self.batch_size, self.splits)
                logits, (sel, counts, splits) = m.mask(scene, out, boxes)
                pred_bits = E.mask_bits(logits, sel, counts, splits, class_raw, 0, mask_threshold)
                if "gt_mask" not in sc:
                    sc["gt_mask"] = pack_gt_masks([mk.to(self.device) for mk in sc["gt_mask_cpu"]])
                gt_mask = sc["gt_mask"]
                acc["bbox"].add_batch(roi_score, boxes, gt_boxes, list(class_indices), gt_label)
                acc["mask"].add_batch(roi_score, pred_bits, gt_mask, list(class_indices), gt_label)
                if eval_on_gt:
                    pseudo = [b.new_ones((len(b),)) for b in gt_boxes]
                    glogits, (gsel, gcounts, gsplits) = m.mask(scene, out, gt_boxes)
                    gt_bits = E.mask_bits(glogits, gsel, gcounts, gsplits, gt_class_raw, 0, mask_threshold)
                    gtl_bits = E.mask_bits(glogits, gsel, gcounts, gsplits, torch.cat(list(gt_label)), 0, mask_threshold)
                    acc["gtbbox"].add_batch(pseudo, gt_boxes, gt_boxes, list(gt_class), gt_label)
                    label_acc.add_list_batch(list(gt_class), gt_label)
                    acc["gtmask"].add_batch(pseudo, gt_bits, gt_mask, list(gt_class), gt_label)
                    acc["gtlabelmask"].add_batch(pseudo, gtl_bits, gt_mask, gt_label, gt_label)
                    bin_acc.add_batch(gtl_bits, gt_mask, gt_boxes, gt_label)
                if m.segmentation is not None and "seg_target" in sc:
                    seg_logits = m.segmentation(out).float()
                    seg_class, _ = SegmentationPredictor(True)(seg_logits)
                    seg_class_count = seg_logits.shape[1]
                    if seg_acc is None:
                        seg_acc = E.ConfusionAccumulator(E.ConfusionCalculator(int(seg_class_count)))
                    seg_acc.add_batch(seg_class, sc["seg_target"])
        helper = E.EvaluationHelper(list(overlap_thresholds), list(range(k_cls)))
        combined, single_class, _, conf, oconf, binary = helper(
            acc, {"segment": seg_acc} if seg_acc is not None else {}, {"gtbbox": label_acc} if eval_on_gt else {},
            {"gtlabelmask": bin_acc} if eval_on_gt else {})
        combined = {key: v for key, v in combined.items() if "gtbbox_AP" not in key}
        self.eval_out = dict(overlap=acc, segment=seg_acc, gtbbox=label_acc if eval_on_gt else None,
                             gtlabelmask=bin_acc if eval_on_gt else None, confusion=conf, overlap_confusion=oconf, binary=binary)
        return combined, single_class

    def step(self):
        n = self.batches_per_step
        for k in range(n - 1):
            with self.flat.accumulate():
                self.forward_backward(k, zero=(k == 0))
        self.forward_backward(n - 1, zero=(n == 1))
        if self.adam is not None:
            self.adam.lr = self.lr
            if self.weighting == "count":
                self.flat.all_reduce_mean(total_weight=self._total_weight)
                self.flat.adam_step(self.adam)
            else:
                self.flat.adam_step_single_rank(self.adam)
            return
        if self.weighting == "count":
            self.flat.all_reduce_mean(total_weight=self._total_weight)
            self.flat.sgd_step(self.lr)
            return
        self.flat.step_single_rank(self.lr)

    def finish(self):
        if self._md_next is not None:
            self._md_next.result()
            self._md_next = None

    def describe(self):
        s = (f"BASELINE {self.baseline_entry}: {self.batch_size} " + ("converted sample(s) per GPU (sample.convert_sample + collate),"
             if self.from_batches else "synthetic ScanNet-shaped sample(s) per GPU,") + f" {self.n_active} "
             f"active voxels (grid {self.grid[0]}x{self.grid[1]}x{self.grid[2]}, 1.15 points/voxel), U-Net "
             + "-".join(map(str, self.channels)) + ", 2 pre-act residual blocks/level, 2^3/2 conv+deconv"
             + (", BatchNormReLU in the residual units (training mode, fp64 statistics; layer-by-layer path)"
                if self.workload.endswith("-bn") else ""))
        if self.n_boxes and self.with_rpn:
            r = self.model.rpn
            sel = (f"-> anchors that leave the scene dropped (anchor.py:103-113) -> sigmoid, top-1024, boxes clipped to the scene, "
                   f"one-launch NMS 0.5, <= {self.n_boxes} boxes/sample" + (f", the {self.mask_boxes} best of them per sample" if self.mask_boxes else "")
                   + f" -> sparse ROI crop ({self.n_roi_rows} cropped points) -> mask "
                   "branch (SubM1 + 2 units @16, internal U-Net 23-32-48-64, Linear 23-32-18); backward from the backbone "
                   "output, rpn_bbox, rpn_score and the mask logits")
            if hasattr(r, "levels"):
                eng = r.levels[0].engine or r.levels[0].ENGINE
                s += ("; + the REFERENCE's RPN shape INSIDE the step (run.py:525-536,609,847-853): " + " + ".join(
                    f"SparseToDense of the stride-{l.stride} level ({l.channels} ch) -> dense dilation stack {l.channels}"
                    + f"-{l.width}" * (len(l.stack) // 2) + f" (3^3) + 1x1 head ({l.n_anchors} anchors/cell)" for l in r.levels)
                    + f", dense layers on engine '{eng}' "
                    + ("(this library's tile kernels on a fully active grid)" if eng == "tiles" else "(torch / MIOpen conv3d)")
                    + "; 1x1 heads instead of AnchorNetworkUpsample's transposed convolutions (dense, out of scope) " + sel)
            else:
                eng = r.engine or r.ENGINE
                s += (f"; + RPN boundary INSIDE the step, a STAND-IN lighter than the reference's (one anchor level, 2 x {r.width} "
                      f"stack, {self.n_boxes} kept; the reference: two levels, 5 x 128 / 5 x 256, 256 kept -- `ref-crop-rpn`): "
                      f"SparseToDense of the stride-{r.stride} level ({r.channels} ch) -> dense dilation stack {r.channels}"
                      + f"-{r.width}" * (len(r.stack) // 2) + f" (3^3, engine '{eng}': "
                      + ("this library's tile kernels on a fully active grid" if eng == "tiles" else "torch / MIOpen conv3d")
                      + f") + 1x1 head ({r.n_anchors} anchors/cell) " + sel)
        elif self.n_boxes:
            s += (f"; + {self.n_boxes} fp32 boxes/scene (edges 8-96 voxels) -> sparse ROI crop ({self.n_roi_rows} cropped "
                  "points) -> mask branch (SubM1 + 2 units @16, internal U-Net 23-32-48-64, Linear 23-32-18); CROP + MASK "
                  "BRANCH ONLY: the boxes are synthetic and known before the forward (no RPN in this step; "
                  "--workload cfg3-rpn has it)")
        if self.rpn_loss:
            s += ("; the RPN trains on the reference's RPN loss (BCE-with-logits + smooth L1, sigma 2) against the synthetic "
                  "boxes: device anchor targets, batch-wide 0.35 / 0.15 sampling, max weight 1/8 (scn_rpnloss.hip)")
        if self.mask_loss:
            s += ("; the mask branch trains on the reference's mask loss: IoU of the proposals against the synthetic ground "
                  "truth" + (f" (the first {self.n_gt} boxes per sample)" if self.n_gt else "") + ", TrainSelector(0.2, 0, "
                  "(24, 0, True)) draws <= 24 proposals with IoU >= 0.2 per sample and appends every ground-truth box "
                  "(one launch), BCE-with-logits of the instance's label column against its ellipsoid mask, mean over the "
                  "boxes with points (scn_maskloss.hip)")
        elif self.n_gt:
            s += f"; ground truth: the first {self.n_gt} synthetic boxes per sample"
        if self.class_loss:
            cb = self.model.class_branch
            s += (("; the DENSE class branch (1^3 conv + 1 unit @32 on the stride-" + str(cb.stride) + " volume of the RPN's dilation "
                   "stack, RoiAlign to " + "x".join(map(str, cb.cut_shape)) + " (scn_roialign.hip), max pool 2 without clamp, "
                   "2^3/2 conv + unit @64 and @128 on fully active box grids, mean pool, Linear 128-64-18) trains the stack too, "
                   "on the reference's class loss: ") if self.dense_class else
                  ("; the class branch (SubM1 + 1 unit @32 on the stride-" + str(cb.stride) + " level, sparse "
                   "ROI cut, 2^3/2 conv + unit @64 and @128, mean pool, Linear 128-64-18) trains on the reference's class loss: "))
            s += ("TrainSelector(0.1, 0, (32, 0, True)) draws <= 32 proposals with IoU >= 0.1 per sample and appends every "
                  "ground-truth box, cross entropy against the associated instance's label (scn_xent.hip)")
        if self.segmentation_loss:
            s += ("; the segmentation head (SubM 1^3 to 20 classes, one row per point) trains on the reference's segmentation "
                  "loss: cross entropy against the instances' labels + 2, -100 (ignored) outside every instance; its gradient "
                  "replaces the synthetic one at the backbone output (scn_xent.hip)")
        if self.batches_per_step > 1:
            s += (f"; {self.batches_per_step} micro-batches (scenes) accumulated per optimizer step (training.py:436,458-460), "
                  "voxels = all of them")
        if self.adam is not None:
            a = self.adam
            s += (f"; step = rulebooks + fwd + bwd (+ grad all-reduce) + Adam (the reference's optimizer, scannet_config/run.py:"
                  f"1449) on the flat parameter buffer, lr {self.lr:g}, betas ({a.betas[0]:g}, {a.betas[1]:g}), eps {a.eps:g}, "
                  f"weight decay {a.weight_decay:g}: one fused update launch per <= 80 tensors")
        else:
            s += (f"; step = rulebooks + fwd + bwd (+ grad all-reduce) + plain SGD on the flat parameter buffer, lr {self.lr:g} "
                  "(the reference trains with Adam, scannet_config/run.py:1449: three more passes over the buffer)")
        if self.step_group and not self.flat.buckets and self.dtype == "f32" and self.batches_per_step == 1:
            s += ("; fp32 weight gradients of the whole step in one grid per kernel variant after the last backward pass "
                  "(workspaces and unit slabs live until then; step_group=False: per pass)")
        if self.prefetch:
            s += "; rulebooks of batch i+1 built on a helper thread during batch i"
        return s
# ... 1 lines not shown
```

Baseline: 28.55 million.

## Fuse SGD update into deferred wgrad reduction and batch bias colsums into step flush

Adds a fused path where the end-of-step weight-gradient reduction kernel also applies the SGD update (W += alpha*grad) for parameters it owns, and reports which parameters were updated so the Python step skips them. Bias column sums in the executor are also deferred into the grouped flush: their partials run as a multi-job kernel and the final reductions are appended as extra blocks of the wgrad sum kernel. This targets launch count and the separate foreach_add pass over the parameters. It adds complexity to the bookkeeping, with a risk of parameters being updated twice or not at all if the done-set tracking goes wrong.

Result: no change. 28.72 million (median of 6 runs) (+0.6%).

```diff
diff --git a/include/scn_mi355x.h b/include/scn_mi355x.h
--- a/include/scn_mi355x.h
+++ b/include/scn_mi355x.h
@@ -174,6 +174,9 @@
 int scn_wgrad_step_flush(scn_stream_t stream);
 int scn_wgrad_step_discard(void);
 void scn_wgrad_group_counts(int64_t out[4], int reset);
+int scn_wgrad_step_flush_sgd(scn_stream_t stream, float alpha, void* const* params, const void* const* grads,
+                             const int64_t* counts, int n, int32_t* updated);
+void scn_leaf_counts(int64_t out[4], int reset);
 int64_t scn_wgrad_scratch_bytes2(int cin, int cout, const int64_t* prefix_host, int n_off);
 int scn_wgrad_bias_rules2(const float* X0, const float* dY0, const float* X1, const float* dY1, int cin, int cout,
                           const int32_t* in_rows, const int32_t* out_rows, const int64_t* prefix_host, int n_off,
@@ -194,6 +197,7 @@
 #define SCN_COLSUM_BLOCKS 512
 int scn_colsum(const float* dY, int64_t n, int c, float* db, void* scratch, scn_stream_t stream);
 int scn_colsum_bf16(const uint16_t* dY, int64_t n, int c, float* db, void* scratch, scn_stream_t stream);
+int scn_colsum_defer(const void* dY, int64_t n, int c, float* db, void* scratch, int bf16, scn_stream_t stream);
 
 
 int scn_relu_fwd(const float* X, int64_t count, float* Y, scn_stream_t stream);
diff --git a/sparse_rcnn_amd/_lib.py b/sparse_rcnn_amd/_lib.py
--- a/sparse_rcnn_amd/_lib.py
+++ b/sparse_rcnn_amd/_lib.py
@@ -87,6 +87,9 @@
     "scn_wgrad_bias_rules_n_bf16": (C.c_int, [C.POINTER(p), C.POINTER(p), i32, i32, i32, p, p, C.POINTER(i64), i32, p, p, C.c_uint32, p, i32, p]),
     "scn_colsum": (C.c_int, [p, i64, i32, p, p, p]),
     "scn_colsum_bf16": (C.c_int, [p, i64, i32, p, p, p]),
+    "scn_colsum_defer": (C.c_int, [p, i64, i32, p, p, i32, p]),
+    "scn_wgrad_step_flush_sgd": (C.c_int, [p, C.c_float, C.POINTER(p), C.POINTER(p), C.POINTER(i64), i32, C.POINTER(i32)]),
+    "scn_leaf_counts": (None, [C.POINTER(i64), i32]),
     "scn_relu_fwd": (C.c_int, [p, i64, p, p]),
     "scn_relu_bwd": (C.c_int, [p, p, i64, p, p]),
     "scn_add": (C.c_int, [p, p, i64, p, p]),
diff --git a/sparse_rcnn_amd/csrc/scn_common.h b/sparse_rcnn_amd/csrc/scn_common.h
--- a/sparse_rcnn_amd/csrc/scn_common.h
+++ b/sparse_rcnn_amd/csrc/scn_common.h
@@ -48,7 +48,7 @@
     SW_TS_SPLIT, SW_TS_SPLIT_MAX, SW_TS_NO_TAIL, SW_TS_W_HALF, SW_TS_W_BOTH, SW_TB_NB, SW_TB_KH, SW_TB_STREAM,
     SW_TB_NO_XORDER, SW_TS_STREAM, SW_TSS_NW, SW_EXEC_DEFER_SUMS, SW_PYRAMID_V1, SW_PYRAMID_ONE_STREAM, SW_WD_NO_T3,
     SW_WGRAD_BF16_MFMA, SW_WGRAD_SPLITS, SW_WD_NO_EVEC, SW_PYRAMID_NO_BRICKS, SW_CU_BUDGET, SW_EXP_A, SW_EXP_B, SW_TS_NO_CHAIN, SW_TS_PROG, SW_TB_NO_BINS,
-    SW_EXEC_GROUP_WGRAD, SW_EXEC_GROUP_STEP, SW_COUNT
+    SW_EXEC_GROUP_WGRAD, SW_EXEC_GROUP_STEP, SW_EXEC_FUSE_SGD, SW_COUNT
 };
 struct SwitchVal { bool set = false; long long i = 0; double f = 0.0; };
 SwitchVal sw(Switch s);
@@ -107,3 +107,44 @@
     const float uni = (area_a + bx[6]) - inter;
     return (inter / uni);
 }
+
+template <bool HB>
+__device__ __forceinline__ void scn_colsum_partial_block(const float* __restrict__ dY, long long n, int c,
+                                                         float* __restrict__ partial, int nblk, int blk) {
+    const unsigned short* dYh = (const unsigned short*)dY;
+    const long long rows_per_block = (n + nblk - 1) / nblk;
+    const long long r_lo = blk * rows_per_block;
+    long long r_hi = r_lo + rows_per_block;
+    if (r_hi > n) r_hi = n;
+    __shared__ float red[256];
+    for (int c0 = 0; c0 < c; c0 += 256) {
+        const int width = min(256, c - c0);
+        const int lanes_per_row = width;
+        const int rows_par = 256 / lanes_per_row > 0 ? 256 / lanes_per_row : 1;
+        const int col = threadIdx.x % lanes_per_row;
+        const int rsub = threadIdx.x / lanes_per_row;
+        float s = 0.f;
+        if (rsub < rows_par)
+            for (long long r = r_lo + rsub; r < r_hi; r += rows_par)
+                s += HB ? __uint_as_float((unsigned)dYh[r * c + c0 + col] << 16) : dY[r * c + c0 + col];
+        red[threadIdx.x] = (rsub < rows_par) ? s : 0.f;
+        __syncthreads();
+        if (threadIdx.x < width) {
+            float t = 0.f;
+            for (int k = 0; k < rows_par; ++k) t += red[k * lanes_per_row + threadIdx.x];
+            partial[(long long)blk * c + c0 + threadIdx.x] = t;
+        }
+        __syncthreads();
+    }
+}
+
+__device__ __forceinline__ float scn_colsum_final_block(const float* __restrict__ partial, int nblk, int c, int col) {
+    float s = 0.f;
+    for (int b = threadIdx.x; b < nblk; b += 256) s += partial[(long long)b * c + col];
+#pragma unroll
+    for (int d = 32; d >= 1; d >>= 1) s += __shfl_down(s, d);
+    __shared__ float w[4];
+    if ((threadIdx.x & 63) == 0) w[threadIdx.x >> 6] = s;
+    __syncthreads();
+    return (w[0] + w[1]) + (w[2] + w[3]);
+}
diff --git a/sparse_rcnn_amd/csrc/scn_conv.hip b/sparse_rcnn_amd/csrc/scn_conv.hip
--- a/sparse_rcnn_amd/csrc/scn_conv.hip
+++ b/sparse_rcnn_amd/csrc/scn_conv.hip
@@ -284,44 +284,13 @@
 template <bool HB>
 __global__ __launch_bounds__(256) void k_colsum_partial(const float* __restrict__ dY, long long n, int c,
                                                         float* __restrict__ partial) {
-    const unsigned short* dYh = (const unsigned short*)dY;
-    const long long rows_per_block = (n + gridDim.x - 1) / gridDim.x;
-    const long long r_lo = blockIdx.x * rows_per_block;
-    long long r_hi = r_lo + rows_per_block;
-    if (r_hi > n) r_hi = n;
-    __shared__ float red[256];
-    for (int c0 = 0; c0 < c; c0 += 256) {
-        const int width = min(256, c - c0);
-        const int lanes_per_row = width;
-        const int rows_par = 256 / lanes_per_row > 0 ? 256 / lanes_per_row : 1;
-        const int col = threadIdx.x % lanes_per_row;
-        const int rsub = threadIdx.x / lanes_per_row;
-        float s = 0.f;
-        if (rsub < rows_par)
-            for (long long r = r_lo + rsub; r < r_hi; r += rows_par)
-                s += HB ? bf16_bits_to_f32(dYh[r * c + c0 + col]) : dY[r * c + c0 + col];
-        red[threadIdx.x] = (rsub < rows_par) ? s : 0.f;
-        __syncthreads();
-        if (threadIdx.x < width) {
-            float t = 0.f;
-            for (int k = 0; k < rows_par; ++k) t += red[k * lanes_per_row + threadIdx.x];
-            partial[(long long)blockIdx.x * c + c0 + threadIdx.x] = t;
-        }
-        __syncthreads();
-    }
+    scn_colsum_partial_block<HB>(dY, n, c, partial, (int)gridDim.x, (int)blockIdx.x);
 }
 
 __global__ __launch_bounds__(256) void k_colsum_final(const float* __restrict__ partial, int nblk, int c,
                                                       float* __restrict__ db) {
-    const int col = blockIdx.x;
-    float s = 0.f;
-    for (int b = threadIdx.x; b < nblk; b += 256) s += partial[(long long)b * c + col];
-#pragma unroll
-    for (int d = 32; d >= 1; d >>= 1) s += __shfl_down(s, d);
-    __shared__ float w[4];
-    if ((threadIdx.x & 63) == 0) w[threadIdx.x >> 6] = s;
-    __syncthreads();
-    if (threadIdx.x == 0) db[col] = (w[0] + w[1]) + (w[2] + w[3]);
+    const float v = scn_colsum_final_block(partial, nblk, c, (int)blockIdx.x);
+    if (threadIdx.x == 0) db[blockIdx.x] = v;
 }
 
 static int colsum_impl(const float* dY, int64_t n, int c, float* db, void* scratch, scn_stream_t stream, bool hb) {
diff --git a/sparse_rcnn_amd/csrc/scn_debug.hip b/sparse_rcnn_amd/csrc/scn_debug.hip
--- a/sparse_rcnn_amd/csrc/scn_debug.hip
+++ b/sparse_rcnn_amd/csrc/scn_debug.hip
@@ -15,7 +15,7 @@
     {"SCN_WGRAD_SPLITS", {}},    {"SCN_WD_NO_EVEC", {}},    {"SCN_PYRAMID_NO_BRICKS", {}},            {"SCN_CU_BUDGET", {}},
     {"SCN_EXP_A", {}},           {"SCN_EXP_B", {}},         {"SCN_TS_NO_CHAIN", {}},
     {"SCN_TS_PROG", {}},         {"SCN_TB_NO_BINS", {}},    {"SCN_EXEC_GROUP_WGRAD", {}},
-    {"SCN_EXEC_GROUP_STEP", {}},
+    {"SCN_EXEC_GROUP_STEP", {}},  {"SCN_EXEC_FUSE_SGD", {}},
 };
 std::once_flag g_once;
 std::mutex g_mu;
diff --git a/sparse_rcnn_amd/csrc/scn_exec.hip b/sparse_rcnn_amd/csrc/scn_exec.hip
--- a/sparse_rcnn_amd/csrc/scn_exec.hip
+++ b/sparse_rcnn_amd/csrc/scn_exec.hip
@@ -26,6 +26,7 @@
 
 int64_t wgrad_scratch_of(const scn_exec_op& o, const scn_exec_level& L) {
     switch (o.op) {
+    case SCN_OP_COLSUM: return (int64_t)SCN_COLSUM_BLOCKS * o.cin * (int64_t)sizeof(float);
     case SCN_OP_WGRAD_SUBM: return scn_wgrad_scratch_bytes(o.cin, o.cout, L.prefix_host, 27);
     case SCN_OP_WGRAD2_SUBM: return scn_wgrad_scratch_bytes2(o.cin, o.cout, L.prefix_host, 27);
     case SCN_OP_WGRAD_DOWN:
@@ -155,6 +156,7 @@
     }
     case SCN_OP_COLSUM: {
         const int64_t n = rows_of(o, L);
+        if (own_scratch) return scn_colsum_defer(B<void>(c, o.x), n, o.cin, G<float>(c, o.b), c.scratch, h ? 1 : 0, st);
         if (h) return scn_colsum_bf16(B<u16>(c, o.x), n, o.cin, G<float>(c, o.b), c.scratch, st);
         return scn_colsum(B<float>(c, o.x), n, o.cin, G<float>(c, o.b), c.scratch, st);
     }
@@ -202,7 +204,10 @@
             }
             break;
         }
-        case SCN_OP_COLSUM: s = (int64_t)SCN_COLSUM_BLOCKS * o.cin * (int64_t)sizeof(float); break;
+        case SCN_OP_COLSUM:
+            s = wgrad_scratch_of(o, L);
+            ws += align256(s);
+            break;
         default: {
             const int64_t w = wgrad_scratch_of(o, L);
             if (w < 0) return scn::fail(SCN_EINVAL, "scn_exec: op %s%lld has bad arguments", "", i);
@@ -312,7 +317,7 @@
         if (align256(shared) + wg_sum <= scratch_bytes) {
             int64_t cursor = align256(shared);
             for (int i = 0; i < n_ops; ++i) {
-                const int64_t w = is_wgrad(ops[i].op) ? wgrad_scratch_of(ops[i], levels[ops[i].level]) : 0;
+                const int64_t w = is_leaf(ops[i].op) ? wgrad_scratch_of(ops[i], levels[ops[i].level]) : 0;
                 if (w > 0) { own[i] = cursor; cursor += align256(w); }
             }
             defer = true;
@@ -350,6 +355,8 @@
                 r.info[6] = child ? L.n : (L.prefix_host ? L.prefix_host[27] - L.prefix_host[0] : 0);
                 g_timing.recs.push_back(r);
             }
+        } else if (defer && ops[i].op == SCN_OP_COLSUM && overwritten_later(ops, n_ops, i, bufs)) {
+            rc = run_op(c, ops[i]);
         } else if (group && is_wgrad(ops[i].op) && overwritten_later(ops, n_ops, i, bufs)) {
             (void)scn::wgrad_defer_group(false);
             rc = run_op(c, ops[i], own[i] ? (char*)scratch + own[i] : nullptr);
diff --git a/sparse_rcnn_amd/csrc/scn_wgrad.hip b/sparse_rcnn_amd/csrc/scn_wgrad.hip
--- a/sparse_rcnn_amd/csrc/scn_wgrad.hip
+++ b/sparse_rcnn_amd/csrc/scn_wgrad.hip
@@ -405,8 +405,10 @@
     unsigned db_mask;
 };
 
+struct SgdPtrs { float* W[WD_MAX_PROB]; float* B[WD_MAX_PROB]; };
+
 template <int V, typename A>
-__device__ __forceinline__ void wgradd_sum_body(const A& a, int block) {
+__device__ __forceinline__ void wgradd_sum_body(const A& a, int block, const SgdPtrs* sgd = nullptr, float alpha = 0.f) {
     typedef typename Frag<V>::type vec_t;
     const float* __restrict__ slabs = a.slabs;
     const int cin = a.cin, cout = a.cout, G = a.G;
@@ -425,7 +427,12 @@
         __shared__ float w[4];
         if ((threadIdx.x & 63) == 0) w[threadIdx.x >> 6] = s;
         __syncthreads();
-        if (threadIdx.x == 0) a.db[cidx] = (w[0] + w[1]) + (w[2] + w[3]);
+        if (threadIdx.x == 0) {
+            const float v = (w[0] + w[1]) + (w[2] + w[3]);
+            a.db[cidx] = v;
+            float* B = sgd ? sgd->B[prob] : nullptr;
+            if (B) B[co] = fmaf(v, alpha, B[co]);
+        }
         return;
     }
     __shared__ __attribute__((aligned(16))) float part[256 * V];
@@ -464,29 +471,100 @@
             }
         }
     }
-    if (g == 0 && eg < total) *(vec_t*)(a.dW + e) = sum;
-}
-
-template <int V>
-__global__ __launch_bounds__(256) void k_wgradd_sum(SumArgs a) { wgradd_sum_body<V>(a, (int)blockIdx.x); }
-
-#define WD_SUM_MANY 6
-struct SumJobs { int n; int block_start[WD_SUM_MANY + 1]; SumArgs job[WD_SUM_MANY]; };
-
-__global__ __launch_bounds__(256) void k_wgradd_sum_many(SumJobs jobs) {
+    if (g == 0 && eg < total) {
+        *(vec_t*)(a.dW + e) = sum;
+        if (sgd) {
+            const long long per_prob = (long long)a.n_real * cin * cout;
+            const int prob = (int)(e / per_prob);
+            float* W = sgd->W[prob];
+            if (W) {
+                vec_t* wp = (vec_t*)(W + (e - prob * per_prob));
+                vec_t wv = *wp;
+#pragma unroll
+                for (int v = 0; v < V; ++v) wv[v] = fmaf(sum[v], alpha, wv[v]);
+                *wp = wv;
+            }
+        }
+    }
+}
+
+struct ColJob { const void* dY; float* partial; float* db; float* bpar; long long n; int c, nblk, hb; };
+#define WD_COL_MANY 8
+struct ColJobs { int n; int block_start[WD_COL_MANY + 1]; ColJob job[WD_COL_MANY]; };
+struct ColFinal { const float* partial; float* db; int nblk, c; };
+struct ColFinals { int n; int block_start[WD_COL_MANY + 1]; ColFinal job[WD_COL_MANY]; };
+
+__device__ __forceinline__ void colsum_partial_job(const ColJob& J, int blk) {
+    if (J.hb) scn_colsum_partial_block<true>((const float*)J.dY, J.n, J.c, J.partial, J.nblk, blk);
+    else scn_colsum_partial_block<false>((const float*)J.dY, J.n, J.c, J.partial, J.nblk, blk);
+}
+__device__ __forceinline__ void colsum_final_job(const float* partial, int nblk, int c, float* db, float* bpar, int col,
+                                                 float alpha) {
+    const float v = scn_colsum_final_block(partial, nblk, c, col);
+    if (threadIdx.x == 0) {
+        db[col] = v;
+        if (bpar) bpar[col] = fmaf(v, alpha, bpar[col]);
+    }
+}
+
+__global__ __launch_bounds__(256) void k_colsum_partial_many(ColJobs cols) {
     int j = 0;
-    while (j + 1 < jobs.n && (int)blockIdx.x >= jobs.block_start[j + 1]) ++j;
-    wgradd_sum_body<4>(jobs.job[j], (int)blockIdx.x - jobs.block_start[j]);
-}
-
-__global__ __launch_bounds__(256) void k_wgradd_sum_many_tab(const SumArgs* __restrict__ job,
-                                                             const int* __restrict__ block_start, int n) {
+    while (j + 1 < cols.n && (int)blockIdx.x >= cols.block_start[j + 1]) ++j;
+    colsum_partial_job(cols.job[j], (int)blockIdx.x - cols.block_start[j]);
+}
+__global__ __launch_bounds__(256) void k_colsum_partial_many_tab(const ColJob* __restrict__ job,
+                                                                 const int* __restrict__ block_start, int n) {
     int lo = 0, hi = n;
     while (hi - lo > 1) {
         const int mid = (lo + hi) >> 1;
         if ((int)blockIdx.x >= block_start[mid]) lo = mid; else hi = mid;
     }
-    wgradd_sum_body<4>(job[lo], (int)blockIdx.x - block_start[lo]);
+    colsum_partial_job(job[lo], (int)blockIdx.x - block_start[lo]);
+}
+
+template <int V>
+__global__ __launch_bounds__(256) void k_wgradd_sum(SumArgs a) { wgradd_sum_body<V>(a, (int)blockIdx.x); }
+
+#define WD_SUM_MANY 6
+struct SumJobs { int n; int block_start[WD_SUM_MANY + 1]; SumArgs job[WD_SUM_MANY]; };
+
+static_assert(sizeof(SumJobs) + sizeof(ColFinals) <= 4096, "k_wgradd_sum_many: kernel arguments are limited to 4 KB");
+__global__ __launch_bounds__(256) void k_wgradd_sum_many(SumJobs jobs, ColFinals cols) {
+    const int tail = (int)blockIdx.x - jobs.block_start[jobs.n];
+    if (tail >= 0) {
+        int j = 0;
+        while (j + 1 < cols.n && tail >= cols.block_start[j + 1]) ++j;
+        const ColFinal& J = cols.job[j];
+        colsum_final_job(J.partial, J.nblk, J.c, J.db, nullptr, tail - cols.block_start[j], 0.f);
+        return;
+    }
+    int j = 0;
+    while (j + 1 < jobs.n && (int)blockIdx.x >= jobs.block_start[j + 1]) ++j;
+    wgradd_sum_body<4>(jobs.job[j], (int)blockIdx.x - jobs.block_start[j]);
+}
+
+__global__ __launch_bounds__(256) void k_wgradd_sum_many_tab(const SumArgs* __restrict__ job,
+                                                             const int* __restrict__ block_start, int n,
+                                                             const ColJob* __restrict__ col,
+                                                             const int* __restrict__ col_start, int ncol,
+                                                             const SgdPtrs* __restrict__ sgd, float alpha) {
+    const int tail = n > 0 ? (int)blockIdx.x - block_start[n] : (int)blockIdx.x;
+    if (tail >= 0) {
+        int lo = 0, hi = ncol;
+        while (hi - lo > 1) {
+            const int mid = (lo + hi) >> 1;
+            if (tail >= col_start[mid]) lo = mid; else hi = mid;
+        }
+        const ColJob& J = col[lo];
+        colsum_final_job(J.partial, J.nblk, J.c, J.db, J.bpar, tail - col_start[lo], alpha);
+        return;
+    }
+    int lo = 0, hi = n;
+    while (hi - lo > 1) {
+        const int mid = (lo + hi) >> 1;
+        if ((int)blockIdx.x >= block_start[mid]) lo = mid; else hi = mid;
+    }
+    wgradd_sum_body<4>(job[lo], (int)blockIdx.x - block_start[lo], sgd ? sgd + lo : nullptr, alpha);
 }
 
 namespace {
@@ -601,6 +679,7 @@
 };
 
 std::atomic<int64_t> g_counts[4];
+std::atomic<int64_t> g_leaf[4];
 
 int launch_direct(const WdLaunch& r, scn_stream_t stream) {
     g_counts[2].fetch_add(1, std::memory_order_relaxed);
@@ -648,6 +727,7 @@
     bool on = false, group = false;
     std::vector<SumArgs> jobs; std::vector<int> blocks;
     std::vector<WdLaunch> units;
+    std::vector<ColJob> cols;
 };
 thread_local DeferState g_defer;
 
@@ -655,7 +735,8 @@
     bool open = false, hold = false;
     std::vector<SumArgs> jobs; std::vector<int> blocks;
     std::vector<WdLaunch> units;
-    void clear() { jobs.clear(); blocks.clear(); units.clear(); }
+    std::vector<ColJob> cols;
+    void clear() { jobs.clear(); blocks.clear(); units.clear(); cols.clear(); }
 };
 thread_local StepState g_step;
 
@@ -774,7 +855,65 @@
     return SCN_OK;
 }
 
-int flush_step(scn_stream_t stream) {
+struct SgdRequest {
+    float alpha; int n;
+    void* const* params; const void* const* grads; const int64_t* counts;
+    int32_t* updated;
+};
+
+int resolve_sgd(const SgdRequest& q, const std::vector<SumArgs>& jobs, std::vector<ColJob>& cols, std::vector<SgdPtrs>& out) {
+    const size_t F = sizeof(float);
+    std::vector<int64_t> covered((size_t)q.n, 0);
+    std::vector<char> bad((size_t)q.n, 0);
+    auto find = [&](const float* g, int64_t len) {
+        const uintptr_t a = (uintptr_t)g;
+        for (int k = 0; k < q.n; ++k) {
+            const uintptr_t b = (uintptr_t)q.grads[k];
+            if (b && q.params[k] && a >= b && a + len * F <= b + q.counts[k] * F) return k;
+        }
+        return -1;
+    };
+    auto param_of = [&](int k, const float* g) { return (float*)((char*)q.params[k] + ((uintptr_t)g - (uintptr_t)q.grads[k])); };
+    for (int pass = 0; pass < 2; ++pass) {
+        for (size_t j = 0; j < jobs.size(); ++j) {
+            const SumArgs& sa = jobs[j];
+            const int n_prob = sa.n_off / sa.n_real;
+            const int64_t per = (int64_t)sa.n_real * sa.cin * sa.cout;
+            for (int p = 0; p < n_prob && p < WD_MAX_PROB; ++p) {
+                const float* gw = sa.dW + p * per;
+                int k = find(gw, per);
+                if (k >= 0) {
+                    if (pass == 0) { covered[k] += per; if ((uintptr_t)param_of(k, gw) & 15) bad[k] = 1; }
+                    else if (covered[k] == q.counts[k] && !bad[k]) out[j].W[p] = param_of(k, gw);
+                }
+                if (!sa.db) continue;
+                const float* gb = sa.db + (int64_t)p * sa.cout;
+                k = find(gb, sa.cout);
+                if (k >= 0) {
+                    if (pass == 0) covered[k] += sa.cout;
+                    else if (covered[k] == q.counts[k] && !bad[k]) out[j].B[p] = param_of(k, gb);
+                }
+            }
+        }
+        for (ColJob& cj : cols) {
+            const int k = find(cj.db, cj.c);
+            if (k < 0) continue;
+            if (pass == 0) covered[k] += cj.c;
+            else if (covered[k] == q.counts[k] && !bad[k]) cj.bpar = param_of(k, cj.db);
+        }
+    }
+    int64_t done = 0;
+    for (int k = 0; k < q.n; ++k) {
+        const bool ok = q.grads[k] && q.params[k] && q.counts[k] > 0 && covered[k] == q.counts[k] && !bad[k];
+        if (q.updated) q.updated[k] = ok ? 1 : 0;
+        done += ok ? 1 : 0;
+    }
+    g_leaf[2].fetch_add(1, std::memory_order_relaxed);
+    g_leaf[3].fetch_add(done, std::memory_order_relaxed);
+    return SCN_OK;
+}
+
+int flush_step(scn_stream_t stream, const SgdRequest* sgd = nullptr) {
     const std::vector<WdLaunch>& R = g_step.units;
     std::vector<int> m2, m4;
     for (size_t k = 0; k < R.size(); ++k) {
@@ -794,12 +933,19 @@
         }
     sort_members(R, m2);
     sort_members(R, m4);
-    const size_t n2 = m2.size(), n4 = m4.size(), ns = g_step.jobs.size();
-    if (n2 + n4 + ns == 0) return SCN_OK;
+    const size_t n2 = m2.size(), n4 = m4.size(), ns = g_step.jobs.size(), nc = g_step.cols.size();
+    if (n2 + n4 + ns + nc == 0) return SCN_OK;
+    std::vector<SgdPtrs> ptrs(sgd ? ns : 0, SgdPtrs{});
+    if (sgd) {
+        const int rc_sgd = resolve_sgd(*sgd, g_step.jobs, g_step.cols, ptrs);
+        if (rc_sgd != SCN_OK) return rc_sgd;
+    }
     auto up = [](size_t b) { return (b + 63) & ~(size_t)63; };
     const size_t o2 = 0, o4 = up(o2 + n2 * sizeof(GJob)), os = up(o4 + n4 * sizeof(GJob));
-    const size_t b2 = up(os + ns * sizeof(SumArgs)), b4 = up(b2 + (n2 + 1) * sizeof(int));
-    const size_t bs = up(b4 + (n4 + 1) * sizeof(int)), bytes = up(bs + (ns + 1) * sizeof(int));
+    const size_t oc = up(os + ns * sizeof(SumArgs)), op = up(oc + nc * sizeof(ColJob));
+    const size_t b2 = up(op + ptrs.size() * sizeof(SgdPtrs)), b4 = up(b2 + (n2 + 1) * sizeof(int));
+    const size_t bs = up(b4 + (n4 + 1) * sizeof(int)), bc = up(bs + (ns + 1) * sizeof(int));
+    const size_t bf = up(bc + (nc + 1) * sizeof(int)), bytes = up(bf + (nc + 1) * sizeof(int));
     int dev_id = 0;
     SCN_HIP(hipGetDevice(&dev_id));
     SCN_REQUIRE(dev_id >= 0 && dev_id < RING_DEVICES);
@@ -830,6 +976,14 @@
         memcpy(h + os + q * sizeof(SumArgs), &g_step.jobs[q], sizeof(SumArgs));
         ss[q + 1] = ss[q] + g_step.blocks[q];
     }
+    int* sc = (int*)(h + bc);
+    int* sf = (int*)(h + bf);
+    for (size_t q = 0; q < nc; ++q) {
+        memcpy(h + oc + q * sizeof(ColJob), &g_step.cols[q], sizeof(ColJob));
+        sc[q + 1] = sc[q] + g_step.cols[q].nblk;
+        sf[q + 1] = sf[q] + g_step.cols[q].c;
+    }
+    if (!ptrs.empty()) memcpy(h + op, ptrs.data(), ptrs.size() * sizeof(SgdPtrs));
     SCN_HIP(hipMemcpyAsync(slot->dev, h, bytes, hipMemcpyHostToDevice, S(stream)));
     const char* d = slot->dev;
     if (n2) {
@@ -840,10 +994,19 @@
         GroupTable t{(const GJob*)(d + o4), (const int*)(d + b4), (int)n4};
         rc = launch_group(4, t, (unsigned)s4[n4], lds4, stream);
     }
-    if (rc == SCN_OK && ns) {
+    if (rc == SCN_OK && nc) {
+        g_leaf[0].fetch_add(1, std::memory_order_relaxed);
+        g_leaf[1].fetch_add((int64_t)nc, std::memory_order_relaxed);
+        hipLaunchKernelGGL(k_colsum_partial_many_tab, dim3((unsigned)sc[nc]), dim3(256), 0, S(stream),
+                           (const ColJob*)(d + oc), (const int*)(d + bc), (int)nc);
+        const hipError_t e = hipGetLastError();
+        if (e != hipSuccess) rc = scn::fail(SCN_EHIP, "kernel launch failed: %s", hipGetErrorString(e));
+    }
+    if (rc == SCN_OK && ns + nc) {
         g_counts[3].fetch_add(1, std::memory_order_relaxed);
-        hipLaunchKernelGGL(k_wgradd_sum_many_tab, dim3((unsigned)ss[ns]), dim3(256), 0, S(stream),
-                           (const SumArgs*)(d + os), (const int*)(d + bs), (int)ns);
+        hipLaunchKernelGGL(k_wgradd_sum_many_tab, dim3((unsigned)(ss[ns] + sf[nc])), dim3(256), 0, S(stream),
+                           (const SumArgs*)(d + os), (const int*)(d + bs), (int)ns, (const ColJob*)(d + oc),
+                           (const int*)(d + bf), (int)nc, sgd ? (const SgdPtrs*)(d + op) : nullptr, sgd ? sgd->alpha : 0.f);
         const hipError_t e = hipGetLastError();
         if (e != hipSuccess) rc = scn::fail(SCN_EHIP, "kernel launch failed: %s", hipGetErrorString(e));
     }
@@ -965,6 +1128,20 @@
     g_defer.jobs.clear();
     g_defer.blocks.clear();
     g_defer.units.clear();
+    g_defer.cols.clear();
+    return SCN_OK;
+}
+
+extern "C" int scn_colsum_defer(const void* dY, int64_t n, int c, float* db, void* scratch, int bf16, scn_stream_t stream) {
+    if (!g_defer.on)
+        return bf16 ? scn_colsum_bf16((const uint16_t*)dY, n, c, db, scratch, stream)
+                    : scn_colsum((const float*)dY, n, c, db, scratch, stream);
+    SCN_REQUIRE(n >= 0 && c >= 1 && db && scratch && (n == 0 || dY));
+    ColJob J{};
+    J.dY = dY; J.partial = (float*)scratch; J.db = db; J.bpar = nullptr; J.n = n; J.c = c; J.hb = bf16 ? 1 : 0;
+    J.nblk = (int)(n < SCN_COLSUM_BLOCKS * 8 ? cdiv(n, 8) : SCN_COLSUM_BLOCKS);
+    if (J.nblk < 1) J.nblk = 1;
+    g_defer.cols.push_back(J);
     return SCN_OK;
 }
 
@@ -976,30 +1153,56 @@
         g_step.units.insert(g_step.units.end(), g_defer.units.begin(), g_defer.units.end());
         g_step.jobs.insert(g_step.jobs.end(), g_defer.jobs.begin(), g_defer.jobs.end());
         g_step.blocks.insert(g_step.blocks.end(), g_defer.blocks.begin(), g_defer.blocks.end());
+        g_step.cols.insert(g_step.cols.end(), g_defer.cols.begin(), g_defer.cols.end());
         g_defer.units.clear();
         g_defer.jobs.clear();
         g_defer.blocks.clear();
+        g_defer.cols.clear();
         return SCN_OK;
     }
     int rc = flush_units(stream);
     g_defer.units.clear();
-    const size_t n = g_defer.jobs.size();
-    for (size_t base = 0; rc == SCN_OK && base < n; base += WD_SUM_MANY) {
+    const size_t n = g_defer.jobs.size(), nc = g_defer.cols.size();
+    for (size_t k = 0; rc == SCN_OK && (k * WD_SUM_MANY < n || k * WD_COL_MANY < nc); ++k) {
+        const size_t base = k * WD_SUM_MANY, cbase = k * WD_COL_MANY;
         SumJobs jobs;
-        jobs.n = (int)(n - base < WD_SUM_MANY ? n - base : WD_SUM_MANY);
+        jobs.n = (int)(base >= n ? 0 : (n - base < WD_SUM_MANY ? n - base : WD_SUM_MANY));
         jobs.block_start[0] = 0;
         for (int j = 0; j < jobs.n; ++j) {
             jobs.job[j] = g_defer.jobs[base + j];
             jobs.block_start[j + 1] = jobs.block_start[j] + g_defer.blocks[base + j];
         }
-        if (jobs.n == 1) hipLaunchKernelGGL(k_wgradd_sum<4>, dim3(jobs.block_start[1]), dim3(256), 0, S(stream), jobs.job[0]);
-        else hipLaunchKernelGGL(k_wgradd_sum_many, dim3(jobs.block_start[jobs.n]), dim3(256), 0, S(stream), jobs);
+        ColJobs cols;
+        ColFinals finals;
+        cols.n = (int)(cbase >= nc ? 0 : (nc - cbase < WD_COL_MANY ? nc - cbase : WD_COL_MANY));
+        cols.block_start[0] = 0;
+        for (int j = 0; j < cols.n; ++j) {
+            cols.job[j] = g_defer.cols[cbase + j];
+            cols.block_start[j + 1] = cols.block_start[j] + cols.job[j].nblk;
+        }
+        finals.n = cols.n;
+        finals.block_start[0] = 0;
+        for (int j = 0; j < cols.n; ++j) {
+            finals.job[j] = ColFinal{cols.job[j].partial, cols.job[j].db, cols.job[j].nblk, cols.job[j].c};
+            finals.block_start[j + 1] = finals.block_start[j] + cols.job[j].c;
+        }
+        if (cols.n) {
+            g_leaf[0].fetch_add(1, std::memory_order_relaxed);
+            g_leaf[1].fetch_add(cols.n, std::memory_order_relaxed);
+            hipLaunchKernelGGL(k_colsum_partial_many, dim3(cols.block_start[cols.n]), dim3(256), 0, S(stream), cols);
+        }
+        if (jobs.n == 1 && cols.n == 0)
+            hipLaunchKernelGGL(k_wgradd_sum<4>, dim3(jobs.block_start[1]), dim3(256), 0, S(stream), jobs.job[0]);
+        else
+            hipLaunchKernelGGL(k_wgradd_sum_many, dim3(jobs.block_start[jobs.n] + finals.block_start[cols.n]), dim3(256), 0,
+                               S(stream), jobs, finals);
         g_counts[3].fetch_add(1, std::memory_order_relaxed);
         const hipError_t e = hipGetLastError();
         if (e != hipSuccess) rc = scn::fail(SCN_EHIP, "kernel launch failed: %s", hipGetErrorString(e));
     }
     g_defer.jobs.clear();
     g_defer.blocks.clear();
+    g_defer.cols.clear();
     return rc;
 }
 
@@ -1022,6 +1225,28 @@
     const int rc = flush_step(stream);
     g_step.clear();
     return rc;
+}
+
+extern "C" int scn_wgrad_step_flush_sgd(scn_stream_t stream, float alpha, void* const* params, const void* const* grads,
+                                        const int64_t* counts, int n, int32_t* updated) {
+    SCN_REQUIRE(g_step.open);
+    SCN_REQUIRE(n >= 0 && (n == 0 || (params && grads && counts && updated)));
+    for (int k = 0; k < n; ++k) updated[k] = 0;
+    const scn::SwitchVal v = scn::sw(scn::SW_EXEC_FUSE_SGD);
+    if (n == 0 || (v.set && v.i == 0)) return scn_wgrad_step_flush(stream);
+    g_step.open = g_step.hold = false;
+    const SgdRequest q{alpha, n, params, grads, counts, updated};
+    const int rc = flush_step(stream, &q);
+    g_step.clear();
+    if (rc != SCN_OK) for (int k = 0; k < n; ++k) updated[k] = 0;
+    return rc;
+}
+
+extern "C" void scn_leaf_counts(int64_t out[4], int reset) {
+    for (int k = 0; k < 4; ++k) {
+        if (out) out[k] = g_leaf[k].load(std::memory_order_relaxed);
+        if (reset) g_leaf[k].store(0, std::memory_order_relaxed);
+    }
 }
 
 extern "C" int scn_wgrad_step_discard(void) {
diff --git a/sparse_rcnn_amd/dp.py b/sparse_rcnn_amd/dp.py
--- a/sparse_rcnn_amd/dp.py
+++ b/sparse_rcnn_amd/dp.py
@@ -196,8 +196,13 @@
     def sgd_step(self, lr: float):
         self.flat.add_(self.flat_grad, alpha=-lr * self.grad_scale)
 
-    def step_single_rank(self, lr: float):
-        if self.buckets or os.environ.get("SCN_STEP_PACKED") or _dist_on(2) or self.rank_weight != 1.0:
+    def single_rank_fast_path(self) -> bool:
+        return not (self.buckets or os.environ.get("SCN_STEP_PACKED") or _dist_on(2) or self.rank_weight != 1.0)
+
+    def step_single_rank(self, lr: float, done=None):
+        if not self.single_rank_fast_path():
+            if done:
+                raise RuntimeError("step_single_rank: `done` parameters on the packed path would be updated twice")
             self.all_reduce_mean()
             self.sgd_step(lr)
             return
@@ -205,8 +210,9 @@
         if self._datas[0].data_ptr() != self.params[0].data_ptr() or self._datas[-1].data_ptr() != self.params[-1].data_ptr():
             self._datas = [p.data for p in self.params]
         grads = [p.grad for p in self.params]
-        if any(g is None for g in grads):
-            have = [(d, g) for d, g in zip(self._datas, grads) if g is not None]
+        if done or any(g is None for g in grads):
+            done = done or ()
+            have = [(d, g) for d, g, p in zip(self._datas, grads, self.params) if g is not None and id(p) not in done]
             if have:
                 torch._foreach_add_([d for d, _ in have], [g for _, g in have], alpha=-lr)
         else:
diff --git a/sparse_rcnn_amd/executor.py b/sparse_rcnn_amd/executor.py
--- a/sparse_rcnn_amd/executor.py
+++ b/sparse_rcnn_amd/executor.py
@@ -425,7 +425,7 @@
 
 
 _step_scope = threading.local()
-LAST_STEP_SCOPE = {"passes": 0, "delivered": 0}
+LAST_STEP_SCOPE = {"passes": 0, "delivered": 0, "updated": 0}
 
 
 class _StepScope:
@@ -434,6 +434,7 @@
         self.pending = set()
         self.keep = []
         self.passes = 0
+        self.updated = set()
 
 
 def step_scope_passes():
@@ -441,8 +442,19 @@
     return None if sc is None else sc.passes
 
 
+def _flush_sgd(lib, sc, alpha):
+    cand = [(p, v) for p, v in sc.deliver if p.grad is None and p.dtype is torch.float32 and p.is_contiguous()]
+    n = len(cand)
+    params, grads = (vp * max(n, 1))(), (vp * max(n, 1))()
+    counts, done = (i64 * max(n, 1))(), (C.c_int32 * max(n, 1))()
+    for k, (p, v) in enumerate(cand):
+        params[k], grads[k], counts[k] = p.data_ptr(), v.data_ptr(), v.numel()
+    L.check(lib.scn_wgrad_step_flush_sgd(L.stream(), float(alpha), params, grads, counts, n, done))
+    sc.updated = {id(p) for k, (p, _) in enumerate(cand) if done[k]}
+
+
 @contextlib.contextmanager
-def step_weight_gradients():
+def step_weight_gradients(sgd_alpha=None):
     if getattr(_step_scope, "scope", None) is not None:
         raise RuntimeError("executor.step_weight_gradients is not nestable")
     lib = L.lib()
@@ -456,11 +468,15 @@
         raise
     _step_scope.scope = None
     try:
-        L.check(lib.scn_wgrad_step_flush(L.stream()))
+        if sgd_alpha is None:
+            L.check(lib.scn_wgrad_step_flush(L.stream()))
+        else:
+            _flush_sgd(lib, sc, sgd_alpha)
     except BaseException:
         lib.scn_wgrad_step_discard()
         raise
     LAST_STEP_SCOPE["passes"], LAST_STEP_SCOPE["delivered"] = sc.passes, len(sc.deliver)
+    LAST_STEP_SCOPE["updated"] = len(sc.updated)
     with torch.no_grad():
         for p, view in sc.deliver:
             if p.grad is None:
diff --git a/sparse_rcnn_amd/trainstep.py b/sparse_rcnn_amd/trainstep.py
--- a/sparse_rcnn_amd/trainstep.py
+++ b/sparse_rcnn_amd/trainstep.py
@@ -32,11 +32,12 @@
 BACKWARD_INLINE = _os.environ.get("SCN_BACKWARD_INLINE", "1") != "0"
 
 
-def _backward(roots, grads, step_scope=False):
+def _backward(roots, grads, step_scope=False, sgd_alpha=None):
     if step_scope:
         from . import executor
-        with executor.step_weight_gradients():
-            return _backward(roots, grads)
+        with executor.step_weight_gradients(sgd_alpha) as sc:
+            _backward(roots, grads)
+        return sc.updated
     if BACKWARD_INLINE:
         with torch.autograd.set_multithreading_enabled(False):
             torch.autograd.backward(roots, grads)
@@ -314,8 +315,9 @@
     def upstream_grads(self, k=0):
         return self._gys.get(k), self._gms.get(k)
 
-    def forward_backward(self, k=0, zero=True):
+    def forward_backward(self, k=0, zero=True, sgd_alpha=None):
         m = self.model
+        self._sgd_done = None
         if k != self._k:
             self._use_scene(k)
         scale = 1.0 / self.batches_per_step
@@ -369,7 +371,8 @@
         if m.mask is None:
             if zero:
                 self.flat.zero_grad()
-            _backward([root0], [gys], step_scope=self.step_group and not self.flat.buckets and self.flat.sync)
+            self._sgd_done = _backward([root0], [gys], sgd_alpha=sgd_alpha,
+                                       step_scope=self.step_group and not self.flat.buckets and self.flat.sync)
             logits = None
         else:
             scene = (self.coords, fin, self.size, self.batch_size, self.splits)
@@ -446,7 +449,8 @@
                 root_grads.append(gm if scale == 1.0 else gm * scale)
             if zero:
                 self.flat.zero_grad()
-            _backward(roots, root_grads, step_scope=self.step_group and not self.flat.buckets and self.flat.sync)
+            self._sgd_done = _backward(roots, root_grads, sgd_alpha=sgd_alpha,
+                                       step_scope=self.step_group and not self.flat.buckets and self.flat.sync)
         self.out, self.logits, self.fin = out, logits, fin
 
     def forward_only(self, k=0):
@@ -567,7 +571,10 @@
         for k in range(n - 1):
             with self.flat.accumulate():
                 self.forward_backward(k, zero=(k == 0))
-        self.forward_backward(n - 1, zero=(n == 1))
+        fuse = (self.adam is None and n == 1 and self.weighting != "count" and self.step_group and not self.flat.buckets
+                and self.flat.sync and self.flat.single_rank_fast_path())
+        self.forward_backward(n - 1, zero=(n == 1),
+                              sgd_alpha=-self.lr if fuse else None)
         if self.adam is not None:
             self.adam.lr = self.lr
             if self.weighting == "count":
@@ -580,7 +587,7 @@
             self.flat.all_reduce_mean(total_weight=self._total_weight)
             self.flat.sgd_step(self.lr)
             return
-        self.flat.step_single_rank(self.lr)
+        self.flat.step_single_rank(self.lr, done=self._sgd_done if fuse else None)
 
     def finish(self):
         if self._md_next is not None:
```
